# saifahmadgit/go2-sim2real-locomotion-rl

Measured on AMD Instinct MI355X. Metric: env-steps/sec (all envs) Go2 walk 4096 envs; 1/2/4/8-GPU scaling, higher is better.
Workload: dtype f32

## Files before the change

### go2_sim2real_locomotion_rl_amd/csrc/go2sim.hip

```cpp

#include <hip/hip_runtime.h>

#include <algorithm>
#include <cstddef>
#include <cstdint>
#include <cstdio>
#include <cstdlib>
#include <cstring>
#include <new>
#include <vector>

#include "../../include/go2sim.h"
#include "../../include/go2sim_detmath.h"

#define DEV __device__ __forceinline__
#define DEVN __device__ __noinline__

namespace {

constexpr int NL = GO2SIM_NL, ND = GO2SIM_ND, NQ = GO2SIM_NQ, NG = GO2SIM_NG, NJ = GO2SIM_NJ;
constexpr int NPAIR = GO2SIM_NPAIR_MAX, MAXC = GO2SIM_MAX_CONTACTS, MAXB = GO2SIM_MAX_BROAD, MAXR = GO2SIM_MAX_ROWS;
constexpr int JOINT_FIXED = 0, JOINT_REVOLUTE = 1, JOINT_FREE = 4;
constexpr int GEOM_PLANE = 0, GEOM_SPHERE = 1, GEOM_CYLINDER = 3, GEOM_BOX = 5, GEOM_TERRAIN = 7;
constexpr int TERRAIN_CB = 4;
// ... 573 lines not shown
  FA(geom_friction) FA3(l_pos) FA4(l_quat) FA3(root_com) FA(dof_pos) FA3(cd_vel) FA3(cd_ang) FA3(contact_force)
  FA(actions) FA(last_actions) FA(applied_actions) FA2(action_history, NA) FA(target_dof_pos) FA(e_dof_pos) FA(e_dof_vel) FA(last_dof_vel)
  FA(torque) FA(base_pos) FA(base_quat) FA(base_lin_vel) FA(base_ang_vel) FA(projected_gravity) FA(base_euler) FA(commands) FA(time_out)
  FA(kp_factors) FA(kd_factors) FA(motor_strength) FA(gravity_offset) FA(current_push_force) FA(push_stored_force) FA(feet_air_time) FA(base_vel_world) FA(last_base_pos_x)
  FA(episode_sums) FA(rew_terms) FA(rew) FA(obs) FA(priv) FA(base_kp) FA(base_kd)
  IA(n_contacts) IA(n_con) IA(err) IA(is_warmstart) IA(first_time) IA(n_broad) IA(solver_iters) IA(ctrl_mode)
  IA(gjk_fallback) IA(delay_steps) IA(episode_length) IA(reset_buf) IA(push_remaining) IA(foot_contact) IA(last_foot_contact) IA(terrain_row) IA(terrain_key)
  AA(acc) AA(qacc_ws) AA(force) AA(qf_smooth) AA(acc_smooth) AA(qfrc_constraint) AA3(cdof_ang) AA3(cdof_vel) AA3(cdofd_ang)
  AA3(cdofd_vel) AA9(cinr_inertial) AA3(cinr_pos) AA(cinr_mass) AA3(i_pos) AA4(i_quat) AA3(g_pos) AA4(g_quat) AA(sort_value) AA3(c_pos) AA3(c_normal)
  AA(c_pen) AA(c_friction) AA2(c_sol, 7) AA3(c_force) AA(efc_force) AA3(normal_cache)
  AIA(sort_ig) AIA(broad) AIA(c_geom) AIA(c_link) AIA(ncache_valid)
#undef FA
#undef FA3
#undef FA4
#undef FA2
#undef IA
#undef AA
#undef AA3
#undef AA4
#undef AA9
#undef AA2
#undef AIA
};
DEV void team_sync() {
  __builtin_amdgcn_fence(__ATOMIC_RELEASE, "workgroup");
  __builtin_amdgcn_wave_barrier();
  __builtin_amdgcn_fence(__ATOMIC_ACQUIRE, "workgroup");
}
DEV void team_sync_lds() {
  __builtin_amdgcn_fence(__ATOMIC_RELEASE, "workgroup", "local");
  __builtin_amdgcn_wave_barrier();
  __builtin_amdgcn_fence(__ATOMIC_ACQUIRE, "workgroup", "local");
}
DEV float gload(const E& e, int off, int k) { return e.f[(size_t)(off + k) * e.B]; }
DEV void gstore(const E& e, int off, int k, float v) { e.f[(size_t)(off + k) * e.B] = v; }
DEV float aload(const E& e, int off, int k) { return e.fa[off + k]; }
DEV void astore(const E& e, int off, int k, float v) { e.fa[off + k] = v; }


template <int N, int T, class F>
DEV void team_for(int tl, F f) {
#pragma unroll
  for (int k0 = 0; k0 < N; k0 += T) { int k = k0 + tl; if (k < N) f(k); }
}
template <int N, int STRIDE, int R, class FL, class FS>
DEV void team_stage_r(int k0, FL& ld, FS& st) {
  if constexpr (R * STRIDE < N) {
    int k = R * STRIDE + k0;
    k = k < N ? k : N - 1;
    const float v = ld(k);
    team_stage_r<N, STRIDE, R + 1>(k0, ld, st);
    st(k, v);
  }
}
template <int N, int T, class FL, class FS>
DEV void team_stage(int tl, FL ld, FS st) { team_stage_r<N, T, 0>(tl, ld, st); }
template <int EPW, int COUNT, class F>
DEV void wg_load(const Pool& P, int b0, int off, F put) {
  const int ev = threadIdx.x % EPW, k0 = threadIdx.x / EPW;
  const int b = (b0 + ev < P.B) ? b0 + ev : P.B - 1;
  auto ld = [&](int k) { return P.f[(size_t)(off + k) * P.B + b]; };
  auto st = [&](int k, float v) { put(ev, k, v); };
  team_stage_r<COUNT, 64 / EPW, 0>(k0, ld, st);
}

#ifdef GO2SIM_PHASE_PROFILE
// ... 8 lines not shown
#else
#define PH_BEGIN
#define PH(i)
#define PHD_BEGIN
#define PHD(i)
#define PHC(i, n)
#define PHB(i)
#endif

#ifdef GO2SIM_STAMP
constexpr int ST_KINDS = 8, ST_MAX_WG = 4096, ST_DEPTH = 4;
__device__ unsigned long long g_stamp[ST_KINDS * ST_MAX_WG * ST_DEPTH * 2];
__device__ unsigned g_stamp_cnt[ST_KINDS * ST_MAX_WG];
struct StampScope {
  int kind; unsigned long long t0;
  DEV StampScope(int k) : kind(k) { t0 = __builtin_amdgcn_s_memrealtime(); }
  DEV ~StampScope() {
    __builtin_amdgcn_s_waitcnt(0);
    const unsigned long long t1 = __builtin_amdgcn_s_memrealtime();
    if (threadIdx.x == 0 && blockIdx.x < ST_MAX_WG) {
      const int w = kind * ST_MAX_WG + (int)blockIdx.x;
      const unsigned c = g_stamp_cnt[w];
      g_stamp[(w * ST_DEPTH + (int)(c % ST_DEPTH)) * 2] = t0; g_stamp[(w * ST_DEPTH + (int)(c % ST_DEPTH)) * 2 + 1] = t1;
      g_stamp_cnt[w] = c + 1;
    }
  }
};
#define STAMP(kind) StampScope stamp_scope_(kind);
#else
#define STAMP(kind)
#endif
enum { STK_PRE_DYN = 0, STK_COLLIDE, STK_SOLVE, STK_INT_FK_DYN, STK_INT_FK, STK_POST_A, STK_POST_B, STK_OTHER };

enum { SV_COST = 0, SV_PREV_COST, SV_GAUSS, SV_QG0, SV_QG1, SV_QG2, SV_GTOL };
enum { SI_LS_IT = 0, SI_LS_RESULT, SI_IMPROVED };

DEV V3 ld3(const float* p, int i) { return v3(p[3 * i], p[3 * i + 1], p[3 * i + 2]); }
DEV void st3(float* p, int i, V3 v) { p[3 * i] = v.x; p[3 * i + 1] = v.y; p[3 * i + 2] = v.z; }
DEV Q4 ld4(const float* p, int i) { return q4(p[4 * i], p[4 * i + 1], p[4 * i + 2], p[4 * i + 3]); }
DEV void st4(float* p, int i, Q4 q) { p[4 * i] = q.w; p[4 * i + 1] = q.x; p[4 * i + 2] = q.y; p[4 * i + 3] = q.z; }
DEV M3 ld9(const float* p, int i) { M3 r;
#pragma unroll
  for (int k = 0; k < 9; ++k) r.m[k / 3][k % 3] = p[9 * i + k];
  return r; }
DEV void st9(float* p, int i, const M3& r) {
#pragma unroll
  for (int k = 0; k < 9; ++k) p[9 * i + k] = r.m[k / 3][k % 3]; }

DEV int xcd_block() {
  const int n = (int)gridDim.x, q = n >> 3, r = n & 7, x = (int)blockIdx.x & 7, i = (int)blockIdx.x >> 3;
  return (x < r ? x * (q + 1) : r * (q + 1) + (x - r) * q) + i;
}

constexpr int LPT_CLS = 32;
DEV int lpt_solver_xcd(int b, int B, int epw_s) {
  const int n = (B + epw_s - 1) / epw_s, q = n >> 3, r = n & 7, L = b / epw_s;
  if (L < r * (q + 1)) return L / (q + 1);
  return r + (L - r * (q + 1)) / (q > 0 ? q : 1);
}
DEV void lpt_file(int* __restrict__ rec, int cap, int L, int B, int epw_s, int nc) {
  const int x = lpt_solver_xcd(L * epw_s, B, epw_s), cls = LPT_CLS - 1 - imn(LPT_CLS - 1, nc);
  const int pos = atomicAdd(&rec[x * LPT_CLS + cls], 1);
  if (pos < cap) rec[8 * LPT_CLS + (x * LPT_CLS + cls) * cap + pos] = L;
}
DEV int lpt_take(const int* __restrict__ rec, int cap, int B, int epw, int slot) {
  const int ident = xcd_block() * epw + slot;
// ... 6 lines not shown
  for (int c = 0; c < LPT_CLS; ++c) {
    const int k = rec[x * LPT_CLS + c];
    if (cls < 0 && local < total + k) { cls = c; off = local - total; }
    total += k;
  }
  if (total != expected) return ident;
  if (cls < 0 || off >= cap) return B;
  return rec[8 * LPT_CLS + (x * LPT_CLS + cls) * cap + off] * epw + slot;
}

struct KinData {
  float qpos[NQ], vel[ND], qpos_next[NQ], vel_next[ND];
  float l_pos[NL * 3], l_quat[NL * 4], i_pos[NL * 3], i_quat[NL * 4];
  float xanchor[NJ * 3], xaxis[NJ * 3];
  float cdof_ang[ND * 3], cdof_vel[ND * 3];
  float cd_vel[NL * 3], cd_ang[NL * 3];
  float mass[NL];
  int valid;
};

#ifndef GO2SIM_FAST_ORDER
#define GO2SIM_FAST_ORDER 1
#endif
template <int CTRL>
DEV float dpp_perm(float x) { return __int_as_float(__builtin_amdgcn_update_dpp(0, __float_as_int(x), CTRL, 0xf, 0xf, true)); }
#if GO2SIM_FAST_ORDER
constexpr bool ARROW_SHAPE = (ND == 18);
DEV float leg_sum4(float x) {
  const auto r = __builtin_amdgcn_permlane16_swap(__float_as_uint(x), __float_as_uint(x), false, false);
  const float p = __uint_as_float(r[0]) + __uint_as_float(r[1]);
  return p + dpp_perm<0x128>(p);
}
DEV float4 lds4(const float* p) { return *(const float4*)p; }
template <int T, int STRIDE>
DEV void arrow_factor(const int mode, const float eps, const float* A, float* F, int tl) {
  static_assert(T == 32 || T == 64, "four groups of eight lanes");
  const int leg = (tl >> 3) & 3, u = tl & 7, ub = u < 6 ? u : 5;
  const int p0 = dm_arrow_dof(mode, leg, 0), p1 = dm_arrow_dof(mode, leg, 1), p2 = dm_arrow_dof(mode, leg, 2);
  const bool w_lane = tl < 32 && u < 6;
  const float a00 = A[p0 * STRIDE + p0], a10 = A[p1 * STRIDE + p0], a11 = A[p1 * STRIDE + p1];
  const float a20 = A[p2 * STRIDE + p0], a21 = A[p2 * STRIDE + p1], a22 = A[p2 * STRIDE + p2];
  const float c0 = A[p0 * STRIDE + ub], c1 = A[p1 * STRIDE + ub], c2 = A[p2 * STRIDE + ub];
  float br[6];
#pragma unroll
  for (int j = 0; j < 6; ++j) br[j] = A[ub * STRIDE + j];
  team_sync();
  const float e0 = fmx(a00, eps), i0 = dm_sqrt(e0) * (1.0f / e0);
  const float l10 = a10 * i0, l20 = a20 * i0;
  const float e1 = fmx(__builtin_fmaf(-l10, l10, a11), eps), i1 = dm_sqrt(e1) * (1.0f / e1);
  const float l21 = __builtin_fmaf(-l20, l10, a21) * i1;
  const float e2 = fmx(__builtin_fmaf(-l21, l21, __builtin_fmaf(-l20, l20, a22)), eps), i2 = dm_sqrt(e2) * (1.0f / e2);
  const float w0 = c0 * i0, w1 = __builtin_fmaf(-w0, l10, c1) * i1, w2 = __builtin_fmaf(-w1, l21, __builtin_fmaf(-w0, l20, c2)) * i2;
  if (w_lane) *(float4*)&F[32 * leg + 8 + 4 * u] = make_float4(w0, w1, w2, 0.0f);
  if (tl < 32 && u == 0) { *(float4*)&F[32 * leg] = make_float4(i0, i1, i2, 0.0f); *(float4*)&F[32 * leg + 4] = make_float4(l10, l20, l21, 0.0f); }
  team_sync();
  float sc[6];
#pragma unroll
  for (int j = 0; j < 6; ++j) {
    const float4 wj = lds4(&F[32 * leg + 8 + 4 * j]);
    sc[j] = __builtin_fmaf(w2, wj.z, __builtin_fmaf(w1, wj.y, w0 * wj.x));
  }
#pragma unroll
  for (int j = 0; j < 6; ++j) sc[j] = leg_sum4(sc[j]);
  const float bp[6] = {br[0] - sc[0], br[1] - sc[1], br[2] - sc[2], br[3] - sc[3], br[4] - sc[4], br[5] - sc[5]};
  if (tl < 6) { *(float4*)&F[128 + 8 * tl] = make_float4(bp[0], bp[1], bp[2], bp[3]); *(float4*)&F[128 + 8 * tl + 4] = make_float4(bp[4], bp[5], 0.0f, 0.0f); }
  team_sync();
  float a[6][6];
#pragma unroll
  for (int k = 0; k < 6; ++k) {
    const float4 lo = lds4(&F[128 + 8 * k]); const float2 hi = *(const float2*)&F[128 + 8 * k + 4];
    a[k][0] = lo.x; a[k][1] = lo.y; a[k][2] = lo.z; a[k][3] = lo.w; a[k][4] = hi.x; a[k][5] = hi.y;
  }
  team_sync();
#pragma unroll
  for (int k = 0; k < 6; ++k) {
    const float e = fmx(a[k][k], eps), ik = dm_sqrt(e) * (1.0f / e);
    a[k][k] = ik;
#pragma unroll
    for (int j = k + 1; j < 6; ++j) a[j][k] = a[j][k] * ik;
#pragma unroll
    for (int j = k + 1; j < 6; ++j)
#pragma unroll
      for (int i = k + 1; i <= j; ++i) a[j][i] = __builtin_fmaf(-a[j][k], a[i][k], a[j][i]);
  }
  if (tl == 0) {
#pragma unroll
    for (int k = 0; k < 6; ++k) {
      *(float4*)&F[128 + 8 * k] = make_float4(a[k][0], k >= 1 ? a[k][1] : 0.0f, k >= 2 ? a[k][2] : 0.0f, k >= 3 ? a[k][3] : 0.0f);
      *(float2*)&F[128 + 8 * k + 4] = make_float2(k >= 4 ? a[k][4] : 0.0f, k >= 5 ? a[k][5] : 0.0f);
    }
  }
  team_sync();
}
template <int T>
DEV void arrow_solve(const float* F, float gl0, float gl1, float gl2, float gb, float* x6, int tl, float (&xb)[6], float& xl0, float& xl1, float& xl2) {
  static_assert(T == 32 || T == 64, "four groups of eight lanes");
  const int leg = (tl >> 3) & 3, u = tl & 7, ub = u < 6 ? u : 5;
  const float4 iv = lds4(&F[32 * leg]), lv = lds4(&F[32 * leg + 4]), wo = lds4(&F[32 * leg + 8 + 4 * ub]);
  float4 W[6];
#pragma unroll
  for (int b = 0; b < 6; ++b) W[b] = lds4(&F[32 * leg + 8 + 4 * b]);
  float L[6][6];
#pragma unroll
  for (int k = 0; k < 6; ++k) {
    const float4 lo = lds4(&F[128 + 8 * k]); const float2 hi = *(const float2*)&F[128 + 8 * k + 4];
    L[k][0] = lo.x; L[k][1] = lo.y; L[k][2] = lo.z; L[k][3] = lo.w; L[k][4] = hi.x; L[k][5] = hi.y;
  }
  const float y0 = gl0 * iv.x, y1 = __builtin_fmaf(-lv.x, y0, gl1) * iv.y, y2 = __builtin_fmaf(-lv.z, y1, __builtin_fmaf(-lv.y, y0, gl2)) * iv.z;
  const float z = leg_sum4(__builtin_fmaf(wo.z, y2, __builtin_fmaf(wo.y, y1, wo.x * y0)));
  if (tl < 6) x6[tl] = gb - z;
  team_sync();
  const float2 r0 = *(const float2*)&x6[0], r1 = *(const float2*)&x6[2], r2 = *(const float2*)&x6[4];
  float x[6] = {r0.x, r0.y, r1.x, r1.y, r2.x, r2.y};
  team_sync();
#pragma unroll
  for (int k = 0; k < 6; ++k) {
    float acc = x[k];
#pragma unroll
    for (int j = 0; j < k; ++j) acc = __builtin_fmaf(-L[k][j], x[j], acc);
    x[k] = acc * L[k][k];
  }
#pragma unroll
  for (int k_ = 0; k_ < 6; ++k_) {
    const int k = 5 - k_;
    float acc = x[k];
#pragma unroll
    for (int j_ = 0; j_ < 5 - k; ++j_) { const int j = 5 - j_; acc = __builtin_fmaf(-L[j][k], x[j], acc); }
    x[k] = acc * L[k][k];
  }
  float v0 = y0, v1 = y1, v2 = y2;
#pragma unroll
  for (int b = 0; b < 6; ++b) { v0 = __builtin_fmaf(-W[b].x, x[b], v0); v1 = __builtin_fmaf(-W[b].y, x[b], v1); v2 = __builtin_fmaf(-W[b].z, x[b], v2); }
  xl2 = v2 * iv.z; xl1 = __builtin_fmaf(-lv.z, xl2, v1) * iv.y; xl0 = __builtin_fmaf(-lv.x, xl1, __builtin_fmaf(-lv.y, xl2, v0)) * iv.x;
#pragma unroll
  for (int k = 0; k < 6; ++k) xb[k] = x[k];
}
#endif
struct DynData {
  float cinr_I[NL * 9], cinr_pos[NL * 3], cinr_mass[NL];
  float crb_I[NL * 9], crb_pos[NL * 3], crb_mass[NL];
  float cdof_ang[ND * 3], cdof_vel[ND * 3], cdofd_ang[ND * 3], cdofd_vel[ND * 3];
  float cd_vel[NL * 3], cd_ang[NL * 3], cdd_vel[NL * 3], cdd_ang[NL * 3], cfrc_vel[NL * 3], cfrc_ang[NL * 3];
  float f_ang[ND * 3], f_vel[ND * 3];
  float vel[ND], qf_applied[ND], qf_passive[ND], force[ND], out[ND], Dinv[ND];
  float M[ND * ND], L[ND * ND];
  int ctrl_mode[ND];
};
// ... 34 lines not shown
      ql = rotvec_to_quat(m.dofs[J.dof_start].motion_ang * dp, m.eps);
    }
    Q4 qloc[LEG_D];
#pragma unroll
    for (int d = 0; d < LEG_D; ++d) {
      const int src = tl < LEG_K ? LEG_D * tl + d : 0;
      qloc[d] = q4(__shfl(ql.w, src, T), __shfl(ql.x, src, T), __shfl(ql.y, src, T), __shfl(ql.z, src, T));
    }
    if (tl < LEG_K) {
      int lk[LEG_D], jk[LEG_D];
      V3 lpos[LEG_D], jpos[LEG_D], axis[LEG_D]; Q4 lquat[LEG_D];
#pragma unroll
      for (int d = 0; d < LEG_D; ++d) {
        lk[d] = m.leg_links[LEG_D * tl + d];
        const auto& L = m.links[lk[d]];
        jk[d] = L.joint_start;
        const Joint& J = m.joints[jk[d]];
        lpos[d] = L.pos; lquat[d] = L.quat; jpos[d] = J.pos; axis[d] = m.dofs[J.dof_start].motion_ang;
      }
      V3 pos = rpos; Q4 quat = rquat;
#pragma unroll
      for (int d = 0; d < LEG_D; ++d) {
        const Q4 pq = quat;
        pos = pos + transform_by_quat(lpos[d], pq);
        quat = transform_quat_by_quat(lquat[d], pq);
        const V3 anchor = transform_by_quat(jpos[d], quat) + pos;
        st3(s->xanchor, jk[d], anchor);
        st3(s->xaxis, jk[d], transform_by_quat(axis[d], quat));
        quat = transform_quat_by_quat(qloc[d], quat);
        pos = anchor - transform_by_quat(jpos[d], quat);
        st3(s->l_pos, lk[d], pos); st4(s->l_quat, lk[d], quat); e.l_pos()[lk[d]] = pos; e.l_quat()[lk[d]] = quat;
      }
    }
    team_sync();
  }
  for (int lev = 0; lev < (legs ? 0 : m.n_levels); ++lev) {
    for (int k = m.level_start[lev] + tl; k < m.level_start[lev + 1]; k += T) {
      int i_l = m.level_links[k];
      const auto& L = m.links[i_l];
      V3 pos = L.pos; Q4 quat = L.quat;
      if (L.parent != -1) {
        Q4 pq = ld4(s->l_quat, L.parent);
        pos = ld3(s->l_pos, L.parent) + transform_by_quat(L.pos, pq);
        quat = transform_quat_by_quat(L.quat, pq);
      }
      for (int i_j = L.joint_start; i_j < L.joint_end; ++i_j) {
        const Joint& J = m.joints[i_j];
        int q_start = J.q_start, dof_start = J.dof_start;
        if (J.type == JOINT_FREE) {
          V3 pos_ = v3(s->qpos[q_start], s->qpos[q_start + 1], s->qpos[q_start + 2]);
          st3(s->xanchor, i_j, pos_);
          st3(s->xaxis, i_j, v3(0, 0, 1));
          Q4 quat_ = q4(s->qpos[q_start + 3], s->qpos[q_start + 4], s->qpos[q_start + 5], s->qpos[q_start + 6]);
          float n = dm_sqrt(norm_sqr(quat_));
          quat_ = q4(quat_.w / n, quat_.x / n, quat_.y / n, quat_.z / n);
          pos = pos_; quat = quat_;
          gstore(e, FO(dof_pos), dof_start + 0, pos.x); gstore(e, FO(dof_pos), dof_start + 1, pos.y); gstore(e, FO(dof_pos), dof_start + 2, pos.z);
          if (dk) { dk->out[dof_start] = pos.x; dk->out[dof_start + 1] = pos.y; dk->out[dof_start + 2] = pos.z; }
        } else if (J.type == JOINT_REVOLUTE) {
          V3 axis = m.dofs[dof_start].motion_ang;
          V3 anchor = transform_by_quat(J.pos, quat) + pos;
          st3(s->xanchor, i_j, anchor);
          st3(s->xaxis, i_j, transform_by_quat(axis, quat));
          float dp = s->qpos[q_start] - m.qpos0[q_start];
          gstore(e, FO(dof_pos), dof_start, dp);
          if (dk) dk->out[dof_start] = dp;
          Q4 qloc = rotvec_to_quat(axis * dp, m.eps);
          quat = transform_quat_by_quat(qloc, quat);
          pos = anchor - transform_by_quat(J.pos, quat);
        }
      }
      if (!(L.parent == -1 && L.is_fixed)) { st3(s->l_pos, i_l, pos); st4(s->l_quat, i_l, quat); e.l_pos()[i_l] = pos; e.l_quat()[i_l] = quat; }
    }
    team_sync();
  }
  PH(18)
  for (int i_l = tl; i_l < NL; i_l += T) {
    const auto& L = m.links[i_l];
    s->mass[i_l] = L.mass + gload(e, FO(mass_shift), i_l);
    V3 ipbw; Q4 iq;
    transform_pos_quat_by_trans_quat(L.inertial_pos + (V3)e.com_shift()[i_l], L.inertial_quat, ld3(s->l_pos, i_l), ld4(s->l_quat, i_l), ipbw, iq);
    st3(s->i_pos, i_l, ipbw); st4(s->i_quat, i_l, iq);
  }
  team_sync();
  V3 rc[2];
#pragma unroll
  for (int i_e = 0; i_e < 2; ++i_e) {
    const Entity& en = m.entities[i_e];
    V3 root_com_bw = v3(0, 0, 0); float mass_sum = 0.0f;
    for (int i_l = en.link_start; i_l < en.link_end; ++i_l) {
      float mass = s->mass[i_l];
      mass_sum = mass_sum + mass;
      root_com_bw = root_com_bw + mass * ld3(s->i_pos, i_l);
    }
    rc[i_e] = root_com_bw / mass_sum;
  }
  team_sync();
  for (int i_l = tl; i_l < NL; i_l += T) {
    const auto& L = m.links[i_l];
    V3 r = (L.entity == 0) ? rc[0] : rc[1];
    e.root_com()[i_l] = r;
    V3 ip = ld3(s->i_pos, i_l) - r;
    Q4 iq = ld4(s->i_quat, i_l);
    if (!dk) e.i_pos()[i_l] = ip;
    e.i_quat()[i_l] = iq;
    float i_mass = s->mass[i_l];
    M3 oI; V3 op;
    transform_inertia_by_trans_quat(L.inertial_i, i_mass, ip, iq, m.eps, oI, op);
    if (!dk) { e.cinr_inertial()[i_l] = oI; e.cinr_pos()[i_l] = op; e.cinr_mass()[i_l] = i_mass; }
    if (dk) { st9(dk->cinr_I, i_l, oI); st9(dk->crb_I, i_l, oI); st3(dk->cinr_pos, i_l, op); st3(dk->crb_pos, i_l, op); dk->cinr_mass[i_l] = i_mass; dk->crb_mass[i_l] = i_mass; }
  }
  for (int i_j = tl; i_j < NJ; i_j += T) {
    const Joint& J = m.joints[i_j];
    const auto& L = m.links[J.link];
    if (L.n_dofs == 0) continue;
    V3 r = (L.entity == 0) ? rc[0] : rc[1];
    V3 offset_pos = r - ld3(s->xanchor, i_j);
    int ds = J.dof_start;
    if (J.type == JOINT_REVOLUTE) {
      V3 ax = ld3(s->xaxis, i_j);
      V3 cv = cross(ax, offset_pos);
      st3(s->cdof_ang, ds, ax); st3(s->cdof_vel, ds, cv);
      e.cdof_ang()[ds] = ax; e.cdof_vel()[ds] = cv;
      if (dk) { st3(dk->cdof_ang, ds, ax); st3(dk->cdof_vel, ds, cv); }
    } else if (J.type == JOINT_FREE) {
      for (int i = 0; i < 3; ++i) {
        V3 cv = v3(0, 0, 0);
        vset(cv, i, 1.0f);
        st3(s->cdof_ang, i + ds, v3(0, 0, 0)); st3(s->cdof_vel, i + ds, cv);
        e.cdof_ang()[i + ds] = v3(0, 0, 0); e.cdof_vel()[i + ds] = cv;
        if (dk) { st3(dk->cdof_ang, i + ds, v3(0, 0, 0)); st3(dk->cdof_vel, i + ds, cv); }
      }
      M3 xmat_T = transpose(quat_to_R(ld4(s->l_quat, J.link), m.eps));
#pragma unroll
      for (int i = 0; i < 3; ++i) {
        V3 row = v3(xmat_T.m[i][0], xmat_T.m[i][1], xmat_T.m[i][2]);
        V3 cv = cross(row, offset_pos);
        st3(s->cdof_ang, i + ds + 3, row); st3(s->cdof_vel, i + ds + 3, cv);
        e.cdof_ang()[i + ds + 3] = row; e.cdof_vel()[i + ds + 3] = cv;
        if (dk) { st3(dk->cdof_ang, i + ds + 3, row); st3(dk->cdof_vel, i + ds + 3, cv); }
      }
    }
  }
  for (int i_g = tl; i_g < NG; i_g += T) {
    const auto& G = m.geoms[i_g];
    bool is_fixed = m.links[G.link].is_fixed;
    if (force_update_fixed || !is_fixed) {
      V3 p; Q4 q;
      transform_pos_quat_by_trans_quat(G.pos, G.quat, ld3(s->l_pos, G.link), ld4(s->l_quat, G.link), p, q);
      e.g_pos()[i_g] = p; e.g_quat()[i_g] = q;
    }
  }
  team_sync();
  PH(19)
  if (legs) {
    const int r = m.leg_root, ds = m.links[r].dof_start;
    float v[6]; V3 ca[6], cv[6];
#pragma unroll
    for (int i = 0; i < 6; ++i) { v[i] = s->vel[ds + i]; ca[i] = ld3(s->cdof_ang, ds + i); cv[i] = ld3(s->cdof_vel, ds + i); }
    V3 cvel_vel = v3(0, 0, 0), cvel_ang = v3(0, 0, 0);
#pragma unroll
    for (int i = 0; i < 3; ++i) { cvel_vel = cvel_vel + cv[i] * v[i]; cvel_ang = cvel_ang + ca[i] * v[i]; }
    if (tl == 0) {
#pragma unroll
      for (int i = 0; i < 3; ++i) {
        if (!dk) { e.cdofd_ang()[ds + i] = v3(0, 0, 0); e.cdofd_vel()[ds + i] = v3(0, 0, 0); }
        if (dk) { st3(dk->cdofd_ang, ds + i, v3(0, 0, 0)); st3(dk->cdofd_vel, ds + i, v3(0, 0, 0)); }
        V3 oa, ov;
        motion_cross_motion(cvel_ang, cvel_vel, ca[i + 3], cv[i + 3], oa, ov);
        if (!dk) { e.cdofd_ang()[ds + i + 3] = oa; e.cdofd_vel()[ds + i + 3] = ov; }
        if (dk) { st3(dk->cdofd_ang, ds + i + 3, oa); st3(dk->cdofd_vel, ds + i + 3, ov); }
      }
    }
#pragma unroll
    for (int i = 0; i < 3; ++i) { cvel_vel = cvel_vel + cv[i + 3] * v[i + 3]; cvel_ang = cvel_ang + ca[i + 3] * v[i + 3]; }
    if (tl == 0) {
      st3(s->cd_vel, r, cvel_vel); st3(s->cd_ang, r, cvel_ang);
      if (!dk) { e.cd_vel()[r] = cvel_vel; e.cd_ang()[r] = cvel_ang; }
      if (dk) { st3(dk->cd_vel, r, cvel_vel); st3(dk->cd_ang, r, cvel_ang); }
    }
    for (int i_l = tl; i_l < NL; i_l += T) {
      if (m.links[i_l].parent != -1 || i_l == r) continue;
      st3(s->cd_vel, i_l, v3(0, 0, 0)); st3(s->cd_ang, i_l, v3(0, 0, 0));
      if (!dk) { e.cd_vel()[i_l] = v3(0, 0, 0); e.cd_ang()[i_l] = v3(0, 0, 0); }
      if (dk) { st3(dk->cd_vel, i_l, v3(0, 0, 0)); st3(dk->cd_ang, i_l, v3(0, 0, 0)); }
    }
    if (tl < LEG_K) {
      int lk[LEG_D], dd[LEG_D]; float lv[LEG_D]; V3 la[LEG_D], lc[LEG_D];
#pragma unroll
      for (int d = 0; d < LEG_D; ++d) {
        lk[d] = m.leg_links[LEG_D * tl + d];
        dd[d] = m.links[lk[d]].dof_start;
        lv[d] = s->vel[dd[d]]; la[d] = ld3(s->cdof_ang, dd[d]); lc[d] = ld3(s->cdof_vel, dd[d]);
      }
#pragma unroll
      for (int d = 0; d < LEG_D; ++d) {
        V3 oa, ov;
        motion_cross_motion(cvel_ang, cvel_vel, la[d], lc[d], oa, ov);
        if (!dk) { e.cdofd_ang()[dd[d]] = oa; e.cdofd_vel()[dd[d]] = ov; }
        if (dk) { st3(dk->cdofd_ang, dd[d], oa); st3(dk->cdofd_vel, dd[d], ov); }
        cvel_vel = cvel_vel + lc[d] * lv[d];
        cvel_ang = cvel_ang + la[d] * lv[d];
        st3(s->cd_vel, lk[d], cvel_vel); st3(s->cd_ang, lk[d], cvel_ang);
        if (!dk) { e.cd_vel()[lk[d]] = cvel_vel; e.cd_ang()[lk[d]] = cvel_ang; }
        if (dk) { st3(dk->cd_vel, lk[d], cvel_vel); st3(dk->cd_ang, lk[d], cvel_ang); }
      }
    }
    team_sync();
  }
  for (int lev = 0; lev < (legs ? 0 : m.n_levels); ++lev) {
    for (int k = m.level_start[lev] + tl; k < m.level_start[lev + 1]; k += T) {
      int i_l = m.level_links[k];
      const auto& L = m.links[i_l];
      V3 cvel_vel = v3(0, 0, 0), cvel_ang = v3(0, 0, 0);
      if (L.parent != -1) { cvel_vel = ld3(s->cd_vel, L.parent); cvel_ang = ld3(s->cd_ang, L.parent); }
      for (int i_j = L.joint_start; i_j < L.joint_end; ++i_j) {
        const Joint& J = m.joints[i_j];
        int ds = J.dof_start;
        if (J.type == JOINT_FREE) {
          for (int i = 0; i < 3; ++i) {
            float v = s->vel[ds + i];
            cvel_vel = cvel_vel + ld3(s->cdof_vel, ds + i) * v;
            cvel_ang = cvel_ang + ld3(s->cdof_ang, ds + i) * v;
          }
          for (int i = 0; i < 3; ++i) {
            if (!dk) { e.cdofd_ang()[ds + i] = v3(0, 0, 0); e.cdofd_vel()[ds + i] = v3(0, 0, 0); }
            if (dk) { st3(dk->cdofd_ang, ds + i, v3(0, 0, 0)); st3(dk->cdofd_vel, ds + i, v3(0, 0, 0)); }
            V3 oa, ov;
            motion_cross_motion(cvel_ang, cvel_vel, ld3(s->cdof_ang, ds + i + 3), ld3(s->cdof_vel, ds + i + 3), oa, ov);
            if (!dk) { e.cdofd_ang()[ds + i + 3] = oa; e.cdofd_vel()[ds + i + 3] = ov; }
            if (dk) { st3(dk->cdofd_ang, ds + i + 3, oa); st3(dk->cdofd_vel, ds + i + 3, ov); }
          }
          for (int i = 0; i < 3; ++i) {
            float v = s->vel[ds + i + 3];
            cvel_vel = cvel_vel + ld3(s->cdof_vel, ds + i + 3) * v;
            cvel_ang = cvel_ang + ld3(s->cdof_ang, ds + i + 3) * v;
          }
        } else {
          for (int i_d = ds; i_d < J.dof_end; ++i_d) {
            V3 oa, ov;
            motion_cross_motion(cvel_ang, cvel_vel, ld3(s->cdof_ang, i_d), ld3(s->cdof_vel, i_d), oa, ov);
            if (!dk) { e.cdofd_ang()[i_d] = oa; e.cdofd_vel()[i_d] = ov; }
            if (dk) { st3(dk->cdofd_ang, i_d, oa); st3(dk->cdofd_vel, i_d, ov); }
          }
          for (int i_d = ds; i_d < J.dof_end; ++i_d) {
            float v = s->vel[i_d];
            cvel_vel = cvel_vel + ld3(s->cdof_vel, i_d) * v;
            cvel_ang = cvel_ang + ld3(s->cdof_ang, i_d) * v;
          }
        }
      }
      st3(s->cd_vel, i_l, cvel_vel); st3(s->cd_ang, i_l, cvel_ang);
      if (!dk) { e.cd_vel()[i_l] = cvel_vel; e.cd_ang()[i_l] = cvel_ang; }
      if (dk) { st3(dk->cd_vel, i_l, cvel_vel); st3(dk->cd_ang, i_l, cvel_ang); }
    }
    team_sync();
  }
  PH(55)
}

template <int T, class MT>
DEV void tk_integrate(const MT& m, const E& e, KinData* s, int tl) {
  for (int i_l = tl; i_l < NL; i_l += T) {
    const auto& L = m.links[i_l];
    if (L.n_dofs == 0) continue;
    int ds = L.dof_start, qs = L.q_start;
    int joint_type = m.joints[L.joint_start].type;
    if (joint_type == JOINT_FREE) {
      V3 pos = v3(s->qpos[qs], s->qpos[qs + 1], s->qpos[qs + 2]);
      V3 v = v3(s->vel_next[ds], s->vel_next[ds + 1], s->vel_next[ds + 2]);
      pos = pos + v * m.substep_dt;
      s->qpos_next[qs] = pos.x; s->qpos_next[qs + 1] = pos.y; s->qpos_next[qs + 2] = pos.z;
      Q4 rot0 = q4(s->qpos[qs + 3], s->qpos[qs + 4], s->qpos[qs + 5], s->qpos[qs + 6]);
      V3 ang = v3(s->vel_next[ds + 3], s->vel_next[ds + 4], s->vel_next[ds + 5]) * m.substep_dt;
      Q4 qrot = rotvec_to_quat(ang, m.eps);
      Q4 rot = transform_quat_by_quat(qrot, rot0);
      s->qpos_next[qs + 3] = rot.w; s->qpos_next[qs + 4] = rot.x; s->qpos_next[qs + 5] = rot.y; s->qpos_next[qs + 6] = rot.z;
    } else {
      for (int j_ = 0; j_ < L.q_end - qs; ++j_) s->qpos_next[qs + j_] = s->qpos[qs + j_] + s->vel_next[ds + j_] * m.substep_dt;
    }
  }
  team_sync();
  bool bad = false;
  for (int d = tl; d < ND; d += T) bad |= isnan_(s->vel_next[d]);
  for (int q = tl; q < NQ; q += T) bad |= isnan_(s->qpos_next[q]);
  if (bad) s->valid = 0;
  team_sync();
  if (s->valid) {
    for (int d = tl; d < ND; d += T) { float v = s->vel_next[d]; s->vel[d] = v; gstore(e, FO(vel), d, v); }
    for (int q = tl; q < NQ; q += T) { float v = s->qpos_next[q]; s->qpos[q] = v; gstore(e, FO(qpos), q, v); }
  } else if (tl == 0) {
    atomicOr(&e.err()[0], GO2SIM_ERR_INVALID_ACC_NAN);
  }
  team_sync();
}

template <int T>
DEV void integrate_fk_body(const Pool& P, const ModelS* __restrict__ mp, int b, KinData* lds, char* ms_raw, bool pre, float pre_vel, float pre_acc) {
  const ModelS& ms = *(const ModelS*)ms_raw;
  wg_dma_to_lds<(int)sizeof(ModelS)>(ms_raw, mp);
  const int tl = threadIdx.x % T, slot = threadIdx.x / T;
  const ModelView m(&ms, mp);
  E e(P, b < P.B ? b : P.B - 1);
  KinData* s = &lds[slot];
  PH_BEGIN
  if (pre) { if (tl < ND) { s->vel[tl] = pre_vel; s->vel_next[tl] = pre_acc; } }
  else {
    team_stage<ND, T>(tl, [&](int d) { return gload(e, FO(vel), d); }, [&](int d, float v) { s->vel[d] = v; });
    team_stage<ND, T>(tl, [&](int d) { return aload(e, AO(acc), d); }, [&](int d, float a) { s->vel_next[d] = a; });
  }
  team_stage<NQ, T>(tl, [&](int q) { return gload(e, FO(qpos), q); }, [&](int q, float v) { s->qpos[q] = v; });
  team_for<ND, T>(tl, [&](int d) { s->vel_next[d] = s->vel[d] + s->vel_next[d] * m.substep_dt; });
  if (tl == 0) s->valid = 1;
  tk_stage_links<T>(e, s, tl);
  team_sync();
  if (b >= P.B) return;
  tk_integrate<T>(m, e, s, tl);
  PH(40)
  tk_kinematics<T>(m, e, s, tl, false);
  PH(41)
}
template <int T>
__global__ __launch_bounds__(64) void k_integrate_fk_team(Pool P, const ModelS* __restrict__ mp) {
  STAMP(STK_INT_FK)
  constexpr int EPW = 64 / T;
  __shared__ KinData lds[EPW];
  __shared__ alignas(16) char ms_raw[MODELS_LDS_BYTES];
  integrate_fk_body<T>(P, mp, xcd_block() * EPW + (int)threadIdx.x / T, lds, ms_raw, false, 0.0f, 0.0f);
}

template <int T>
__global__ __launch_bounds__(64) void k_fk_team(Pool P, const ModelS* __restrict__ mp, int force_update_fixed, const int* __restrict__ cond) {
  constexpr int EPW = 64 / T;
  __shared__ KinData lds[EPW];
  __shared__ alignas(16) char ms_raw[MODELS_LDS_BYTES];
  const ModelS& ms = *(const ModelS*)ms_raw;
  if (cond && *cond <= 0) return;
  wg_dma_to_lds<(int)sizeof(ModelS)>(ms_raw, mp);
  const int tl = threadIdx.x % T, slot = threadIdx.x / T;
  const int b = xcd_block() * EPW + slot;
  const ModelView m(&ms, mp);
  E e(P, b < P.B ? b : P.B - 1);
  KinData* s = &lds[slot];
  team_stage<ND, T>(tl, [&](int d) { return gload(e, FO(vel), d); }, [&](int d, float v) { s->vel[d] = v; });
  team_stage<NQ, T>(tl, [&](int q) { return gload(e, FO(qpos), q); }, [&](int q, float v) { s->qpos[q] = v; });
  tk_stage_links<T>(e, s, tl);
  team_sync();
  if (b >= P.B) return;
  tk_kinematics<T>(m, e, s, tl, force_update_fixed != 0);
}

template <int T, class MT>
DEV void tk_dynamics(const MT& m, const E& e, DynData* s, int tl, bool env_valid) {
  PH_BEGIN
  const bool legs = (T == 32 || T == 64) && m.leg_form;
  if (legs) {
    for (int c = tl; c < 13; c += T) {
      auto at = [&](int i_l) -> float* { return (c < 9) ? &s->crb_I[9 * i_l + c] : ((c < 12) ? &s->crb_pos[3 * i_l + c - 9] : &s->crb_mass[i_l]); };
      const int r = m.leg_root;
      float x[LEG_K][LEG_D];
#pragma unroll
      for (int l = 0; l < LEG_K; ++l)
#pragma unroll
        for (int d = 0; d < LEG_D; ++d) x[l][d] = *at(m.leg_links[LEG_D * l + d]);
      float a = *at(r);
#pragma unroll
      for (int l = 0; l < LEG_K; ++l) {
#pragma unroll
        for (int d = LEG_D - 2; d >= 0; --d) { x[l][d] = x[l][d] + x[l][d + 1]; *at(m.leg_links[LEG_D * l + d]) = x[l][d]; }
      }
#pragma unroll
      for (int l = 0; l < LEG_K; ++l) a = a + x[l][0];
      *at(r) = a;
    }
    team_sync();
  }
  for (int lev = (legs ? -1 : m.n_levels - 2); lev >= 0; --lev) {
    int n_par = m.level_start[lev + 1] - m.level_start[lev];
    for (int w = tl; w < n_par * 13; w += T) {
      int i_p = m.level_links[m.level_start[lev] + w / 13], comp = w % 13;
      float* dst = (comp < 9) ? &s->crb_I[9 * i_p + comp] : ((comp < 12) ? &s->crb_pos[3 * i_p + comp - 9] : &s->crb_mass[i_p]);
      float a = *dst;
      for (int c = m.child_start[i_p]; c < m.child_start[i_p + 1]; ++c) {
        int i_l = m.child_list[c];
        float v = (comp < 9) ? s->crb_I[9 * i_l + comp] : ((comp < 12) ? s->crb_pos[3 * i_l + comp - 9] : s->crb_mass[i_l]);
        a = a + v;
      }
      *dst = a;
    }
    team_sync();
  }
  PH(21)
  for (int i_d = tl; i_d < ND; i_d += T) {
    int i_l = m.dof_link[i_d];
    V3 oa, ov;
    inertial_mul(ld3(s->crb_pos, i_l), ld9(s->crb_I, i_l), s->crb_mass[i_l], ld3(s->cdof_vel, i_d), ld3(s->cdof_ang, i_d), oa, ov);
    st3(s->f_ang, i_d, oa); st3(s->f_vel, i_d, ov);
  }
  team_sync();
  for (int idx = tl; idx < ND * (ND + 1) / 2; idx += T) {
    int i_d, j_d;
    tri_index(m, idx, i_d, j_d);
    float v = (dot(ld3(s->f_ang, i_d), ld3(s->cdof_ang, j_d)) + dot(ld3(s->f_vel, i_d), ld3(s->cdof_vel, j_d))) * mass_mask(m, i_d, j_d);
    if (i_d == j_d) {
      v = v + m.dofs[i_d].armature;
      v = v + m.dofs[i_d].damping * m.substep_dt;
      int cm = s->ctrl_mode[i_d];
      if (cm == CTRL_POSITION || cm == CTRL_VELOCITY) v = v + m.dofs[i_d].kv * m.substep_dt;
    }
    s->M[i_d * ND + j_d] = v; s->M[j_d * ND + i_d] = v;
    s->L[i_d * ND + j_d] = v;
  }
  team_sync();
  PH(22)
#if GO2SIM_FAST_ORDER
  const bool arrow = ARROW_SHAPE && (T == 32 || T == 64) && m.arrow_mode != 0;
  float* const AF = (float*)(((uintptr_t)s->L + 15) & ~(uintptr_t)15);
#else
  const bool arrow = false;
#endif
  if constexpr (T == 32 || T == 64) {
#if GO2SIM_FAST_ORDER
    if (arrow) arrow_factor<T, ND>(m.arrow_mode, m.eps, s->M, AF, tl);
#endif
  }
  if (arrow) {
  } else if constexpr (T >= ND) {
    const int row = tl < ND ? tl : ND - 1;
    float Lr[ND];
#pragma unroll
    for (int k = 0; k < ND; ++k) Lr[k] = s->L[row * ND + k];
    float dinv_own = 0.0f;
#pragma unroll
    for (int i_d_ = 0; i_d_ < ND; ++i_d_) {
      const int i_d = ND - i_d_ - 1;
      if (i_d_ > 0) {
        if (tl == i_d) {
#pragma unroll
          for (int k = 0; k <= i_d; ++k) s->L[i_d * ND + k] = Lr[k];
        }
        team_sync();
      }
      float ri[ND];
#pragma unroll
      for (int k = 0; k <= i_d; ++k) ri[k] = s->L[i_d * ND + k];
      const float lij = s->L[i_d * ND + (row < i_d ? row : 0)];
      const float D_inv = 1.0f / ri[i_d];
      if (row == i_d) dinv_own = D_inv;
      const bool act = row < i_d;
      const float a = lij * D_inv;
#pragma unroll
      for (int k = 0; k < i_d; ++k) { const float nv = Lr[k] - a * ri[k]; Lr[k] = act ? nv : Lr[k]; }
    }
    team_sync();
    if (tl < ND) {
#pragma unroll
      for (int k = 0; k < ND; ++k) if (k < row) s->L[row * ND + k] = Lr[k] * dinv_own;
      s->L[row * ND + row] = 1.0f;
      s->Dinv[row] = dinv_own;
    }
    team_sync();
  } else {
#pragma unroll
    for (int i_d_ = 0; i_d_ < ND; ++i_d_) {
      const int i_d = ND - i_d_ - 1;
      float D_inv = 1.0f / s->L[i_d * ND + i_d];
      for (int idx = tl; idx < i_d * (i_d + 1) / 2; idx += T) {
        int j_d, k_d;
        tri_index(m, idx, j_d, k_d);
        float a = s->L[i_d * ND + j_d] * D_inv;
        s->L[j_d * ND + k_d] -= a * s->L[i_d * ND + k_d];
      }
      team_sync();
      for (int j_d = tl; j_d < i_d; j_d += T) s->L[i_d * ND + j_d] = s->L[i_d * ND + j_d] * D_inv;
      if (tl == 0) { s->Dinv[i_d] = D_inv; s->L[i_d * ND + i_d] = 1.0f; }
      team_sync();
    }
  }
  PH(23)
  for (int i_d = tl; i_d < ND; i_d += T) {
    const Dof& D = m.dofs[i_d];
    const auto& L = m.links[m.dof_link[i_d]];
    int joint_type = m.joints[L.joint_start].type;
    float force = 0.0f;
    int cm = s->ctrl_mode[i_d];
    const float in_ctrl_force = s->qf_applied[i_d], in_ctrl_pos = s->qf_passive[i_d], in_ctrl_vel = s->force[i_d], in_dof_pos = s->out[i_d];
    if (cm == CTRL_FORCE) force = in_ctrl_force;
    else if (cm == CTRL_VELOCITY) force = D.kv * (in_ctrl_vel - s->vel[i_d]);
    else if (cm == CTRL_POSITION && !(joint_type == JOINT_FREE && i_d >= L.dof_start + 3))
      force = D.kp * (in_ctrl_pos - in_dof_pos) + D.kv * (in_ctrl_vel - s->vel[i_d]);
    s->qf_applied[i_d] = clampf(force, D.force_range[0], D.force_range[1]);
    float qp = -D.damping * s->vel[i_d];
    if (joint_type != JOINT_FREE && joint_type != JOINT_FIXED) qp = qp + (-in_dof_pos * D.stiffness);
    s->qf_passive[i_d] = qp;
  }
  if (legs) {
    const int r = m.leg_root;
    if (tl < 6 * LEG_K) {
      const int l = tl / 6, c = tl % 6;
      const float* src = (c < 3) ? s->cdofd_vel : s->cdofd_ang;
      const int cc = (c < 3) ? c : c - 3;
      const V3 g0 = -m.gravity * (1.0f - 0.0f);
      const int ds = m.links[r].dof_start;
      float vr[6], xr[6], vl[LEG_D], xl[LEG_D]; int lk[LEG_D];
#pragma unroll
      for (int i = 0; i < 6; ++i) { vr[i] = s->vel[ds + i]; xr[i] = src[3 * (ds + i) + cc]; }
#pragma unroll
      for (int d = 0; d < LEG_D; ++d) {
        lk[d] = m.leg_links[LEG_D * l + d];
        const int i_d = m.links[lk[d]].dof_start;
        vl[d] = s->vel[i_d]; xl[d] = src[3 * i_d + cc];
      }
      float* dst = (c < 3) ? s->cdd_vel : s->cdd_ang;
      float a = (c < 3) ? ((cc == 0) ? g0.x : ((cc == 1) ? g0.y : g0.z)) : 0.0f;
#pragma unroll
      for (int i = 0; i < 6; ++i) a = a + xr[i] * vr[i];
      if (l == 0) dst[3 * r + cc] = a;
#pragma unroll
      for (int d = 0; d < LEG_D; ++d) { a = a + xl[d] * vl[d]; dst[3 * lk[d] + cc] = a; }
    }
    for (int i_l = tl; i_l < NL; i_l += T) {
      if (m.links[i_l].parent != -1 || i_l == r) continue;
      st3(s->cdd_vel, i_l, -m.gravity * (1.0f - 0.0f)); st3(s->cdd_ang, i_l, v3(0, 0, 0));
    }
    team_sync();
  }
  for (int lev = 0; lev < (legs ? 0 : m.n_levels); ++lev) {
    for (int k = m.level_start[lev] + tl; k < m.level_start[lev + 1]; k += T) {
      int i_l = m.level_links[k];
      const auto& L = m.links[i_l];
      V3 cv, ca;
      if (L.parent == -1) { cv = -m.gravity * (1.0f - 0.0f); ca = v3(0, 0, 0); }
      else { cv = ld3(s->cdd_vel, L.parent); ca = ld3(s->cdd_ang, L.parent); }
      for (int i_d = L.dof_start; i_d < L.dof_end; ++i_d) {
        float v = s->vel[i_d];
        V3 local_cdd_vel = ld3(s->cdofd_vel, i_d) * v;
        V3 local_cdd_ang = ld3(s->cdofd_ang, i_d) * v;
        cv = cv + local_cdd_vel;
        ca = ca + local_cdd_ang;
      }
      st3(s->cdd_vel, i_l, cv); st3(s->cdd_ang, i_l, ca);
    }
    team_sync();
  }
  for (int i_l = tl; i_l < NL; i_l += T) {
    V3 f1_ang, f1_vel, f2_ang, f2_vel, f3_ang, f3_vel;
    M3 I = ld9(s->cinr_I, i_l); V3 cp = ld3(s->cinr_pos, i_l); float cm = s->cinr_mass[i_l];
    V3 cdv = ld3(s->cd_vel, i_l), cda = ld3(s->cd_ang, i_l);
    inertial_mul(cp, I, cm, ld3(s->cdd_vel, i_l), ld3(s->cdd_ang, i_l), f1_ang, f1_vel);
    inertial_mul(cp, I, cm, cdv, cda, f2_ang, f2_vel);
    motion_cross_force(cda, cdv, f2_ang, f2_vel, f3_ang, f3_vel);
    V3 ext_ang = ld3(s->cfrc_ang, i_l), ext_vel = ld3(s->cfrc_vel, i_l);
    st3(s->cfrc_vel, i_l, f1_vel + f3_vel + ext_vel + v3(0, 0, 0));
    st3(s->cfrc_ang, i_l, f1_ang + f3_ang + ext_ang + v3(0, 0, 0));
  }
  team_sync();
  if (legs) {
    for (int c = tl; c < 6; c += T) {
      auto at = [&](int i_l) -> float* { return (c < 3) ? &s->cfrc_vel[3 * i_l + c] : &s->cfrc_ang[3 * i_l + c - 3]; };
      const int r = m.leg_root;
      float x[LEG_K][LEG_D];
#pragma unroll
      for (int l = 0; l < LEG_K; ++l)
#pragma unroll
        for (int d = 0; d < LEG_D; ++d) x[l][d] = *at(m.leg_links[LEG_D * l + d]);
      float a = *at(r);
#pragma unroll
      for (int l = 0; l < LEG_K; ++l) {
#pragma unroll
        for (int d = LEG_D - 2; d >= 0; --d) { x[l][d] = x[l][d] + x[l][d + 1]; *at(m.leg_links[LEG_D * l + d]) = x[l][d]; }
      }
#pragma unroll
      for (int l = 0; l < LEG_K; ++l) a = a + x[l][0];
      *at(r) = a;
    }
    team_sync();
  }
  for (int lev = (legs ? -1 : m.n_levels - 2); lev >= 0; --lev) {
    int n_par = m.level_start[lev + 1] - m.level_start[lev];
    for (int w = tl; w < n_par * 6; w += T) {
      int i_p = m.level_links[m.level_start[lev] + w / 6], comp = w % 6;
      float* dst = (comp < 3) ? &s->cfrc_vel[3 * i_p + comp] : &s->cfrc_ang[3 * i_p + comp - 3];
      float a = *dst;
      for (int c = m.child_start[i_p]; c < m.child_start[i_p + 1]; ++c) {
        int i_l = m.child_list[c];
        a = a + ((comp < 3) ? s->cfrc_vel[3 * i_l + comp] : s->cfrc_ang[3 * i_l + comp - 3]);
      }
      *dst = a;
    }
    team_sync();
  }
  for (int i_d = tl; i_d < ND; i_d += T) {
    int i_l = m.dof_link[i_d];
    float qf_bias = dot(ld3(s->cdof_ang, i_d), ld3(s->cfrc_ang, i_l)) + dot(ld3(s->cdof_vel, i_d), ld3(s->cfrc_vel, i_l));
    float f = s->qf_passive[i_d] - qf_bias + s->qf_applied[i_d];
    s->force[i_d] = f;
    if (env_valid) { astore(e, AO(force), i_d, f); astore(e, AO(qf_smooth), i_d, f); }
  }
  team_sync();
  PH(24)
  bool solved = false;
#if GO2SIM_FAST_ORDER
  if constexpr (T == 32 || T == 64) {
    if (arrow) {
      const int leg = (tl >> 3) & 3, u = tl & 7, ub = u < 6 ? u : 5;
      const int p0 = dm_arrow_dof(m.arrow_mode, leg, 0), p1 = dm_arrow_dof(m.arrow_mode, leg, 1), p2 = dm_arrow_dof(m.arrow_mode, leg, 2);
      float xb[6], x0, x1, x2;
      arrow_solve<T>(AF, s->force[p0], s->force[p1], s->force[p2], s->force[ub], s->Dinv, tl, xb, x0, x1, x2);
      if (tl == 0) {
#pragma unroll
        for (int k = 0; k < 6; ++k) s->out[k] = xb[k];
      }
      if (tl < 32 && u == 0) { s->out[p0] = x0; s->out[p1] = x1; s->out[p2] = x2; }
      solved = true;
    }
  }
#endif
  if (!solved) {
    float y[ND];
#pragma unroll
    for (int i_d_ = 0; i_d_ < ND; ++i_d_) {
      const int i_d = ND - i_d_ - 1;
      float cur = s->force[i_d];
#pragma unroll
      for (int j_d = i_d + 1; j_d < ND; ++j_d) cur = cur - s->L[j_d * ND + i_d] * y[j_d];
      y[i_d] = cur;
    }
#pragma unroll
    for (int i_d = 0; i_d < ND; ++i_d) y[i_d] = y[i_d] * s->Dinv[i_d];
#pragma unroll
    for (int i_d = 0; i_d < ND; ++i_d) {
      float cur = y[i_d];
#pragma unroll
      for (int j_d = 0; j_d < i_d; ++j_d) cur = cur - s->L[i_d * ND + j_d] * y[j_d];
      y[i_d] = cur;
    }
    if (tl == 0) {
#pragma unroll
      for (int i_d = 0; i_d < ND; ++i_d) s->out[i_d] = y[i_d];
    }
  }
  team_sync();
  if (env_valid) for (int i_d = tl; i_d < ND; i_d += T) { float a = s->out[i_d]; astore(e, AO(acc_smooth), i_d, a); astore(e, AO(acc), i_d, a); }
  if (env_valid) for (int idx = tl; idx < NTRI; idx += T) { int i, j; tri_index(m, idx, i, j); astore(e, AO(mass_mat), idx, s->M[i * ND + j]); }
  PH(25)
}

template <int T> DEV unsigned long long team_ballot(bool p) {
  const unsigned long long b = __ballot(p);
  if constexpr (T == 64) return b;
  else return (b >> (threadIdx.x & (64 - T))) & ((1ull << T) - 1ull);
}
template <int T>
struct BroadData {
  alignas(16) float amin[NG * 4], amax[NG * 4];
  alignas(16) unsigned long long skey[2 * NG];
  alignas(8) int rank_mm[NG * 2];
  int cand_key[MAXB], cand_pair[MAXB];
  unsigned pair_sorted[MAXB];
};
static_assert(NPAIR <= (1 << 16) && NG <= (1 << 8), "broad_word: 8 bits per geom, 16 bits of pair index");
DEV unsigned broad_word(int packed, int pidx) { return (unsigned)packed | ((unsigned)pidx << 16); }
constexpr int BROAD_PAD = 12;
template <int T> constexpr bool BROAD_OVERLAY = sizeof(BroadData<T>) + BROAD_PAD <= sizeof(DynData);
template <bool OVERLAY, int T> struct BroadSeparate { BroadData<T> k[64 / T]; DEV BroadData<T>* at(int slot, DynData*) { return &k[slot]; } };
template <int T> struct BroadSeparate<true, T> {
  DEV BroadData<T>* at(int slot, DynData* d) {
    static_assert(sizeof(BroadData<T>) + BROAD_PAD <= sizeof(DynData) && sizeof(DynData) % 4 == 0 && alignof(BroadData<T>) == 16, "BroadData overlay");
    return (BroadData<T>*)((char*)d + (16 - (slot * (int)sizeof(DynData)) % 16) % 16);
  }
};
static_assert((BROAD_OVERLAY<16> && BROAD_OVERLAY<32> && BROAD_OVERLAY<64>) || NG != 28 || ND != 18, "the Go2 shape keeps the dynamics kernels' LDS size");

template <int T>
DEV void tk_broadphase(const Model& m, const E& e, BroadData<T>* s, int tl) {
  const float inf = dm_bits2f(0x7f800000u);
  PH_BEGIN
  const int nc_old = e.n_contacts()[0];
  const bool first = e.first_time()[0] != 0;
  const unsigned ncv_old = (unsigned)e.ncache_valid()[tl < NCV ? tl : NCV - 1];
  constexpr int n2 = 2 * NG, NK = (2 * NG + T - 1) / T, NPI = (NPAIR + T - 1) / T, NGR = (NG + T - 1) / T;
  int sig_[NK];
#pragma unroll
  for (int q = 0; q < NK; ++q) { const int i = tl + q * T; sig_[q] = e.sort_ig()[i < n2 ? i : n2 - 1]; }
  int packed_[NPI];
  {
    const int n_pairs = m.n_pairs;
#pragma unroll
    for (int it = 0; it < NPI; ++it) { int pidx = it * T + tl; int v = m.pair_list[pidx < NPAIR ? pidx : NPAIR - 1]; packed_[it] = (pidx < n_pairs) ? v : -1; }
  }
  V3 lower_[NGR], upper_[NGR];
#pragma unroll
  for (int g = 0; g < NGR; ++g) {
    const int i_g = (g * T + tl < NG) ? g * T + tl : NG - 1;
    V3 lower = v3(inf, inf, inf), upper = v3(-inf, -inf, -inf);
    V3 gp = e.g_pos()[i_g]; Q4 gq = e.g_quat()[i_g];
#pragma unroll
    for (int c = 0; c < 8; ++c) {
      V3 corner = transform_by_trans_quat(m.geoms[i_g].aabb[c], gp, gq);
      lower = vmin(lower, corner); upper = vmax(upper, corner);
    }
    lower_[g] = lower; upper_[g] = upper;
  }
  team_sync();
#pragma unroll
  for (int g = 0; g < NGR; ++g) {
    const int i_g = (g * T + tl < NG) ? g * T + tl : NG - 1;
    *(float4*)&s->amin[4 * i_g] = make_float4(lower_[g].x, lower_[g].y, lower_[g].z, 0.0f);
    *(float4*)&s->amax[4 * i_g] = make_float4(upper_[g].x, upper_[g].y, upper_[g].z, 0.0f);
  }
  team_sync();
  PH(30)
  int r[NK]; float sorted_v[NK]; int sorted_sg[NK];
  unsigned long long key[NK];
#pragma unroll
  for (int q = 0; q < NK; ++q) {
    const int i = (tl + q * T < n2) ? tl + q * T : n2 - 1;
    const int sg = first ? ((i >> 1) | ((i & 1) ? 0x100 : 0)) : sig_[q];
    const int g = sg & 0xff;
    const float v = (sg & 0x100) ? s->amax[4 * g] : s->amin[4 * g];
    unsigned u = (unsigned)__float_as_int(v + 0.0f);
    u = (u & 0x80000000u) ? ~u : (u | 0x80000000u);
    key[q] = ((unsigned long long)u << 8) | (unsigned long long)i;
    s->skey[i] = key[q];
    sorted_v[q] = v; sorted_sg[q] = sg; r[q] = 0;
  }
  team_sync();
#pragma unroll
  for (int j = 0; j < 2 * NG; ++j) {
    const unsigned long long kj = s->skey[j];
#pragma unroll
    for (int q = 0; q < NK; ++q) r[q] += (kj < key[q]) ? 1 : 0;
  }
#pragma unroll
  for (int q = 0; q < NK; ++q)
    if (tl + q * T < n2) s->rank_mm[2 * (sorted_sg[q] & 0xff) + ((sorted_sg[q] & 0x100) ? 1 : 0)] = r[q];
  team_sync();
  PH(31)
  int n_cand = 0;
  unsigned ncv_clear = 0u;
  static_assert(NCV <= T, "one lane per word of the normal-cache mask");
#pragma unroll
  for (int it = 0; it < NPI; ++it) {
    const int packed = packed_[it];
    const int a = (packed < 0) ? 0 : (packed & 0xff), bg = (packed < 0) ? 0 : (packed >> 8);
    const int2 rka = *(const int2*)&s->rank_mm[2 * a], rkb = *(const int2*)&s->rank_mm[2 * bg];
    const float4 amn = *(const float4*)&s->amin[4 * a], amx = *(const float4*)&s->amax[4 * a], bmn = *(const float4*)&s->amin[4 * bg], bmx = *(const float4*)&s->amax[4 * bg];
    const int ra = rka.x, rb = rkb.x;
    const int rs = (ra < rb) ? rb : ra, rf = (ra < rb) ? ra : rb;
    const int rmax_first = (ra < rb) ? rka.y : rkb.y;
    const bool swept = packed >= 0 && rs < rmax_first;
    const bool any1 = (amx.x <= bmn.x) || (amx.y <= bmn.y) || (amx.z <= bmn.z);
    const bool any2 = (amn.x >= bmx.x) || (amn.y >= bmx.y) || (amn.z >= bmx.z);
    const bool cand = swept && !(any1 || any2);
    const unsigned long long cb = team_ballot<T>(cand);
    if (cand) {
      const int pos = n_cand + __popcll(cb & ((1ull << tl) - 1ull));
      if (pos < MAXB) { s->cand_key[pos] = rs * 64 + rf; s->cand_pair[pos] = (int)broad_word(packed, it * T + tl); }
    }
    n_cand += __popcll(cb);
    const unsigned long long sep = team_ballot<T>(swept && (any1 || any2));
    if constexpr (T < 32) { if (tl == ((it * T) >> 5)) ncv_clear |= (unsigned)(sep << ((it * T) & 31)); }
    else if constexpr (T == 32) { if (tl == it) ncv_clear |= (unsigned)sep; }
    else { if (tl == 2 * it) ncv_clear |= (unsigned)sep; if (tl == 2 * it + 1) ncv_clear |= (unsigned)(sep >> 32); }
  }
  const bool overflow = n_cand > m.max_broad_pairs;
  n_cand = imn(n_cand, MAXB);
  team_sync();
  for (int c = tl; c < n_cand; c += T) {
    const int ck = s->cand_key[c]; int cr = 0;
    for (int j = 0; j < n_cand; ++j) cr += s->cand_key[j] < ck;
    s->pair_sorted[cr] = (unsigned)s->cand_pair[c];
  }
  const int n_broad = imn(n_cand, m.max_broad_pairs);
  team_sync();
  for (int c = tl; c < n_broad; c += T) e.broad()[c] = (int)s->pair_sorted[c];
#pragma unroll
  for (int q = 0; q < NK; ++q) if (tl + q * T < n2) { e.sort_value()[r[q]] = sorted_v[q]; e.sort_ig()[r[q]] = sorted_sg[q]; }
  if (tl < NCV && ncv_clear != 0u) e.ncache_valid()[tl] = (int)(ncv_old & ~ncv_clear);
  if (tl == 0) {
    e.n_broad()[0] = n_broad;
    if (first) e.first_time()[0] = 0;
    if (overflow) atomicOr(&e.err()[0], GO2SIM_ERR_OVERFLOW_CANDIDATE_CONTACTS);
  }
  for (int i_c = tl; i_c < nc_old; i_c += T) {
    e.c_link()[i_c] = -1; e.c_link()[MAXC + i_c] = -1; e.c_geom()[i_c] = -1; e.c_geom()[MAXC + i_c] = -1;
    e.c_pen()[i_c] = 0.0f; e.c_pos()[i_c] = v3(0, 0, 0); e.c_normal()[i_c] = v3(0, 0, 0); e.c_force()[i_c] = v3(0, 0, 0);
  }
  PH(32)
}

template <int T>
__global__ __launch_bounds__(64) void k_dynamics_team(Pool P, const ModelS* __restrict__ mp, const Model* __restrict__ gm) {
  constexpr int EPW = 64 / T;
  __shared__ alignas(16) DynData lds[EPW];
  __shared__ alignas(16) char ms_raw[MODELS_LDS_BYTES];
  __shared__ BroadSeparate<BROAD_OVERLAY<T>, T> lds_b;
  const ModelS& ms = *(const ModelS*)ms_raw;
  wg_dma_to_lds<(int)sizeof(ModelS)>(ms_raw, mp);
  {
    const int b0 = xcd_block() * EPW;
    wg_load<EPW, NL * 3>(P, b0, FO(cd_vel), [&](int ev, int k, float v) { lds[ev].cd_vel[k] = v; });
    wg_load<EPW, NL * 3>(P, b0, FO(cd_ang), [&](int ev, int k, float v) { lds[ev].cd_ang[k] = v; });
    wg_load<EPW, ND>(P, b0, FO(vel), [&](int ev, int k, float v) { lds[ev].vel[k] = v; });
  }
  const int tl = threadIdx.x % T, slot = threadIdx.x / T;
  const int b = xcd_block() * EPW + slot;
  const bool env_valid = b < P.B;
  const ModelView m(&ms, mp);
  E e(P, env_valid ? b : P.B - 1);
  DynData* s = &lds[slot];
  PH_BEGIN
  team_stage<NL * 9, T>(tl, [&](int k) { return aload(e, AO(cinr_inertial), k); }, [&](int k, float v) { s->cinr_I[k] = v; s->crb_I[k] = v; });
  team_stage<NL * 3, T>(tl, [&](int k) { return aload(e, AO(cinr_pos), k); }, [&](int k, float v) { s->cinr_pos[k] = v; s->crb_pos[k] = v; });
  team_stage<NL, T>(tl, [&](int k) { return aload(e, AO(cinr_mass), k); }, [&](int k, float v) { s->cinr_mass[k] = v; s->crb_mass[k] = v; });
  team_stage<ND, T>(tl, [&](int d) { return __int_as_float((int)e.ctrl_mode()[d]); }, [&](int d, float v) { s->ctrl_mode[d] = __float_as_int(v); });
  team_stage<ND * 3, T>(tl, [&](int k) { return aload(e, AO(cdof_ang), k); }, [&](int k, float v) { s->cdof_ang[k] = v; });
  team_stage<ND * 3, T>(tl, [&](int k) { return aload(e, AO(cdof_vel), k); }, [&](int k, float v) { s->cdof_vel[k] = v; });
  team_stage<ND * 3, T>(tl, [&](int k) { return aload(e, AO(cdofd_ang), k); }, [&](int k, float v) { s->cdofd_ang[k] = v; });
  team_stage<ND * 3, T>(tl, [&](int k) { return aload(e, AO(cdofd_vel), k); }, [&](int k, float v) { s->cdofd_vel[k] = v; });
  team_stage<ND, T>(tl, [&](int d) { return gload(e, FO(ctrl_force), d); }, [&](int d, float v) { s->qf_applied[d] = v; });
  team_stage<ND, T>(tl, [&](int d) { return gload(e, FO(ctrl_pos), d); }, [&](int d, float v) { s->qf_passive[d] = v; });
  team_stage<ND, T>(tl, [&](int d) { return gload(e, FO(ctrl_vel), d); }, [&](int d, float v) { s->force[d] = v; });
  team_stage<ND, T>(tl, [&](int d) { return gload(e, FO(dof_pos), d); }, [&](int d, float v) { s->out[d] = v; });
  team_stage<NL * 6, T>(tl, [&](int k) { return gload(e, FO(ext), k); },
                        [&](int k, float v) { int i_l = k / 6, c = k % 6; if (c < 3) s->cfrc_ang[3 * i_l + c] = v; else s->cfrc_vel[3 * i_l + c - 3] = v; });
  team_sync();
  PH(20)
  tk_dynamics<T>(m, e, s, tl, env_valid);
  if (env_valid) tk_broadphase<T>(*gm, e, lds_b.at(slot, s), tl);
}


template <bool OVERLAY, int EPW> struct KinSeparate { KinData k[EPW]; DEV KinData* at(int slot, void*) { return &k[slot]; } };
template <int EPW> struct KinSeparate<true, EPW> { DEV KinData* at(int, void* overlay) { return (KinData*)overlay; } };
constexpr bool KIN_OVERLAY = sizeof(KinData) <= 2 * sizeof(float) * ND * ND;
template <int T>
DEV void integrate_fk_dynamics_body(const Pool& P, const ModelS* __restrict__ mp, const Model* __restrict__ gm, int b, DynData* lds_d, char* ms_raw,
                                    KinSeparate<KIN_OVERLAY, 64 / T>& lds_k, BroadSeparate<BROAD_OVERLAY<T>, T>& lds_b, bool pre, float pre_vel, float pre_acc) {
  const ModelS& ms = *(const ModelS*)ms_raw;
  wg_dma_to_lds<(int)sizeof(ModelS)>(ms_raw, mp);
  const int tl = threadIdx.x % T, slot = threadIdx.x / T;
  const ModelView m(&ms, mp);
  asm volatile("" : "+v"(b));
  E e(P, b < P.B ? b : P.B - 1);
  DynData* d = &lds_d[slot];
  static_assert(offsetof(DynData, L) == offsetof(DynData, M) + sizeof(float) * ND * ND, "KinData overlay");
  KinData* s = lds_k.at(slot, d->M);
  PH_BEGIN
  if (pre) { if (tl < ND) { s->vel[tl] = pre_vel; s->vel_next[tl] = pre_acc; } }
  else {
    team_stage<ND, T>(tl, [&](int i) { return gload(e, FO(vel), i); }, [&](int i, float v) { s->vel[i] = v; });
    team_stage<ND, T>(tl, [&](int i) { return aload(e, AO(acc), i); }, [&](int i, float a) { s->vel_next[i] = a; });
  }
  team_stage<NQ, T>(tl, [&](int q) { return gload(e, FO(qpos), q); }, [&](int q, float v) { s->qpos[q] = v; });
  team_stage<ND, T>(tl, [&](int i) { return __int_as_float((int)e.ctrl_mode()[i]); }, [&](int i, float v) { d->ctrl_mode[i] = __float_as_int(v); });
  team_stage<ND, T>(tl, [&](int i) { return gload(e, FO(ctrl_force), i); }, [&](int i, float v) { d->qf_applied[i] = v; });
  team_stage<ND, T>(tl, [&](int i) { return gload(e, FO(ctrl_pos), i); }, [&](int i, float v) { d->qf_passive[i] = v; });
  team_stage<ND, T>(tl, [&](int i) { return gload(e, FO(ctrl_vel), i); }, [&](int i, float v) { d->force[i] = v; });
  team_stage<NL * 6, T>(tl, [&](int k) { return gload(e, FO(ext), k); },
                        [&](int k, float v) { int i_l = k / 6, c = k % 6; if (c < 3) d->cfrc_ang[3 * i_l + c] = v; else d->cfrc_vel[3 * i_l + c - 3] = v; });
  team_for<ND, T>(tl, [&](int i) { s->vel_next[i] = s->vel[i] + s->vel_next[i] * m.substep_dt; });
  if (tl == 0) s->valid = 1;
  tk_stage_links<T>(e, s, tl);
  team_sync();
  if (b >= P.B) return;
  tk_integrate<T>(m, e, s, tl);
  PH(40)
  tk_kinematics<T>(m, e, s, tl, false, d);
  team_for<ND, T>(tl, [&](int i) { d->vel[i] = s->vel[i]; });
  team_sync();
  PH(41)
  tk_dynamics<T>(m, e, d, tl, true);
  tk_broadphase<T>(*gm, e, lds_b.at(slot, d), tl);
}
template <int T>
__global__ __launch_bounds__(64) void k_integrate_fk_dynamics_team(Pool P, const ModelS* __restrict__ mp, const Model* __restrict__ gm) {
  STAMP(STK_INT_FK_DYN)
  constexpr int EPW = 64 / T;
  __shared__ alignas(16) DynData lds_d[EPW];
  __shared__ alignas(16) char ms_raw[MODELS_LDS_BYTES];
  __shared__ KinSeparate<KIN_OVERLAY, EPW> lds_k;
  __shared__ BroadSeparate<BROAD_OVERLAY<T>, T> lds_b;
  integrate_fk_dynamics_body<T>(P, mp, gm, xcd_block() * EPW + (int)threadIdx.x / T, lds_d, ms_raw, lds_k, lds_b, false, 0.0f, 0.0f);
}

DEV int wrap180(float x) {
  if (!(x >= 0.0f)) return 0;
  int i = (x >= 180.0f) ? (int)(x - 180.0f) : (int)x;
  return (i > 179) ? 179 : i;
}
DEV int clampidx(float x) {
  if (!(x >= 0.0f)) return 0;
  return (x >= 179.0f) ? 179 : (int)x;
}
DEV V3 support_cylinder_local(const Model& m, const Geom& G, V3 d_mesh, int* vid_out = nullptr) {
  const float PI = 3.14159265358979323846f;
  float theta = dm_atan2(d_mesh.y, d_mesh.x);
// ... 626 lines not shown
}

template <int T>
__global__ __launch_bounds__(64) void k_collide_team(Pool P, const Model* __restrict__ mp, const GeomK* __restrict__ gkp, GjkStoreFull* __restrict__ gjk_scratch, int* __restrict__ lpt_rec, int lpt_cap, int solver_epw) {
  STAMP(STK_COLLIDE)
  constexpr int EPW = 64 / T;
  __shared__ CollideData<T> lds[EPW];
  __shared__ alignas(16) char gk_raw[GEOMK_LDS_BYTES];
  static_assert(T != 16 || NG != 28 || sizeof(CollideData<T>) * EPW + GEOMK_LDS_BYTES <= 40960, "k_collide_team<16>: four workgroups per CU");
  wg_dma_to_lds<GEOMK_BYTES>(gk_raw, gkp);
  const GeomK* gk = (const GeomK*)gk_raw;
  const int tl = threadIdx.x % T, slot = threadIdx.x / T;
  const int b = xcd_block() * EPW + slot;
  if (slot >= EPW || b >= P.B) return;
  const Model& m = *mp;
  E e(P, b);
  CollideData<T>* s = &lds[slot];
  PH_BEGIN
  constexpr int NPRE = (T == 16) ? 2 : 1;
  static_assert(NPRE * T <= MAXB, "the unconditional pair-word loads stay inside e.broad()");
  const int n_broad_ld = e.n_broad()[0];
  unsigned ncv_ld[(NCV + T - 1) / T]; int pw_ld[NPRE];
#pragma unroll
  for (int q = 0; q < (NCV + T - 1) / T; ++q) { const int i = tl + q * T; ncv_ld[q] = (unsigned)e.ncache_valid()[i < NCV ? i : NCV - 1]; }
#pragma unroll
  for (int q = 0; q < NPRE; ++q) pw_ld[q] = e.broad()[tl + q * T];
  if (tl == 0) s->gjk_slot_mask = 0u;
  const int n_broad = imn(imx(n_broad_ld, 0), MAXB);
#pragma unroll
  for (int q = 0; q < (NCV + T - 1) / T; ++q) if (tl + q * T < NCV) s->ncv[tl + q * T] = ncv_ld[q];
#pragma unroll
  for (int q = 0; q < NPRE; ++q) if (tl + q * T < n_broad) s->pair_w[tl + q * T] = (unsigned)pw_ld[q];
  for (int c = tl + NPRE * T; c < n_broad; c += T) s->pair_w[c] = (unsigned)e.broad()[c];
  team_sync();
  PH(62)
  int nc_run = 0;
  const int n_np_iter = (n_broad + T - 1) / T;
  struct PairConst { float friction, sol[7]; int link_a, link_b; };
  struct Fric { float gf_a, fr_a, gf_b, fr_b; };
  auto load_fric = [&](int i_ga, int i_gb) { Fric f = {e.geom_friction()[i_ga], e.friction_ratio()[i_ga], e.geom_friction()[i_gb], e.friction_ratio()[i_gb]}; return f; };
  auto pair_const = [&](int i_ga, int i_gb, const Fric& f) {
    PairConst pc;
    float friction_a = f.gf_a * f.fr_a;
    float friction_b = f.gf_b * f.fr_b;
    pc.friction = fmx(fmx(friction_a, friction_b), 1e-2f);
#pragma unroll
    for (int q = 0; q < 7; ++q) pc.sol[q] = 0.5f * (gk[i_ga].sol_params[q] + gk[i_gb].sol_params[q]);
    pc.link_a = gk[i_ga].link; pc.link_b = gk[i_gb].link;
    return pc;
  };
  static_assert(MAX_CONTACTS_PER_PAIR < 8, "append_staged: three bits of contact count");
  auto append_staged = [&](const ContactStage& cs, int i_ga, int i_gb, const PairConst& pc) {
    const unsigned long long b0 = team_ballot<T>((cs.n & 1) != 0), b1 = team_ballot<T>((cs.n & 2) != 0), b2 = team_ballot<T>((cs.n & 4) != 0);
    const unsigned long long below = (1ull << tl) - 1ull;
    const int off = __popcll(b0 & below) + 2 * __popcll(b1 & below) + 4 * __popcll(b2 & below);
    const int tot = __popcll(b0) + 2 * __popcll(b1) + 4 * __popcll(b2);
    for (int k = 0; k < cs.n; ++k) {
      int i_c = nc_run + off + k;
      if (i_c < m.max_contact_pairs) {
        const float* p = cs.st + 7 * k;
        e.c_geom()[i_c] = i_ga; e.c_geom()[MAXC + i_c] = i_gb;
        e.c_normal()[i_c] = v3(p[0], p[1], p[2]); e.c_pos()[i_c] = v3(p[3], p[4], p[5]); e.c_pen()[i_c] = p[6];
        e.c_friction()[i_c] = pc.friction;
        auto sol = e.c_sol()[i_c];
#pragma unroll
        for (int q = 0; q < 7; ++q) sol[q] = pc.sol[q];
        e.c_link()[i_c] = pc.link_a; e.c_link()[MAXC + i_c] = pc.link_b;
// ... 261 lines not shown
DEV int update_bracket(LsPoint& p, const float alphas[3], const float costs[3], const float grads[3], const float hess[3], float& p_next_alpha) {
  int flag = 0;
#pragma unroll
  for (int i = 0; i < 3; ++i) {
    if (p.grad < 0 && grads[i] < 0 && p.grad < grads[i]) { p.alpha = alphas[i]; p.cost = costs[i]; p.grad = grads[i]; p.hess = hess[i]; flag = 1; }
    else if (p.grad > 0 && grads[i] > 0 && p.grad > grads[i]) { p.alpha = alphas[i]; p.cost = costs[i]; p.grad = grads[i]; p.hess = hess[i]; flag = 2; }
  }
  p_next_alpha = p.alpha;
  if (flag > 0) p_next_alpha = p.alpha - p.grad / p.hess;
  return flag;
}

struct BrOut { float alpha, cost, grad, hess, next_alpha; int flag; };
DEVN BrOut update_bracket_v(float pa, float pc, float pg, float ph, float a0, float a1, float a2, float c0, float c1, float c2, float g0, float g1, float g2,
                            float h0, float h1, float h2) {
  LsPoint p = {pa, pc, pg, ph};
  const float alphas[3] = {a0, a1, a2}, costs[3] = {c0, c1, c2}, grads[3] = {g0, g1, g2}, hess[3] = {h0, h1, h2};
  int flag = 0;
#pragma unroll
  for (int i = 0; i < 3; ++i) {
    if (p.grad < 0 && grads[i] < 0 && p.grad < grads[i]) { p.alpha = alphas[i]; p.cost = costs[i]; p.grad = grads[i]; p.hess = hess[i]; flag = 1; }
    else if (p.grad > 0 && grads[i] > 0 && p.grad > grads[i]) { p.alpha = alphas[i]; p.cost = costs[i]; p.grad = grads[i]; p.hess = hess[i]; flag = 2; }
  }
  float next_alpha = p.alpha;
  if (flag > 0) next_alpha = p.alpha - p.grad / p.hess;
  BrOut o = {p.alpha, p.cost, p.grad, p.hess, next_alpha, flag};
  return o;
}

constexpr int RL = 32;
constexpr int RL_TERRAIN = 96;
constexpr int DS = 20;

template <int R>
struct alignas(16) SolverData {
  float J[R * DS];
  float H[ND * DS];
  float M[ND * DS];
  float qacc[DS], Ma[DS], grad[DS], Mgrad[DS], search[DS], mv[DS], force[DS], acc_smooth[DS], qfrc[DS], ntv[DS], vel[DS];
  union {
    struct { float cdof_ang[ND * 3], cdof_vel[ND * 3], root_com[NL * 3]; alignas(16) float rot[ND][4]; };
    float Ablk[21 * 9];
  };
  alignas(16) float aref[R];
  alignas(16) float efc_D[R]; alignas(16) float Jaref[R]; alignas(16) float jv[R]; alignas(16) float efc_force[R];
  alignas(16) float qf0[R]; alignas(16) float qf1[R]; alignas(16) float qf2[R]; alignas(16) float DA[R];
  alignas(16) int active[R]; alignas(16) int prev_active[R];
};

template <int T>
DEV float team_bcast(float x, const int k) {
  if constexpr (T == 64) {
    return __int_as_float(__builtin_amdgcn_readlane(__float_as_int(x), k));
  } else if constexpr (T == 32) {
    const int lo = __builtin_amdgcn_readlane(__float_as_int(x), k), hi = __builtin_amdgcn_readlane(__float_as_int(x), 32 + k);
    return __int_as_float((threadIdx.x & 32) ? hi : lo);
  } else {
    return __shfl(x, k, T);
  }
}
template <int T>
DEV float team_bcast_dyn(float x, int k_uniform) {
  static_assert(T == 32 || T == 64, "teams of 32 or 64 lanes");
  const int k = __builtin_amdgcn_readfirstlane(k_uniform);
  if constexpr (T == 64) {
    return __int_as_float(__builtin_amdgcn_readlane(__float_as_int(x), k));
  } else {
    const int lo = __builtin_amdgcn_readlane(__float_as_int(x), k), hi = __builtin_amdgcn_readlane(__float_as_int(x), 32 + k);
// ... 41 lines not shown
#pragma unroll
  for (int q = 0; q < NQ; ++q) {
    const auto r = __builtin_amdgcn_permlane16_swap(__float_as_uint(a[q]), __float_as_uint(a[q]), false, false);
    const float pair = __uint_as_float(r[0]) + __uint_as_float(r[1]);
    if constexpr (T == 32) total[q] = pair;
    else { const auto h = __builtin_amdgcn_permlane32_swap(__float_as_uint(pair), __float_as_uint(pair), false, false); total[q] = __uint_as_float(h[0]) + __uint_as_float(h[1]); }
  }
}
template <int T>
DEV float team_tree_sum1(float x) { const float xs[1] = {x}; float t[1]; team_tree_sum<T, 1>(xs, t); return t[0]; }

template <int T, class S, class MT>
DEV void ts_update_constraint(const MT& m, S* s, int tl, int n_con, float& cost, float& prev_cost, float& gauss) {
  prev_cost = cost;
  float row_cost = 0.0f;
  bool first_row = true;
  for (int c = tl; c < n_con; c += T) {
    s->prev_active[c] = s->active[c];
    float Ja = s->Jaref[c];
    int act = Ja < 0.0f;
    s->active[c] = act;
    float D = s->efc_D[c];
    const float DA = D * (float)act;
    s->DA[c] = DA;
    s->efc_force[c] = 0.0f + (-Ja * D * (float)act);
    const float rc = 0.5f * (Ja * Ja * DA);
#if GO2SIM_FAST_ORDER
    row_cost = first_row ? rc : row_cost + rc;
    first_row = false;
#else
    row_cost = rc;
#endif
  }
  team_sync();
  for (int d = tl; d < ND; d += T) {
    float q = 0.0f;
#pragma unroll 16
    for (int c = 0; c < n_con; ++c) q = q + s->J[c * DS + d] * s->efc_force[c];
    s->qfrc[d] = q;
  }
  bool done = false;
#if GO2SIM_FAST_ORDER
  if constexpr (T >= 32) {
    const int d = tl < ND ? tl : ND - 1;
    const float v = 0.5f * (s->Ma[d] - s->force[d]) * (s->qacc[d] - s->acc_smooth[d]);
    const float xs[2] = {tl < ND ? v : 0.0f, row_cost};
    float tot[2];
    team_tree_sum<T, 2>(xs, tot);
    gauss = tot[0]; cost = tot[1] + tot[0];
    done = true;
  }
#endif
  if constexpr (T >= 32 && !GO2SIM_FAST_ORDER) {
    const int n_wave = __builtin_amdgcn_readfirstlane(imx(__shfl(n_con, 0), __shfl(n_con, T == 64 ? 0 : 32)));
    if (n_wave <= T) {
      const int d = tl < ND ? tl : ND - 1;
      const float v = 0.5f * (s->Ma[d] - s->force[d]) * (s->qacc[d] - s->acc_smooth[d]);
      const float xd[1] = {tl < ND ? v : 0.0f}, zero[1] = {0.0f};
      float g[1], ct[1];
      team_serial_sum<T, 1>(xd, zero, tl, 2, g);
      const float xr[1] = {tl < n_con ? row_cost : 0.0f};
      team_serial_sum<T, 1>(xr, g, tl, (n_wave + 15) / 16, ct);
      gauss = g[0]; cost = (n_wave > 0) ? ct[0] : g[0];
      done = true;
    }
  }
  if (!done) {
    float cost_i = 0.0f, gauss_i = 0.0f;
#pragma unroll
    for (int d = 0; d < ND; ++d) {
      float v = 0.5f * (s->Ma[d] - s->force[d]) * (s->qacc[d] - s->acc_smooth[d]);
      gauss_i = gauss_i + v;
      cost_i = cost_i + v;
    }
#pragma unroll 16
    for (int c = 0; c < n_con; ++c) { float Ja = s->Jaref[c]; cost_i = cost_i + 0.5f * (Ja * Ja * s->DA[c]); }
    gauss = gauss_i; cost = cost_i;
  }
  team_sync();
}

#if GO2SIM_FAST_ORDER
template <int T, class S, class MT>
DEV void ts_hessian_direct(const MT& m, S* s, int tl, int n_con) {
  constexpr int NB = 21, G = (T >= 3 * NB) ? 3 : 1;
  for (int u0 = 0; u0 < NB * G; u0 += T) {
    const int u = u0 + tl;
    const bool on = u < NB * G;
    const int g = on ? u / NB : 0, blk = on ? u - NB * g : 0;
    const int bi = (blk >= 15) ? 5 : (blk >= 10) ? 4 : (blk >= 6) ? 3 : (blk >= 3) ? 2 : (blk >= 1) ? 1 : 0;
    const int bj = blk - bi * (bi + 1) / 2;
    float h[3][3];
#pragma unroll
    for (int a = 0; a < 3; ++a)
#pragma unroll
      for (int q = 0; q < 3; ++q) h[a][q] = 0.0f;
    const float* Ji = &s->J[3 * bi];
    const float* Jj = &s->J[3 * bj];
    const int n_c = on ? n_con : 0;
#pragma unroll 4
    for (int c = g; c < n_c; c += G) {
      const float D = s->DA[c];
      float jd[3], jj[3];
#pragma unroll
      for (int a = 0; a < 3; ++a) { const float j1 = Ji[c * DS + a]; jd[a] = (dm_abs(j1) > m.eps) ? j1 * D : 0.0f; jj[a] = Jj[c * DS + a]; }
#pragma unroll
      for (int a = 0; a < 3; ++a)
#pragma unroll
        for (int q = 0; q < 3; ++q) h[a][q] = __builtin_fmaf(jj[q], jd[a], h[a][q]);
    }
    if constexpr (G == 3) {
#pragma unroll
      for (int a = 0; a < 3; ++a)
#pragma unroll
        for (int q = 0; q < 3; ++q) { const float p1 = __shfl(h[a][q], tl + NB, T), p2 = __shfl(h[a][q], tl + 2 * NB, T); h[a][q] = (h[a][q] + p1) + p2; }
    }
    if (on && g == 0) {
#pragma unroll
      for (int a = 0; a < 3; ++a)
#pragma unroll
        for (int q = 0; q < 3; ++q) {
          const int i = 3 * bi + a, j = 3 * bj + q;
          const float v = h[a][q] + s->M[i * DS + j];
          if constexpr (T >= NB) s->Ablk[blk * 9 + 3 * a + q] = v;
          if (j <= i) s->H[i * DS + j] = v;
        }
    }
  }
  team_sync();
}
template <int T, class S, class MT>
DEV void ts_hessian_update(const MT& m, S* s, int tl, int n_con) {
  constexpr int NB = 21;
  static_assert(T >= NB, "one lane per block");
  const bool on = tl < NB;
  const int blk = on ? tl : 0;
  const int bi = (blk >= 15) ? 5 : (blk >= 10) ? 4 : (blk >= 6) ? 3 : (blk >= 3) ? 2 : (blk >= 1) ? 1 : 0;
  const int bj = blk - bi * (bi + 1) / 2;
  float h[3][3];
#pragma unroll
  for (int a = 0; a < 3; ++a)
#pragma unroll
    for (int q = 0; q < 3; ++q) h[a][q] = s->Ablk[blk * 9 + 3 * a + q];
  const float* Ji = &s->J[3 * bi];
  const float* Jj = &s->J[3 * bj];
  for (int base = 0; base < n_con; base += T) {
    const int c_me = base + tl;
    unsigned long long mask = team_ballot<T>(c_me < n_con && ((s->active[c_me] != 0) != (s->prev_active[c_me] != 0)));
    while (mask != 0ull) {
      const int c = base + __ffsll((long long)mask) - 1;
      mask &= mask - 1ull;
      const float D = s->efc_D[c], sg = (s->active[c] != 0) ? 1.0f : -1.0f;
      float jd[3], jj[3];
#pragma unroll
      for (int a = 0; a < 3; ++a) { const float j1 = Ji[c * DS + a]; jd[a] = (dm_abs(j1) > m.eps) ? sg * (j1 * D) : 0.0f; jj[a] = Jj[c * DS + a]; }
#pragma unroll
      for (int a = 0; a < 3; ++a)
#pragma unroll
        for (int q = 0; q < 3; ++q) h[a][q] = __builtin_fmaf(jj[q], jd[a], h[a][q]);
    }
  }
  if (on) {
#pragma unroll
    for (int a = 0; a < 3; ++a)
#pragma unroll
      for (int q = 0; q < 3; ++q) {
        const int i = 3 * bi + a, j = 3 * bj + q;
        s->Ablk[blk * 9 + 3 * a + q] = h[a][q];
        if (j <= i) s->H[i * DS + j] = h[a][q];
      }
  }
  team_sync();
}
#else
template <int T, class S, class MT>
DEV void ts_hessian_direct(const MT& m, S* s, int tl, int n_con) {
  for (int idx = tl; idx < ND * (ND + 1) / 2; idx += T) {
    int i, j;
    tri_index(m, idx, i, j);
    float h = 0.0f;
#pragma unroll 16
    for (int c = 0; c < n_con; ++c) {
      float j1 = s->J[c * DS + i];
      float t = s->J[c * DS + j] * j1 * s->DA[c];
      h = (dm_abs(j1) > m.eps) ? (h + t) : h;
    }
    h = h + s->M[i * DS + j];
    s->H[i * DS + j] = h;
  }
  team_sync();
}
#endif

template <int T, class S, class MT>
DEV void ts_cholesky_factor_columns(const MT& m, S* s, int tl) {
#pragma unroll
  for (int i_d = 0; i_d < ND; ++i_d) {
    float pr[ND];
#pragma unroll
    for (int k = 0; k < i_d; ++k) pr[k] = s->H[i_d * DS + k];
    float tmp = s->H[i_d * DS + i_d];
#pragma unroll
    for (int k = 0; k < i_d; ++k) tmp = tmp - pr[k] * pr[k];
    float dgn = dm_sqrt(fmx(tmp, m.eps));
    float inv = 1.0f / dgn;
    if (tl == 0) s->H[i_d * DS + i_d] = dgn;
    for (int j_d = i_d + 1 + tl; j_d < ND; j_d += T) {
      float dotv = 0.0f;
#pragma unroll
      for (int k = 0; k < i_d; ++k) dotv = dotv + s->H[j_d * DS + k] * pr[k];
      float v = (s->H[j_d * DS + i_d] - dotv) * inv;
      s->H[j_d * DS + i_d] = v; s->H[i_d * DS + j_d] = v;
    }
    team_sync();
  }
}
template <int T, class S, class MT>
DEV void ts_cholesky_factor_rows(const MT& m, S* s, int tl) {
  static_assert(T >= ND, "one lane per row");
  const int row = tl < ND ? tl : ND - 1;
  const bool own = tl < ND;
  float r[ND];
#pragma unroll
  for (int k = 0; k < ND; ++k) r[k] = s->H[row * DS + k];
#pragma unroll
  for (int k = 0; k < ND; ++k) {
    const float akk = team_bcast<T>(r[k], k);
    const float d = dm_sqrt(fmx(akk, m.eps));
    const float inv = 1.0f / d;
    const float l = r[k] * inv;
    if (own && row >= k) s->H[row * DS + k] = (row == k) ? d : l;
    if (k < ND - 1) {
      if (own && row > k) s->H[k * DS + row] = l;
      team_sync();
      float col[ND];
#pragma unroll
      for (int i = k + 1; i < ND; ++i) col[i] = s->H[k * DS + i];
#pragma unroll
      for (int i = k + 1; i < ND; ++i) r[i] = __builtin_fmaf(-l, col[i], r[i]);
    }
  }
  team_sync();
}
#if GO2SIM_FAST_ORDER
template <int T, class S, class MT>
DEV void ts_cholesky_factor_arrow(const MT& m, S* s, int tl) { arrow_factor<T, DS>(m.arrow_mode, m.eps, s->H, s->H, tl); }
template <int T, class S, class MT>
DEV float ts_update_gradient_arrow(const MT& m, S* s, int tl) {
  const int leg = (tl >> 3) & 3, u = tl & 7, ub = u < 6 ? u : 5;
  const int p0 = dm_arrow_dof(m.arrow_mode, leg, 0), p1 = dm_arrow_dof(m.arrow_mode, leg, 1), p2 = dm_arrow_dof(m.arrow_mode, leg, 2);
  const int row = tl < ND ? tl : ND - 1;
  const float g_own = s->Ma[row] - s->force[row] - s->qfrc[row];
  const float gl0 = s->Ma[p0] - s->force[p0] - s->qfrc[p0], gl1 = s->Ma[p1] - s->force[p1] - s->qfrc[p1], gl2 = s->Ma[p2] - s->force[p2] - s->qfrc[p2];
  const float gb = s->Ma[ub] - s->force[ub] - s->qfrc[ub];
  if (tl < ND) s->grad[row] = g_own;
  const float grad_sq = team_tree_sum1<T>(tl < ND ? g_own * g_own : 0.0f);
  float xb[6], x0, x1, x2;
  arrow_solve<T>(s->H, gl0, gl1, gl2, gb, s->Mgrad, tl, xb, x0, x1, x2);
  if (tl == 0) { *(float4*)&s->Mgrad[0] = make_float4(xb[0], xb[1], xb[2], xb[3]); *(float2*)&s->Mgrad[4] = make_float2(xb[4], xb[5]); }
  if (tl < 32 && u == 0) { s->Mgrad[p0] = x0; s->Mgrad[p1] = x1; s->Mgrad[p2] = x2; }
  team_sync();
  return grad_sq;
}
#endif
template <int T, class S, class MT>
DEV void ts_cholesky_factor(const MT& m, S* s, int tl) {
#if GO2SIM_FAST_ORDER
  if constexpr (T >= ND) { ts_cholesky_factor_rows<T>(m, s, tl); return; }
#endif
  ts_cholesky_factor_columns<T>(m, s, tl);
}

template <int T, class S, class MT>
DEV bool ts_cholesky_incremental_reg(const MT& m, S* s, int tl, int n_con) {
  static_assert(T >= ND, "one lane per row of the factor");
  bool degenerated = false, touched = false;
  const int row = tl < ND ? tl : ND - 1;
  float Lr[ND];
#pragma unroll
  for (int k = 0; k < ND; ++k) Lr[k] = s->H[row * DS + k];
  for (int base = 0; base < n_con && !degenerated; base += T) {
    const int c_me = base + tl;
    const bool flip = c_me < n_con && ((s->active[c_me] != 0) != (s->prev_active[c_me] != 0));
    const unsigned long long bal = __ballot(flip);
    unsigned long long mask = (T == 64) ? bal : ((bal >> ((threadIdx.x / T) * T)) & ((1ull << (T & 63)) - 1ull));
    PHC(50, 1)
    while (mask != 0ull && !degenerated) {
      PHC(51, 1)
      const int c = base + __ffsll((long long)mask) - 1;
      mask &= mask - 1ull;
      touched = true;
      const float sign = (s->active[c] != 0) ? 1.0f : -1.0f;
      const float efc_D_sqrt = dm_sqrt(s->efc_D[c]);
      float v = s->J[c * DS + row] * efc_D_sqrt;
#pragma unroll
      for (int k = 0; k < ND; ++k) {
        const float vk = team_bcast<T>(v, k), Lkk = team_bcast<T>(Lr[k], k);
        if (dm_abs(vk) > m.eps) {
          const float tmp = Lkk * Lkk + sign * (vk * vk);
          if (tmp < m.eps) { degenerated = true; break; }
          const float r = dm_sqrt(tmp);
          const float cc = r / Lkk;
          const float cinv = 1.0f / cc;
          const float sk = vk / Lkk;
          if (row == k) Lr[k] = r;
          else if (row > k) {
            const float hik = (Lr[k] + sk * v * sign) * cinv;
            Lr[k] = hik;
            v = v * cc - sk * hik;
          }
        }
      }
    }
  }
  if (touched && !degenerated && tl < ND) {
#pragma unroll
    for (int k = 0; k < ND; ++k)
      if (k <= row) { s->H[row * DS + k] = Lr[k]; if (k < row) s->H[k * DS + row] = Lr[k]; }
  }
  team_sync();
  return degenerated;
}
template <int T, int FMAX, class S, class MT>
DEV bool ts_cholesky_incremental_pipelined(const MT& m, S* s, int tl, int n_con) {
  static_assert(T >= ND && (T == 32 || T == 64), "one lane per row of the factor");
  bool degenerated = false;
  const int row = tl < ND ? tl : ND - 1;
  const bool own = tl < ND;
  const unsigned urow = own ? (unsigned)row : 0u;
  float Ld = s->H[row * DS + row];
  for (int base = 0; base < n_con && !degenerated; base += T) {
    const int c_me = base + tl;
    const bool flip = c_me < n_con && ((s->active[c_me] != 0) != (s->prev_active[c_me] != 0));
    const unsigned long long bal = __ballot(flip);
    unsigned long long mask = (T == 64) ? bal : ((bal >> ((threadIdx.x / T) * T)) & ((1ull << (T & 63)) - 1ull));
    while (mask != 0ull && !degenerated) {
      float W[FMAX], sg[FMAX]; int nb = 0;
#pragma unroll
      for (int f = 0; f < FMAX; ++f) {
        W[f] = 0.0f; sg[f] = 0.0f;
        if (mask != 0ull) {
          const int c = base + __ffsll((long long)mask) - 1;
          mask &= mask - 1ull;
          W[f] = s->J[c * DS + row] * dm_sqrt(s->efc_D[c]);
          sg[f] = (s->active[c] != 0) ? 1.0f : -1.0f;
          nb = f + 1;
        }
      }
      const int nb_wave = __builtin_amdgcn_readfirstlane(imx(__shfl(nb, 0), __shfl(nb, T == 64 ? 0 : 32)));
      PHC(52, 1) PHC(53, nb_wave) PHC(54, ND - 1 + nb_wave)
      for (int t = 0; t < ND - 1 + nb_wave && !degenerated; ++t) {
        float hcur[FMAX];
#pragma unroll
        for (int f = 0; f < FMAX; ++f) hcur[f] = s->H[row * DS + imn(imx(t - f, 0), ND - 2)];
        const int f_me = t - row;
        float dv = 0.0f, sg_me = 0.0f;
#pragma unroll
        for (int f = 0; f < FMAX; ++f) { dv = (f_me == f) ? W[f] : dv; sg_me = (f_me == f) ? sg[f] : sg_me; }
        const bool rot = own && sg_me != 0.0f && dm_abs(dv) > m.eps;
        const float tmp = Ld * Ld + sg_me * (dv * dv);
        const bool deg = rot && tmp < m.eps;
        const float r = dm_sqrt(tmp);
        const float cc = r / Ld;
        float cinv = 1.0f / cc;
        const float sk = dv / Ld;
        cinv = rot ? cinv : 0.0f;
        {
          const unsigned long long dbal = __ballot(deg);
          const unsigned long long mine = (T == 64) ? dbal : ((dbal >> ((threadIdx.x / T) * T)) & ((1ull << (T & 63)) - 1ull));
          if (mine != 0ull) { degenerated = true; break; }
        }
        if (rot) { Ld = r; s->H[row * DS + row] = r; }
        if (own) *(float4*)&s->rot[row][0] = make_float4(cc, cinv, sk, 0.0f);
        team_sync();
        float4 rp[FMAX];
#pragma unroll
        for (int f = 0; f < FMAX; ++f) rp[f] = *(const float4*)&s->rot[imn(imx(t - f, 0), ND - 2)][0];
#pragma unroll
        for (int f = 0; f < FMAX; ++f) {
          const int k = t - f;
          const bool on = (unsigned)k < urow && sg[f] != 0.0f && rp[f].y != 0.0f;
          const float hik = (hcur[f] + rp[f].z * W[f] * sg[f]) * rp[f].y;
          const float wn = W[f] * rp[f].x - rp[f].z * hik;
          float* dst = on ? &s->H[row * DS + k] : &s->rot[row][3];
          *dst = hik;
          W[f] = on ? wn : W[f];
        }
      }
    }
  }
  team_sync();
  if (!degenerated) {
    for (int idx = tl; idx < NTRI; idx += T) {
      int i, j;
      tri_index(m, idx, i, j);
      if (i != j) s->H[j * DS + i] = s->H[i * DS + j];
    }
    team_sync();
  }
  return degenerated;
}
template <int T, class S, class MT>
DEV bool ts_cholesky_incremental(const MT& m, S* s, int tl, int n_con) {
  if constexpr (T >= ND && (T == 32 || T == 64)) {
#if GO2SIM_FAST_ORDER
    int n_exact = 0;
    for (int base = 0; base < n_con; base += T) {
      const int c = base + tl;
      n_exact += __popcll(team_ballot<T>(c < n_con && ((s->active[c] != 0) != (s->prev_active[c] != 0))));
    }
    if (n_exact >= 1) return true;
    return false;
#else
    int n_flip = 0;
    for (int c = tl; c < n_con; c += T) n_flip += ((s->active[c] != 0) != (s->prev_active[c] != 0)) ? 1 : 0;
    unsigned long long any2, n_mine;
    {
      const unsigned long long fb = __ballot(n_flip > 0);
      const unsigned long long mine = (T == 64) ? fb : ((fb >> ((threadIdx.x / T) * T)) & ((1ull << (T & 63)) - 1ull));
      any2 = __ballot(__popcll(mine) >= 2);
      n_mine = mine;
    }
    if (any2 != 0ull) {
      const int n_team = __popcll(n_mine);
      const int n_wave = __builtin_amdgcn_readfirstlane(imx(__shfl(n_team, 0), __shfl(n_team, T == 64 ? 0 : 32)));
      if (n_wave <= 2) return ts_cholesky_incremental_pipelined<T, 2>(m, s, tl, n_con);
      if (n_wave <= 3) return ts_cholesky_incremental_pipelined<T, 3>(m, s, tl, n_con);
      if (n_wave <= 4) return ts_cholesky_incremental_pipelined<T, 4>(m, s, tl, n_con);
      if (n_wave <= 6) return ts_cholesky_incremental_pipelined<T, 6>(m, s, tl, n_con);
      return ts_cholesky_incremental_pipelined<T, 8>(m, s, tl, n_con);
    }
    return ts_cholesky_incremental_reg<T>(m, s, tl, n_con);
#endif
  }
  bool degenerated = false;
  for (int c = 0; c < n_con && !degenerated; ++c) {
    bool is_active = s->active[c] != 0, was_active = s->prev_active[c] != 0;
    if (is_active ^ was_active) {
      float sign = is_active ? 1.0f : -1.0f;
      float efc_D_sqrt = dm_sqrt(s->efc_D[c]);
      team_sync();
      for (int d = tl; d < ND; d += T) s->ntv[d] = s->J[c * DS + d] * efc_D_sqrt;
      team_sync();
      for (int k = 0; k < ND; ++k) {
        float vk = s->ntv[k];
        if (dm_abs(vk) > m.eps) {
          float Lkk = s->H[k * DS + k];
          float tmp = Lkk * Lkk + sign * (vk * vk);
          if (tmp < m.eps) { degenerated = true; break; }
          float r = dm_sqrt(tmp);
          float cc = r / Lkk;
          float cinv = 1.0f / cc;
          float sk = vk / Lkk;
          team_sync();
          if (tl == 0) s->H[k * DS + k] = r;
          for (int i = k + 1 + tl; i < ND; i += T) {
            float nv = s->ntv[i];
            float hik = (s->H[i * DS + k] + sk * nv * sign) * cinv;
            s->H[i * DS + k] = hik; s->H[k * DS + i] = hik;
            s->ntv[i] = nv * cc - sk * hik;
          }
          team_sync();
        }
      }
    }
  }
  return degenerated;
}

template <int T, class S>
DEV void ts_update_gradient(S* s, int tl) {
#if GO2SIM_FAST_ORDER
  if constexpr (T >= 32) {
    const int row = tl < ND ? tl : ND - 1;
    float Hr[ND];
#pragma unroll
    for (int k = 0; k < ND; ++k) Hr[k] = s->H[row * DS + k];
    const float g = s->Ma[row] - s->force[row] - s->qfrc[row];
    if (tl < ND) s->grad[row] = g;
    const float linv = 1.0f / s->H[row * DS + row];
    float cur = g;
#pragma unroll
    for (int j = 0; j < ND; ++j) {
      const float yj = team_bcast<T>(cur * linv, j);
      cur = (row == j) ? yj : ((row > j) ? cur - Hr[j] * yj : cur);
    }
#pragma unroll
    for (int j_ = 0; j_ < ND; ++j_) {
      const int j = ND - 1 - j_;
      const float xj = team_bcast<T>(cur * linv, j);
      cur = (row == j) ? xj : ((row < j) ? cur - Hr[j] * xj : cur);
    }
    if (tl < ND) s->Mgrad[row] = cur;
    team_sync();
    return;
  }
#endif
  for (int d = tl; d < ND; d += T) s->grad[d] = s->Ma[d] - s->force[d] - s->qfrc[d];
  team_sync();
  float y[ND];
#pragma unroll
  for (int i_d = 0; i_d < ND; ++i_d) {
    float cur = s->grad[i_d];
#pragma unroll
    for (int j_d = 0; j_d < i_d; ++j_d) cur = cur - s->H[i_d * DS + j_d] * y[j_d];
    y[i_d] = cur / s->H[i_d * DS + i_d];
  }
#pragma unroll
  for (int i_d_ = 0; i_d_ < ND; ++i_d_) {
    const int i_d = ND - 1 - i_d_;
    float cur = y[i_d];
#pragma unroll
    for (int j_d = i_d + 1; j_d < ND; ++j_d) cur = cur - s->H[i_d * DS + j_d] * y[j_d];
    y[i_d] = cur / s->H[i_d * DS + i_d];
  }
  if (tl == 0) {
#pragma unroll
    for (int d = 0; d < ND; ++d) s->Mgrad[d] = y[d];
  }
  team_sync();
}

struct LsRow { float Ja, jv, q0, q1, q2; };
#if GO2SIM_FAST_ORDER
template <int T, class S>
DEV void ts_ls_partials(S* s, int tl, int n_con, const LsRow& rw, float alpha, float (&p)[3]) {
  if (n_con <= T) {
    const float act = (float)((rw.Ja + alpha * rw.jv) < 0.0f);
    p[0] = rw.q0 * act; p[1] = rw.q1 * act; p[2] = rw.q2 * act;
    return;
  }
  p[0] = p[1] = p[2] = 0.0f;
  bool first = true;
  for (int c = tl; c < n_con; c += T) {
    const float act = (float)((s->Jaref[c] + alpha * s->jv[c]) < 0.0f);
    const float a0 = s->qf0[c] * act, a1 = s->qf1[c] * act, a2 = s->qf2[c] * act;
    p[0] = first ? a0 : p[0] + a0; p[1] = first ? a1 : p[1] + a1; p[2] = first ? a2 : p[2] + a2;
    first = false;
  }
}
#endif
template <int T, class S, class MT>
DEV LsPoint ts_ls_point(const MT& m, S* s, int tl, int n_con, int nseg, const LsRow& rw, float alpha, float qg0, float qg1, float qg2) {
  float t0 = qg0 + 0.0f, t1 = qg1 + 0.0f, t2 = qg2 + 0.0f;
  bool done = false;
#if GO2SIM_FAST_ORDER
  if constexpr (T >= 32) {
    float pp[3], tot[3];
    ts_ls_partials<T>(s, tl, n_con, rw, alpha, pp);
    team_tree_sum<T, 3>(pp, tot);
    t0 = tot[0] + t0; t1 = tot[1] + t1; t2 = tot[2] + t2;
    done = true;
  }
// ... 152 lines not shown
#pragma unroll
  for (int d = 0; d < ND; ++d) sr[d] = s->search[d];
#if GO2SIM_FAST_ORDER
  if constexpr (T >= 32) {
    const int d = tl < ND ? tl : ND - 1;
    float mv_own = 0.0f;
    for (int d1 = tl; d1 < ND; d1 += T) {
      float mv = 0.0f;
#pragma unroll
      for (int d2 = 0; d2 < ND; ++d2) mv = mv + s->M[d1 * DS + d2] * sr[d2];
      s->mv[d1] = mv; mv_own = mv;
    }
    LsRow rw = {0.0f, 0.0f, 0.0f, 0.0f, 0.0f};
    float pp[3] = {0.0f, 0.0f, 0.0f};
    bool first = true;
    for (int c = tl; c < n_con; c += T) {
      float jv = 0.0f;
#pragma unroll
      for (int dd = 0; dd < ND; ++dd) jv = jv + s->J[c * DS + dd] * sr[dd];
      s->jv[c] = jv;
      float Ja = s->Jaref[c], D = s->efc_D[c];
      const float q0 = D * (0.5f * Ja * Ja), q1 = D * (jv * Ja), q2 = D * (0.5f * jv * jv);
      s->qf0[c] = q0; s->qf1[c] = q1; s->qf2[c] = q2;
      rw.Ja = Ja; rw.jv = jv; rw.q0 = q0; rw.q1 = q1; rw.q2 = q2;
      const float active = (float)(Ja < 0.0f);
      const float a0 = q0 * active, a1 = q1 * active, a2 = q2 * active;
      pp[0] = first ? a0 : pp[0] + a0; pp[1] = first ? a1 : pp[1] + a1; pp[2] = first ? a2 : pp[2] + a2;
      first = false;
    }
    const float sd = s->search[d];
    const float xs[6] = {tl < ND ? sd * sd : 0.0f, tl < ND ? (sd * s->Ma[d] - sd * s->force[d]) : 0.0f, tl < ND ? 0.5f * sd * mv_own : 0.0f, pp[0], pp[1], pp[2]};
    float tot[6];
    team_tree_sum<T, 6>(xs, tot);
    team_sync();
    const float snorm = dm_sqrt(tot[0]);
    const float scale = m.meaninertia * (float)imx(1, ND);
    const float gtol = m.tolerance * m.ls_tolerance * snorm * scale;
    if (snorm < m.eps) return 0.0f;
    const int nseg = 0;
    const float qg0 = gauss, qg1 = tot[1], qg2 = tot[2];
    LsPoint p0;
    p0.alpha = 0.0f; p0.cost = tot[3] + qg0; p0.grad = tot[4] + qg1; p0.hess = 2.0f * (tot[5] + qg2);
    if (p0.hess <= 0.0f) p0.hess = m.eps;
    LS_MARK(50)
    return ts_linesearch_tail<T>(m, s, tl, n_con, nseg, rw, gtol, qg0, qg1, qg2, p0);
  }
#endif
  float snorm = 0.0f;
  if constexpr (T >= 32) {
    const float my = s->search[tl < ND ? tl : ND - 1];
#if GO2SIM_FAST_ORDER
    snorm = team_tree_sum1<T>(tl < ND ? my * my : 0.0f);
#else
    const float xq[1] = {tl < ND ? my * my : 0.0f}, zero[1] = {0.0f};
    float tot[1];
    team_serial_sum<T, 1>(xq, zero, tl, 2, tot);
    snorm = tot[0];
#endif
  } else {
#pragma unroll
    for (int jd = 0; jd < ND; ++jd) snorm = snorm + sr[jd] * sr[jd];
  }
  snorm = dm_sqrt(snorm);
  float scale = m.meaninertia * (float)imx(1, ND);
  float gtol = m.tolerance * m.ls_tolerance * snorm * scale;
  if (snorm < m.eps) return 0.0f;
  int nseg = 0;
  if constexpr (T >= 32) {
    const int n_wave = __builtin_amdgcn_readfirstlane(imx(__shfl(n_con, 0), __shfl(n_con, T == 64 ? 0 : 32)));
    nseg = (n_wave <= T) ? (n_wave + 15) / 16 : 0;
  }
  for (int d1 = tl; d1 < ND; d1 += T) {
    float mv = 0.0f;
#pragma unroll
    for (int d2 = 0; d2 < ND; ++d2) mv = mv + s->M[d1 * DS + d2] * sr[d2];
    s->mv[d1] = mv;
  }
  LsRow rw = {0.0f, 0.0f, 0.0f, 0.0f, 0.0f};
  for (int c = tl; c < n_con; c += T) {
    float jv = 0.0f;
#pragma unroll
    for (int d = 0; d < ND; ++d) jv = jv + s->J[c * DS + d] * sr[d];
    s->jv[c] = jv;
    float Ja = s->Jaref[c], D = s->efc_D[c];
    const float q0 = D * (0.5f * Ja * Ja), q1 = D * (jv * Ja), q2 = D * (0.5f * jv * jv);
    s->qf0[c] = q0; s->qf1[c] = q1; s->qf2[c] = q2;
    rw.Ja = Ja; rw.jv = jv; rw.q0 = q0; rw.q1 = q1; rw.q2 = q2;
  }
  team_sync();
  float qg1 = 0.0f, qg2 = 0.0f;
  if constexpr (T >= 32) {
    const int d = tl < ND ? tl : ND - 1;
    const float sd = s->search[d];
    const float xq[2] = {tl < ND ? (sd * s->Ma[d] - sd * s->force[d]) : 0.0f, tl < ND ? 0.5f * sd * s->mv[d] : 0.0f}, zero[2] = {0.0f, 0.0f};
    float tot[2];
#if GO2SIM_FAST_ORDER
    team_tree_sum<T, 2>(xq, tot);
#else
    team_serial_sum<T, 2>(xq, zero, tl, 2, tot);
#endif
    qg1 = tot[0]; qg2 = tot[1];
  } else {
#pragma unroll
    for (int d = 0; d < ND; ++d) {
      float sd = sr[d];
      qg1 = qg1 + (sd * s->Ma[d] - sd * s->force[d]);
      qg2 = qg2 + 0.5f * sd * s->mv[d];
    }
  }
  const float qg0 = gauss;
  LsPoint p0;
  {
    float t0 = qg0, t1 = qg1, t2 = qg2;
    bool done = false;
#if GO2SIM_FAST_ORDER
    if constexpr (T >= 32) {
      float pp[3], tot[3];
      if (n_con <= T) {
        const float active = (float)(rw.Ja < 0.0f);
        pp[0] = rw.q0 * active; pp[1] = rw.q1 * active; pp[2] = rw.q2 * active;
      } else {
        pp[0] = pp[1] = pp[2] = 0.0f;
// ... 17 lines not shown
        float tot[3];
        team_serial_sum<T, 3>(xs, bs, tl, nseg, tot);
        t0 = tot[0]; t1 = tot[1]; t2 = tot[2];
        done = true;
      }
    }
    if (!done) {
#pragma unroll 16
      for (int c = 0; c < n_con; ++c) {
        float active = (float)(s->Jaref[c] < 0.0f);
        t0 = t0 + s->qf0[c] * active; t1 = t1 + s->qf1[c] * active; t2 = t2 + s->qf2[c] * active;
      }
    }
    p0.alpha = 0.0f; p0.cost = t0; p0.grad = t1; p0.hess = 2.0f * t2;
    if (p0.hess <= 0.0f) p0.hess = m.eps;
  }
  LS_MARK(50)
  return ts_linesearch_tail<T>(m, s, tl, n_con, nseg, rw, gtol, qg0, qg1, qg2, p0);
}

#undef LS_MARK
template <int T, class S, class MT>
DEV int ts_solve(const MT& m, const E& e, S* s, int tl, int nc, int n_con, unsigned lim_mask, int ws_flag) {
  PH_BEGIN
  const bool ws = (n_con > 0) && ws_flag;
  team_stage<NTRI, T>(tl, [&](int k) { return aload(e, AO(mass_mat), k); }, [&](int k, float v) { int i, j; tri_index(m, k, i, j); s->M[i * DS + j] = v; s->M[j * DS + i] = v; });
  team_stage<ND * 3, T>(tl, [&](int k) { return aload(e, AO(cdof_ang), k); }, [&](int k, float v) { s->cdof_ang[k] = v; });
  team_stage<ND * 3, T>(tl, [&](int k) { return aload(e, AO(cdof_vel), k); }, [&](int k, float v) { s->cdof_vel[k] = v; });
  team_stage<NL * 3, T>(tl, [&](int k) { return gload(e, FO(root_com), k); }, [&](int k, float v) { s->root_com[k] = v; });
  team_stage<ND, T>(tl, [&](int d) { return gload(e, FO(vel), d); }, [&](int d, float v) { s->vel[d] = v; });
  team_stage<ND, T>(tl, [&](int d) { return aload(e, AO(force), d); }, [&](int d, float v) { s->force[d] = v; });
  team_stage<ND, T>(tl, [&](int d) { return aload(e, AO(acc_smooth), d); }, [&](int d, float v) { s->acc_smooth[d] = v; });
  team_stage<ND, T>(tl, [&](int d) { return aload(e, AO(qacc_ws), d); }, [&](int d, float v) { s->qacc[d] = v; });
  team_sync();
  if (!ws) team_for<ND, T>(tl, [&](int d) { s->qacc[d] = s->acc_smooth[d]; });
  team_sync();
  PH(0)
  bool rows_coupled = false;
  for (int r = tl; r < 4 * nc; r += T) {
    int i_col = r >> 2, i = r & 3;
    int link_a = e.c_link()[i_col], link_b = e.c_link()[MAXC + i_col];
    V3 cpos = e.c_pos()[i_col], cnormal = e.c_normal()[i_col];
    float friction = e.c_friction()[i_col], pen = e.c_pen()[i_col];
    float sol[7];
    auto csol = e.c_sol()[i_col];
#pragma unroll
    for (int k = 0; k < 7; ++k) sol[k] = csol[k];
    V3 d1, d2;
    orthogonals(cnormal, d1, d2);
    float invweight = m.links[link_a].invweight[0];
    if (link_b > -1) invweight = invweight + m.links[link_b].invweight[0];
    V3 d = (float)(2 * (i % 2) - 1) * ((i < 2) ? d1 : d2);
    V3 n = d * friction - cnormal;
    float* row = &s->J[r * DS];
#pragma unroll
    for (int i_d = 0; i_d < DS; ++i_d) row[i_d] = 0.0f;
    float jac_qvel = 0.0f;
    unsigned legs = 0u;
    for (int i_ab = 0; i_ab < 2; ++i_ab) {
      float sign = -1.0f; int link = link_a;
      if (i_ab == 1) { sign = 1.0f; link = link_b; }
      while (link > -1) {
        V3 t_pos = cpos - v3(s->root_com[3 * link], s->root_com[3 * link + 1], s->root_com[3 * link + 2]);
        const int nd = m.links[link].n_dofs, de = m.links[link].dof_end;
        if (nd > 0 && de > 6) legs |= 1u << dm_arrow_leg(m.arrow_mode, de - 1);
        for (int i_d_ = 0; i_d_ < nd; ++i_d_) {
          int i_d = de - 1 - i_d_;
          V3 ca = v3(s->cdof_ang[3 * i_d], s->cdof_ang[3 * i_d + 1], s->cdof_ang[3 * i_d + 2]);
          V3 cv = v3(s->cdof_vel[3 * i_d], s->cdof_vel[3 * i_d + 1], s->cdof_vel[3 * i_d + 2]);
// ... 6 lines not shown
        link = m.links[link].parent;
      }
    }
    float imp, aref;
    imp_aref(sol, -pen, jac_qvel, -pen, imp, aref);
    float diag = invweight + friction * friction * invweight;
    diag *= 2.0f * friction * friction * (1.0f - imp) / imp;
    diag = fmx(diag, m.eps);
    s->aref[r] = aref; s->efc_D[r] = 1.0f / diag;
    rows_coupled = rows_coupled || (legs & (legs - 1u)) != 0u;
  }
  for (int i_j = tl; i_j < NJ; i_j += T) {
    if (!((lim_mask >> i_j) & 1u)) continue;
    const Joint& Jt = m.joints[i_j];
    int i_d = Jt.dof_start;
    float q = gload(e, FO(qpos), Jt.q_start);
    float pos_delta_min = q - m.dofs[i_d].limit[0];
    float pos_delta_max = m.dofs[i_d].limit[1] - q;
    float pos_delta = fmn(pos_delta_min, pos_delta_max);
    {
      int r = 4 * nc + __popc(lim_mask & ((1u << i_j) - 1u));
      float j = (float)((pos_delta_min < pos_delta_max) * 2 - 1);
      float jac_qvel = j * s->vel[i_d];
      float imp, aref;
      imp_aref(Jt.sol_params, pos_delta, jac_qvel, pos_delta, imp, aref);
      float diag = fmx(m.dofs[i_d].invweight * (1.0f - imp) / imp, m.eps);
      s->aref[r] = aref; s->efc_D[r] = 1.0f / diag;
      float* row = &s->J[r * DS];
#pragma unroll
      for (int i_d2 = 0; i_d2 < DS; ++i_d2) row[i_d2] = 0.0f;
      row[i_d] = j;
    }
  }
  team_sync();
  PH(1)
  {
    float qa[ND];
#pragma unroll
    for (int d = 0; d < ND; ++d) qa[d] = s->qacc[d];
    for (int d1 = tl; d1 < ND; d1 += T) {
      float Ma_ = 0.0f;
#pragma unroll
      for (int d2 = 0; d2 < ND; ++d2) Ma_ = Ma_ + s->M[d1 * DS + d2] * qa[d2];
      s->Ma[d1] = Ma_;
    }
    for (int c = tl; c < n_con; c += T) {
      float Jv = -s->aref[c];
#pragma unroll
      for (int d = 0; d < ND; ++d) Jv = Jv + s->J[c * DS + d] * qa[d];
      s->Jaref[c] = Jv;
    }
  }
  team_sync();
  float cost = 0.0f, prev_cost = 0.0f, gauss = 0.0f;
  ts_update_constraint<T>(m, s, tl, n_con, cost, prev_cost, gauss);
  PH(2)
  int iters = 0;
  if (n_con > 0) {
    const float tol_scaled = (m.meaninertia * (float)imx(1, ND)) * m.tolerance;
    bool need_full = true;
    [[maybe_unused]] bool arrow = false;
#if GO2SIM_FAST_ORDER
    if constexpr (ARROW_SHAPE && (T == 32 || T == 64)) arrow = m.arrow_mode != 0 && team_ballot<T>(rows_coupled) == 0ull;
#endif
    for (int it = 0;; ++it) {
      if (need_full) {
#if GO2SIM_FAST_ORDER
        if constexpr (T >= 21) { if (it == 0) ts_hessian_direct<T>(m, s, tl, n_con); else ts_hessian_update<T>(m, s, tl, n_con); }
        else ts_hessian_direct<T>(m, s, tl, n_con);
        PH(3)
        if constexpr (ARROW_SHAPE && (T == 32 || T == 64)) { if (arrow) ts_cholesky_factor_arrow<T>(m, s, tl); else ts_cholesky_factor<T>(m, s, tl); }
        else ts_cholesky_factor<T>(m, s, tl);
#else
        ts_hessian_direct<T>(m, s, tl, n_con);
        PH(3)
        ts_cholesky_factor<T>(m, s, tl);
#endif
        PH(4)
      }
#if GO2SIM_FAST_ORDER
      [[maybe_unused]] float grad_sq_arrow = 0.0f;
      if constexpr (ARROW_SHAPE && (T == 32 || T == 64)) { if (arrow) grad_sq_arrow = ts_update_gradient_arrow<T>(m, s, tl); else ts_update_gradient<T>(s, tl); }
      else ts_update_gradient<T>(s, tl);
#else
      ts_update_gradient<T>(s, tl);
#endif
      PH(5)
      if (it > 0) {
        float improvement = prev_cost - cost;
        float grad_norm = 0.0f;
        if constexpr (T >= 32) {
          const float g = s->grad[tl < ND ? tl : ND - 1];
#if GO2SIM_FAST_ORDER
          if (ARROW_SHAPE && (T == 32 || T == 64) && arrow) grad_norm = grad_sq_arrow;
          else grad_norm = team_tree_sum1<T>(tl < ND ? g * g : 0.0f);
#else
          const float xq[1] = {tl < ND ? g * g : 0.0f}, zero[1] = {0.0f};
          float tot[1];
          team_serial_sum<T, 1>(xq, zero, tl, 2, tot);
          grad_norm = tot[0];
#endif
        } else {
#pragma unroll
          for (int d = 0; d < ND; ++d) { float g = s->grad[d]; grad_norm = grad_norm + g * g; }
        }
        grad_norm = dm_sqrt(grad_norm);
        bool improved = (grad_norm > tol_scaled) && (improvement > tol_scaled);
        if (!improved) break;
      }
      if (it == m.iterations) break;
      for (int d = tl; d < ND; d += T) s->search[d] = -s->Mgrad[d];
      team_sync();
      float alpha = ts_linesearch<T>(m, s, tl, n_con, gauss);
      PH(6)
      iters++;
      if (dm_abs(alpha) < m.eps) break;
      team_sync();
      for (int d = tl; d < ND; d += T) {
        s->qacc[d] = s->qacc[d] + s->search[d] * alpha;
        s->Ma[d] = s->Ma[d] + s->mv[d] * alpha;
      }
      for (int c = tl; c < n_con; c += T) s->Jaref[c] = s->Jaref[c] + s->jv[c] * alpha;
      team_sync();
      ts_update_constraint<T>(m, s, tl, n_con, cost, prev_cost, gauss);
      PH(7)
      need_full = ts_cholesky_incremental<T>(m, s, tl, n_con);
      team_sync();
      PH(8)
    }
  }
  return iters;
}

template <int T, class S, class MT>
DEV void ts_commit(const MT& m, const E& e, S* s, int tl, int nc, int n_con, int iters) {
  const int d0 = tl < ND ? tl : ND - 1, c0 = tl < nc ? tl : (nc > 0 ? nc - 1 : 0);
  const float qfs0 = aload(e, AO(qf_smooth), d0);
  V3 cn0 = v3(0, 0, 0); float fr0 = 0.0f; int lk0 = 0;
  if (nc > 0) { cn0 = e.c_normal()[c0]; fr0 = e.c_friction()[c0]; lk0 = e.c_link()[c0] | (e.c_link()[MAXC + c0] << 8); }
  int err = 0;
  for (int d = tl; d < ND; d += T) {
    float q = s->qacc[d];
    astore(e, AO(acc), d, q);
    astore(e, AO(force), d, ((d == d0) ? qfs0 : aload(e, AO(qf_smooth), d)) + s->qfrc[d]);
    astore(e, AO(qacc_ws), d, q);
    astore(e, AO(qfrc_constraint), d, s->qfrc[d]);
    if (isnan_(q)) err |= GO2SIM_ERR_INVALID_FORCE_NAN;
  }
  if (err) atomicOr(&e.err()[0], err);
  for (int c = tl; c < n_con; c += T) astore(e, AO(efc_force), c, s->efc_force[c]);
  if (tl == 0) { e.is_warmstart()[0] = 1; e.n_con()[0] = n_con; e.solver_iters()[0] = iters; }
  team_sync();
  float* cf = s->J;
  for (int i_c = tl; i_c < nc; i_c += T) {
    const bool pre = i_c == c0;
    V3 cnormal = pre ? cn0 : (V3)e.c_normal()[i_c]; float friction = pre ? fr0 : (float)e.c_friction()[i_c];
    V3 f = v3(0, 0, 0), d1, d2;
    orthogonals(cnormal, d1, d2);
#pragma unroll
    for (int i_dir = 0; i_dir < 4; ++i_dir) {
      V3 d = (float)(2 * (i_dir % 2) - 1) * ((i_dir < 2) ? d1 : d2);
      V3 n = d * friction - cnormal;
      f = f + n * s->efc_force[i_c * 4 + i_dir];
    }
    e.c_force()[i_c] = f;
    cf[4 * i_c] = f.x; cf[4 * i_c + 1] = f.y; cf[4 * i_c + 2] = f.z;
    ((int*)cf)[4 * i_c + 3] = pre ? lk0 : (e.c_link()[i_c] | (e.c_link()[MAXC + i_c] << 8));
  }
  team_sync();
  for (int i_l = tl; i_l < NL; i_l += T) {
    V3 acc = v3(0, 0, 0);
#pragma unroll 4
    for (int i_c = 0; i_c < nc; ++i_c) {
      int lk = ((const int*)cf)[4 * i_c + 3];
      int la = lk & 0xff, lb = lk >> 8;
      V3 f = v3(cf[4 * i_c], cf[4 * i_c + 1], cf[4 * i_c + 2]);
      if (la == i_l) acc = acc - f;
      if (lb == i_l) acc = acc + f;
    }
    e.contact_force()[i_l] = acc;
  }
}

template <int T>
DEVN void ts_solve_overflow(float* Pf, int* Pi, int PB, float* Pfa, int* Pia, int b, const LinkS* lnk, const unsigned char* tri_i, const unsigned char* tri_j,
                            const Model* __restrict__ gm, SolverData<MAXR>* s, int tl, int nc, int n_con, unsigned lim_mask, int ws_flag) {
  Pool P; P.f = Pf; P.i = Pi; P.B = PB; P.fa = Pfa; P.ia = Pia;
  const E e(P, b);
  const ModelView m(lnk, tri_i, tri_j, gm);
  int iters = ts_solve<T>(m, e, s, tl, nc, n_con, lim_mask, ws_flag);
  ts_commit<T>(m, e, s, tl, nc, n_con, iters);
}

template <int T, int RLN>
DEV void solve_body(const Pool& P, const Model* __restrict__ gm, const ModelS* __restrict__ mp, SolverData<MAXR>* __restrict__ overflow,
                    const int* __restrict__ lpt_rec, int* __restrict__ lpt_next, int lpt_cap, SolverData<RLN>* lds, char* blk_raw, int& b_out, bool& resident_out) {
  constexpr int EPW = 64 / T;
  const LinkS* lnk = (const LinkS*)blk_raw;
  const unsigned char* tri_i = (const unsigned char*)(blk_raw + sizeof(LinkS) * NL);
  const unsigned char* tri_j = tri_i + (NTRI + 1);
  static_assert(T >= NJ, "one lane per joint in the limit test");
  PH_BEGIN
  wg_dma_to_lds<SOLVER_BLOCK_BYTES>(blk_raw, mp->links);
  const int tl = threadIdx.x % T, slot = threadIdx.x / T;
  const int b = lpt_take(lpt_rec, lpt_cap, P.B, EPW, slot);
  if (lpt_next && blockIdx.x == 0) for (int i = threadIdx.x; i < 8 * LPT_CLS; i += 64) lpt_next[i] = 0;
  const bool env_valid = b < P.B;
  b_out = b; resident_out = false;
  E e(P, env_valid ? b : P.B - 1);
  const int nc = e.n_contacts()[0];
  const int ws_flag = e.is_warmstart()[0];
  const JLim jl = mp->jlim[tl < NJ ? tl : NJ - 1];
  const float q_lim = gload(e, FO(qpos), jl.q_start < 0 ? 0 : jl.q_start);
  const bool lim = tl < NJ && jl.q_start >= 0 && fmn(q_lim - jl.lo, jl.hi - q_lim) < 0;
  const unsigned lim_mask = (unsigned)((__ballot(lim) >> (slot * T)) & ((T == 64) ? ~0ull : ((1ull << T) - 1ull)));
  const int n_lim = __popc(lim_mask);
  __syncthreads();
  PH(9)
  const ModelView m(lnk, tri_i, tri_j, gm);
  if (!env_valid) return;
  const int n_con = 4 * nc + n_lim;
  if (n_con <= RLN) {
    SolverData<RLN>* s = &lds[slot];
    resident_out = true;
    int iters = ts_solve<T>(m, e, s, tl, nc, n_con, lim_mask, ws_flag);
    PH(10)
    ts_commit<T>(m, e, s, tl, nc, n_con, iters);
    PH(11)
  } else {
    ts_solve_overflow<T>(P.f, P.i, P.B, P.fa, P.ia, b, lnk, tri_i, tri_j, gm, &overflow[b], tl, nc, n_con, lim_mask, ws_flag);
  }
}
template <int T, int RLN>
__global__ __launch_bounds__(64) __attribute__((amdgpu_waves_per_eu(2, 2))) void k_constraint_solve_team(Pool P, const Model* __restrict__ gm, const ModelS* __restrict__ mp, SolverData<MAXR>* __restrict__ overflow,
                                                                                                         const int* __restrict__ lpt_rec, int* __restrict__ lpt_next, int lpt_cap) {
  STAMP(STK_SOLVE)
  constexpr int EPW = 64 / T;
  __shared__ SolverData<RLN> lds[EPW];
  __shared__ alignas(16) char blk_raw[lds_dma_bytes(SOLVER_BLOCK_BYTES)];
  int b; bool resident;
  solve_body<T, RLN>(P, gm, mp, overflow, lpt_rec, lpt_next, lpt_cap, lds, blk_raw, b, resident);
}

constexpr size_t cmax(size_t a, size_t b) { return a > b ? a : b; }
template <int T, int RLN, bool WITH_DYN>
__global__ __launch_bounds__(64) __attribute__((amdgpu_waves_per_eu(2, 2))) void k_solve_integrate_team(Pool P, const Model* __restrict__ gm, const ModelS* __restrict__ mp,
                                                                                                        SolverData<MAXR>* __restrict__ overflow, const int* __restrict__ lpt_rec,
                                                                                                        int* __restrict__ lpt_next, int lpt_cap) {
  STAMP(STK_SOLVE)
// ... 383 lines not shown
  auto hist = e.action_history();
  const int delay = e.delay_steps()[0];
  const float a_in = (ia < na) ? actions_in[(size_t)eb * na + ia] : 0.0f;
  const bool base_env = c.i[GO2SIM_IC_ENV_KIND] == 1;
  const int depth = c.i[GO2SIM_IC_MAX_DELAY] + 1;
  const int read_idx = (((write_idx - delay) % depth) + depth) % depth;
  const float h_ = base_env ? e.last_actions()[ia] : hist[read_idx][ia];
  const float kpf = e.kp_factors()[im], kdf = e.kd_factors()[im], mst = e.motor_strength()[im], dp = e.e_dof_pos()[im], dv = e.e_dof_vel()[im];
  const bool manual_pd = c.i[GO2SIM_IC_MANUAL_PD] != 0, pls = c.i[GO2SIM_IC_PLS_ENABLE] != 0;
  const bool base_gains = manual_pd && !pls && c.i[GO2SIM_IC_HAS_KP_RANGE];
  const float bkp = base_gains ? e.base_kp()[0] : c.f[GO2SIM_FC_KP], bkd = base_gains ? e.base_kd()[0] : c.f[GO2SIM_FC_KD];
  const bool push_on = c.i[GO2SIM_IC_HAS_PUSH] && g.push_enable;
  const int pl = c.i[GO2SIM_IC_PUSH_LINK];
  auto psf = e.push_stored_force(); auto prem = e.push_remaining(); auto cpf = e.current_push_force(); auto ext = e.ext();
  float psf_[3] = {psf[0], psf[1], psf[2]}; int rem0 = prem[0];
  const V3 pl_pos = e.l_pos()[pl], pl_com = e.root_com()[pl];
  float ext_[6];
#pragma unroll
  for (int k = 0; k < 6; ++k) ext_[k] = ext[6 * pl + k];
  team_stage<NL * 9, T>(tl, [&](int k) { return aload(e, AO(cinr_inertial), k); }, [&](int k, float v) { s->cinr_I[k] = v; s->crb_I[k] = v; });
  team_stage<NL * 3, T>(tl, [&](int k) { return aload(e, AO(cinr_pos), k); }, [&](int k, float v) { s->cinr_pos[k] = v; s->crb_pos[k] = v; });
  team_stage<NL, T>(tl, [&](int k) { return aload(e, AO(cinr_mass), k); }, [&](int k, float v) { s->cinr_mass[k] = v; s->crb_mass[k] = v; });
  team_stage<ND, T>(tl, [&](int d) { return __int_as_float((int)e.ctrl_mode()[d]); }, [&](int d, float v) { s->ctrl_mode[d] = __float_as_int(v); });
  team_stage<ND * 3, T>(tl, [&](int k) { return aload(e, AO(cdof_ang), k); }, [&](int k, float v) { s->cdof_ang[k] = v; });
  team_stage<ND * 3, T>(tl, [&](int k) { return aload(e, AO(cdof_vel), k); }, [&](int k, float v) { s->cdof_vel[k] = v; });
  team_stage<ND * 3, T>(tl, [&](int k) { return aload(e, AO(cdofd_ang), k); }, [&](int k, float v) { s->cdofd_ang[k] = v; });
  team_stage<ND * 3, T>(tl, [&](int k) { return aload(e, AO(cdofd_vel), k); }, [&](int k, float v) { s->cdofd_vel[k] = v; });
  team_stage<ND, T>(tl, [&](int d) { return gload(e, FO(ctrl_force), d); }, [&](int d, float v) { s->qf_applied[d] = v; });
  team_stage<ND, T>(tl, [&](int d) { return gload(e, FO(ctrl_pos), d); }, [&](int d, float v) { s->qf_passive[d] = v; });
  team_stage<ND, T>(tl, [&](int d) { return gload(e, FO(ctrl_vel), d); }, [&](int d, float v) { s->force[d] = v; });
  team_stage<ND, T>(tl, [&](int d) { return gload(e, FO(dof_pos), d); }, [&](int d, float v) { s->out[d] = v; });
  team_stage<NL * 6, T>(tl, [&](int k) { return gload(e, FO(ext), k); },
                        [&](int k, float v) { int i_l = k / 6, cc = k % 6; if (cc < 3) s->cfrc_ang[3 * i_l + cc] = v; else s->cfrc_vel[3 * i_l + cc - 3] = v; });
  team_sync();
  if (env_valid) {
    const float clip = c.f[GO2SIM_FC_CLIP_ACTIONS];
    float delayed = 0.0f;
    if (tl < NA && tl < na) {
      const float a = fmn(fmx(a_in, -clip), clip);
      e.actions()[tl] = a;
      if (base_env) delayed = (depth > 1) ? h_ : a;
      else { hist[write_idx][tl] = a; delayed = (read_idx == write_idx) ? a : h_; }
      e.applied_actions()[tl] = delayed;
    }
    const float delayed_leg = __shfl(delayed, NM + im / 3, T);
    if (tl < NM) {
      float target = delayed * c.f[GO2SIM_FC_ACTION_SCALE] + c.f[GO2SIM_FC_DEFAULT_DOF_POS0 + tl];
      if (g.action_noise_std_cur > 0.0) {
        dm_u4 r = rng4(seed, RNG_ACTION_NOISE, b, step_count, tl / 4);
        float n0, n1;
        if ((tl & 2) == 0) dm_normal2(r.v[0], r.v[1], &n0, &n1); else dm_normal2(r.v[2], r.v[3], &n0, &n1);
        target = target + ((tl & 1) ? n1 : n0) * (float)g.action_noise_std_cur;
      }
      e.target_dof_pos()[tl] = target;
      const int d = c.i[GO2SIM_IC_MOTOR_DOF0 + tl];
      if (!manual_pd) {
        e.ctrl_mode()[d] = CTRL_POSITION; e.ctrl_pos()[d] = target; e.ctrl_vel()[d] = 0.0f; e.ctrl_force()[d] = 0.0f;
        e.torque()[tl] = 0.0f;
        s->ctrl_mode[d] = CTRL_POSITION; s->qf_passive[d] = target; s->force[d] = 0.0f; s->qf_applied[d] = 0.0f;
      } else {
        float eff_kp, eff_kd;
        if (pls) {
          float kp_leg = c.f[GO2SIM_FC_PLS_KP_DEFAULT] + delayed_leg * c.f[GO2SIM_FC_PLS_KP_ACTION_SCALE];
          kp_leg = fmn(fmx(kp_leg, c.f[GO2SIM_FC_PLS_KP_MIN]), c.f[GO2SIM_FC_PLS_KP_MAX]);
          const float kd_j = 0.2f * dm_sqrt(kp_leg);
          eff_kp = kp_leg * kpf * mst;
          eff_kd = kd_j * kdf;
// ... 3 lines not shown
        const float pos_error = target - dp;
        float torque = eff_kp * pos_error - eff_kd * dv;
        const float lim = c.f[GO2SIM_FC_TORQUE_LIMIT0 + tl];
        torque = fmn(fmx(torque, -lim), lim);
        e.torque()[tl] = torque;
        e.ctrl_mode()[d] = CTRL_FORCE; e.ctrl_force()[d] = torque;
        s->ctrl_mode[d] = CTRL_FORCE; s->qf_applied[d] = torque;
      }
    }
    if (tl == T - 1) {
      if (!push_on) {
        cpf[0] = 0.0f; cpf[1] = 0.0f; cpf[2] = 0.0f;
      } else {
        if (g.push_counter % g.push_interval == 0) {
          dm_u4 r = rng4(seed, RNG_PUSH, b, step_count, 0);
          psf_[0] = rand_float(g.push_force_lo, g.push_force_hi, r.v[0]);
          psf_[1] = rand_float(g.push_force_lo, g.push_force_hi, r.v[1]);
          psf_[2] = 0.0f;
          psf[0] = psf_[0]; psf[1] = psf_[1]; psf[2] = psf_[2];
          rem0 = rand_int(c.i[GO2SIM_IC_PUSH_DUR_LO], c.i[GO2SIM_IC_PUSH_DUR_HI], r.v[2]);
        }
        const float active = (rem0 > 0) ? 1.0f : 0.0f;
        const V3 force = v3(psf_[0] * active, psf_[1] * active, psf_[2] * active);
        cpf[0] = force.x; cpf[1] = force.y; cpf[2] = force.z;
        prem[0] = imx(rem0 - 1, 0);
        const V3 tq = cross(pl_pos - pl_com, force);
        const float x0 = ext_[0] - tq.x, x1 = ext_[1] - tq.y, x2 = ext_[2] - tq.z, x3 = ext_[3] - force.x, x4 = ext_[4] - force.y, x5 = ext_[5] - force.z;
        ext[6 * pl + 0] = x0; ext[6 * pl + 1] = x1; ext[6 * pl + 2] = x2; ext[6 * pl + 3] = x3; ext[6 * pl + 4] = x4; ext[6 * pl + 5] = x5;
        s->cfrc_ang[3 * pl + 0] = x0; s->cfrc_ang[3 * pl + 1] = x1; s->cfrc_ang[3 * pl + 2] = x2;
        s->cfrc_vel[3 * pl + 0] = x3; s->cfrc_vel[3 * pl + 1] = x4; s->cfrc_vel[3 * pl + 2] = x5;
      }
    }
  }
  team_sync();
  PH(20)
  tk_dynamics<T>(m, e, s, tl, env_valid);
  if (env_valid) tk_broadphase<T>(*gm, e, lds_b.at(slot, s), tl);
}

struct RewCtx { float link_vel_xy[8], foot_z[4], foot_xy[8]; float vel_world[3]; int was_reset; };
struct RewState {
  float cmd[3], blv[3], bav[3], pg[3], base_pos[3];
  float dof_pos[NM], dof_vel[NM], last_dof_vel[NM], target[NM], ctrl_force[NM];
  float actions[NA], last_actions[NA];
  float fat[4]; int fc[4];
  float last_x;
  float ctrl_pos[NM], ctrl_vel[NM], s_vel[NM], s_dof_pos[NM]; int ctrl_mode[NM];
};
DEV void load_rew_state(const DCfg& c, const E& e, RewState& rs) {
  auto cmd = e.commands(); auto ldv = e.last_dof_vel(); auto t = e.target_dof_pos(); auto cf = e.ctrl_force(); auto a = e.actions(); auto la = e.last_actions();
  auto fat = e.feet_air_time();
#pragma unroll
  for (int i = 0; i < 3; ++i) rs.cmd[i] = cmd[i];
#pragma unroll
  for (int i = 0; i < NM; ++i) { rs.last_dof_vel[i] = ldv[i]; rs.target[i] = t[i]; rs.ctrl_force[i] = cf[c.i[GO2SIM_IC_MOTOR_DOF0 + i]]; }
#pragma unroll
  for (int i = 0; i < NA; ++i) { rs.actions[i] = a[i]; rs.last_actions[i] = la[i]; }
#pragma unroll
  for (int i = 0; i < 4; ++i) rs.fat[i] = fat[i];
  rs.last_x = e.last_base_pos_x()[0];
  if (c.i[GO2SIM_IC_ENV_KIND] == 1) {
    auto ctrl_mode = e.ctrl_mode(); auto cp = e.ctrl_pos(); auto cv = e.ctrl_vel(); auto vel = e.vel(); auto sdp = e.dof_pos();
#pragma unroll
    for (int i = 0; i < NM; ++i) {
      int d = c.i[GO2SIM_IC_MOTOR_DOF0 + i];
      rs.ctrl_mode[i] = ctrl_mode[d]; rs.ctrl_pos[i] = cp[d]; rs.ctrl_vel[i] = cv[d]; rs.s_vel[i] = vel[d]; rs.s_dof_pos[i] = sdp[d];
    }
// ... 726 lines not shown
  off = (k >= PB_PUSH) ? FO(current_push_force) + k - PB_PUSH : off;
  off = (k >= PB_REW) ? FO(rew) : off;
  off = (k >= PB_TIMEOUT) ? FO(time_out) : off;
  off = (k >= PB_ACTIONS) ? FO(actions) + k - PB_ACTIONS : off;
  return off;
}
template <int T>
__global__ __launch_bounds__(128) void k_env_post_b_team(Pool P, const Model* __restrict__ mp, const ModelS* __restrict__ msp, const DCfg* __restrict__ cp,
                                                        const Glob* __restrict__ gp, uint64_t seed, uint32_t step_count, float* __restrict__ obs_out,
                                                        float* __restrict__ priv_out, float* __restrict__ rew_out, uint8_t* __restrict__ reset_out,
                                                        float* __restrict__ timeout_out) {
  STAMP(STK_POST_B)
  constexpr int EPW = 64 / T;
  __shared__ KinData fk_lds[EPW];
  __shared__ alignas(16) char ms_raw[MODELS_LDS_BYTES];
  const bool fk_needed = gp->n_reset_now > 0;
  const int na = cp->i[GO2SIM_IC_NUM_ACTIONS], nobs = cp->i[GO2SIM_IC_NUM_OBS], npriv = cp->i[GO2SIM_IC_NUM_PRIV_OBS], env_kind = cp->i[GO2SIM_IC_ENV_KIND];
  const int lane = (int)threadIdx.x & 63, wave = (int)threadIdx.x >> 6;
  if (wave == 1) {
    if (!fk_needed) return;
    wg_dma_to_lds<(int)sizeof(ModelS)>(ms_raw, msp, lane);
  }
  const int tl = lane % T, slot = lane / T;
  const int b = xcd_block() * EPW + slot;
  if (wave == 1) {
    __syncthreads();
    __builtin_amdgcn_fence(__ATOMIC_ACQUIRE, "workgroup");
    if (b >= P.B) return;
    E e(P, b);
    KinData* ks = &fk_lds[slot];
    team_stage<ND, T>(tl, [&](int d) { return gload(e, FO(vel), d); }, [&](int d, float v) { ks->vel[d] = v; });
    team_stage<NQ, T>(tl, [&](int q) { return gload(e, FO(qpos), q); }, [&](int q, float v) { ks->qpos[q] = v; });
    tk_stage_links<T>(e, ks, tl);
    team_sync();
    const ModelView mv((const ModelS*)ms_raw, msp);
    tk_kinematics<T>(mv, e, ks, tl, true);
    return;
  }
  const bool valid = b < P.B;
  PH_BEGIN
  const Model& m = *mp; const DCfg& c = *cp; const Glob& g = *gp;
  E e(P, valid ? b : P.B - 1);
  auto fk_refresh = [&]() {};
  const int was_reset = valid ? e.reset_buf()[0] : 0;
  if (valid && g.n_reset_now > 0) {
    {
      const ResetDraws rd = env_reset_draws_team<T>(c, g, e, b, seed, tl, was_reset != 0);
      if (tl == 0 && was_reset) env_reset_one(m, c, g, e, b, seed, &rd);
    }
    const bool per_env = c.i[GO2SIM_IC_PER_ENV_GLOBAL_DR] != 0;
    if (c.i[GO2SIM_IC_HAS_FRICTION_DR] && !per_env) for (int i = tl; i < NG; i += T) e.geom_friction()[i] = g.friction;
    if (tl == 0) {
      int bl = c.i[GO2SIM_IC_BASE_LINK];
      if (c.i[GO2SIM_IC_HAS_MASS_DR] && !per_env) e.mass_shift()[bl] = g.mass_shift;
      if (c.i[GO2SIM_IC_HAS_COM_DR]) e.com_shift()[bl] = v3(g.com_shift[0], g.com_shift[1], g.com_shift[2]);
      if (c.i[GO2SIM_IC_HAS_LEGM_DR]) for (int k = 0; k < 4; ++k) e.mass_shift()[c.i[GO2SIM_IC_HIP_LINK0 + k]] = g.leg_mass_shift[k];
    }
    team_sync();
  }
  if (fk_needed) { __builtin_amdgcn_fence(__ATOMIC_RELEASE, "workgroup"); __syncthreads(); }
  PHB(0)
  if (!valid) return;
  if (env_kind == 1) {
    if (tl == 0) {
      RewCtx rc; rc.was_reset = was_reset;
      auto bvw = e.base_vel_world();
      for (int k = 0; k < 3; ++k) rc.vel_world[k] = was_reset ? 0.0f : bvw[k];
// ... 35 lines not shown
    for (int i = tl; i < NM; i += T) gstore(e, FO(last_dof_vel), i, gload(e, FO(e_dof_vel), i));
    if (tl == 0) {
      if (rew_out) rew_out[b] = e.rew()[0];
      if (reset_out) reset_out[b] = (uint8_t)was_reset;
      if (timeout_out) timeout_out[b] = e.time_out()[0];
    }
    fk_refresh();
    return;
  }
  __shared__ float pb_src[EPW][PB_N + 2];
  float* src = pb_src[slot];
  constexpr int PB_ROUNDS = (PB_N + T - 1) / T;
  float stg[PB_ROUNDS];
#pragma unroll
  for (int r = 0; r < PB_ROUNDS; ++r) {
    int k = r * T + tl; k = k < PB_N ? k : PB_N - 1;
    const float* p = (k < PB_POOL_N) ? e.f + (size_t)post_b_src_off(k) * e.B : (k < PB_GLOB) ? &c.f[GO2SIM_FC_DEFAULT_DOF_POS0 + k - PB_DEF] : (const float*)((const char*)&g + offsetof(Glob, friction)) + (k - PB_GLOB);
    stg[r] = *p;
  }
  const int delay_steps = e.delay_steps()[0];
  const bool noisy = c.i[GO2SIM_IC_HAS_OBS_NOISE] && c.d[GO2SIM_FC_OBS_NOISE_LEVEL_MAX] > 0.0;
  const double lvl = g.obs_noise_level_cur;
  const float s_ang = c.f[GO2SIM_FC_OBS_SCALE_ANG_VEL], s_lin = c.f[GO2SIM_FC_OBS_SCALE_LIN_VEL], s_dp = c.f[GO2SIM_FC_OBS_SCALE_DOF_POS], s_dv = c.f[GO2SIM_FC_OBS_SCALE_DOF_VEL];
  const float nv_ang = (float)(c.d[GO2SIM_FC_OBS_NOISE_ANG_VEL] * c.d[GO2SIM_FC_OBS_SCALE_ANG_VEL] * lvl), nv_grav = (float)(c.d[GO2SIM_FC_OBS_NOISE_GRAVITY] * lvl);
  const float nv_dp = (float)(c.d[GO2SIM_FC_OBS_NOISE_DOF_POS] * c.d[GO2SIM_FC_OBS_SCALE_DOF_POS] * lvl), nv_dv = (float)(c.d[GO2SIM_FC_OBS_NOISE_DOF_VEL] * c.d[GO2SIM_FC_OBS_SCALE_DOF_VEL] * lvl);
  const bool per_env_dr = c.i[GO2SIM_IC_PER_ENV_GLOBAL_DR] != 0;
  float n0[4] = {0.0f, 0.0f, 0.0f, 0.0f};
  if (noisy && tl * 4 < nobs) {
    dm_u4 r = rng4(seed, RNG_OBS_NOISE, b, step_count, tl);
    dm_normal2(r.v[0], r.v[1], &n0[0], &n0[1]); dm_normal2(r.v[2], r.v[3], &n0[2], &n0[3]);
  }
#pragma unroll
  for (int r = 0; r < PB_ROUNDS; ++r) { int k = r * T + tl; k = k < PB_N ? k : PB_N - 1; src[k] = stg[r]; }
  team_sync();
  PHB(1)
  for (int blk = tl; blk * 4 < nobs; blk += T) {
    float n[4] = {n0[0], n0[1], n0[2], n0[3]};
    if (noisy && blk != tl) {
      dm_u4 r = rng4(seed, RNG_OBS_NOISE, b, step_count, blk);
      dm_normal2(r.v[0], r.v[1], &n[0], &n[1]); dm_normal2(r.v[2], r.v[3], &n[2], &n[3]);
    }
#pragma unroll
    for (int k = 0; k < 4; ++k) {
      int i = 4 * blk + k;
      if (i < nobs) {
        float v, nv = 0.0f;
        if (i < 33) {
          const int a = (i < 3) ? PB_BAV + i : (i < 6) ? PB_PG + i - 3 : (i < 9) ? PB_CMD + i - 6 : (i < 21) ? PB_DP + i - 9 : PB_DV + i - 21;
          const float x = src[a];
          const float s = (i < 3) ? s_ang : (i < 8) ? s_lin : (i < 9) ? s_ang : (i < 21) ? s_dp : s_dv;
          nv = (i < 3) ? nv_ang : (i < 6) ? nv_grav : (i < 9) ? 0.0f : (i < 21) ? nv_dp : nv_dv;
          if (i >= 3 && i < 6) v = x + src[PB_GOFF + i - 3];
          else if (i >= 9 && i < 21) v = (x - src[PB_DEF + i - 9]) * s;
          else v = x * s;
        }
        else { v = (i - 33 < na) ? src[PB_ACT + i - 33] : gload(e, FO(obs), i); }
        if (noisy) v = v + n[k] * nv;
        gstore(e, FO(obs), i, v); gstore(e, FO(priv), i, v);
        if (obs_out) obs_out[(size_t)b * nobs + i] = v;
        if (priv_out) priv_out[(size_t)b * npriv + i] = v;
      }
    }
  }
  PHB(2)
  const int max_delay = c.i[GO2SIM_IC_MAX_DELAY], base_link = c.i[GO2SIM_IC_BASE_LINK], use_terrain = c.i[GO2SIM_IC_USE_TERRAIN], scan_n = c.i[GO2SIM_IC_SCAN_N], n_terrain_rows = c.i[GO2SIM_IC_N_TERRAIN_ROWS];
  for (int i = nobs + tl; i < npriv; i += T) {
    int j = i - nobs;
// ... 1029 lines not shown

int go2sim_debug_narrowphase(go2sim_t* h, int which, int i_ga, int i_gb, const float* pa, const float* qa, const float* pb, const float* qb, float* out8) {
  if (!h || !out8 || !pa || !qa || !pb || !qb || i_ga < 0 || i_gb < 0 || i_ga >= NG || i_gb >= NG || which < 0 || which > 6) return GO2SIM_E_BADARG;
  float* dout = nullptr;
  HIPCHK(hipSetDevice(h->device));
  HIPCHK(hipMalloc((void**)&dout, 8 * sizeof(float)));
  V3 pos_a = v3h(pa[0], pa[1], pa[2]), pos_b = v3h(pb[0], pb[1], pb[2]);
  Q4 quat_a = {qa[0], qa[1], qa[2], qa[3]}, quat_b = {qb[0], qb[1], qb[2], qb[3]};
  hipLaunchKernelGGL(k_debug_narrowphase, dim3(1), dim3(64), 0, 0, h->dm, which, i_ga, i_gb, pos_a, quat_a, pos_b, quat_b, h->gjk_scratch, dout);
  hipError_t e1 = hipGetLastError(), e2 = hipMemcpy(out8, dout, 8 * sizeof(float), hipMemcpyDeviceToHost);
  (void)hipFree(dout);
  HIPCHK(e1); HIPCHK(e2);
  return GO2SIM_E_OK;
}

#ifdef GO2SIM_STAMP
int go2sim_debug_stamps(go2sim_t* h, unsigned long long* stamps, unsigned* counts) {
  if (!h || !stamps || !counts) return GO2SIM_E_BADARG;
  HIPCHK(hipDeviceSynchronize());
  HIPCHK(hipMemcpyFromSymbol(stamps, HIP_SYMBOL(g_stamp), sizeof(unsigned long long) * ST_KINDS * ST_MAX_WG * ST_DEPTH * 2));
  HIPCHK(hipMemcpyFromSymbol(counts, HIP_SYMBOL(g_stamp_cnt), sizeof(unsigned) * ST_KINDS * ST_MAX_WG));
  return GO2SIM_E_OK;
}
#endif
#ifdef GO2SIM_PHASE_PROFILE
int go2sim_debug_phases(go2sim_t* h, unsigned long long* out64, int reset) {
  if (!h || !out64) return GO2SIM_E_BADARG;
  HIPCHK(hipDeviceSynchronize());
  HIPCHK(hipMemcpyFromSymbol(out64, HIP_SYMBOL(g_phase_cycles), sizeof(unsigned long long) * 64 * PH_MAX_WG));
  if (reset) { void* p = nullptr; HIPCHK(hipGetSymbolAddress(&p, HIP_SYMBOL(g_phase_cycles))); HIPCHK(hipMemset(p, 0, sizeof(unsigned long long) * 64 * PH_MAX_WG)); }
  return GO2SIM_E_OK;
}
#endif
int go2sim_debug_field(go2sim_t* h, const char* name, void** ptr, int* k, int* is_int) {
  if (!h || !name || !ptr) return GO2SIM_E_BADARG;
#define X(n, c) if (!strcmp(name, #n)) { *ptr = h->P.f + (size_t)FO(n) * h->B; if (k) *k = (c); if (is_int) *is_int = 0; return GO2SIM_E_OK; }
  GO2SIM_FLOAT_FIELDS(X)
#undef X
#define X(n, c) if (!strcmp(name, #n)) { *ptr = h->P.i + (size_t)IO(n) * h->B; if (k) *k = (c); if (is_int) *is_int = 1; return GO2SIM_E_OK; }
  GO2SIM_INT_FIELDS(X)
#undef X
  return GO2SIM_E_BADARG;
}

}
```

Measured before the change: 18.21 million.

## Narrow team barriers to LDS-only fences and explicit DMA waits; add sync profiler

Replaces many full workgroup fences (team_sync) with LDS-scoped fences where the protected data lives only in shared memory. The solver path picks its fence type from the storage policy S. After staging loads it uses an explicit vmcnt wait plus an LDS fence. Narrower fences avoid waiting on outstanding global memory operations at each barrier. This risks ordering bugs wherever global stores or reads actually needed the wider fence. It also adds an opt-in per-site sync-wait profiler under a compile flag.

```diff
diff --git a/go2_sim2real_locomotion_rl_amd/csrc/go2sim.hip b/go2_sim2real_locomotion_rl_amd/csrc/go2sim.hip
--- a/go2_sim2real_locomotion_rl_amd/csrc/go2sim.hip
+++ b/go2_sim2real_locomotion_rl_amd/csrc/go2sim.hip
@@ -629,6 +629,14 @@
   __builtin_amdgcn_wave_barrier();
   __builtin_amdgcn_fence(__ATOMIC_ACQUIRE, "workgroup", "local");
 }
+DEV void lds_dma_wait() {
+  __builtin_amdgcn_s_waitcnt(0x0F70);
+  team_sync_lds();
+}
+template <bool GLOBAL_MEM>
+DEV void mem_sync() { if constexpr (GLOBAL_MEM) team_sync(); else team_sync_lds(); }
+template <class S>
+DEV void store_sync() { mem_sync<S::GLOBAL_MEM>(); }
 DEV float gload(const E& e, int off, int k) { return e.f[(size_t)(off + k) * e.B]; }
 DEV void gstore(const E& e, int off, int k, float v) { e.f[(size_t)(off + k) * e.B] = v; }
 DEV float aload(const E& e, int off, int k) { return e.fa[off + k]; }
@@ -703,6 +711,69 @@
 #endif
 enum { STK_PRE_DYN = 0, STK_COLLIDE, STK_SOLVE, STK_INT_FK_DYN, STK_INT_FK, STK_POST_A, STK_POST_B, STK_OTHER };
 
+#ifdef GO2SIM_SYNC_PROFILE
+constexpr int SP_KINDS = 8, SP_SITES = 160, SP_MAX_WG = 4096;
+__device__ unsigned long long g_sync_site[SP_KINDS * SP_SITES * 2];
+__device__ unsigned long long g_sync_wg[SP_KINDS * SP_MAX_WG];
+__device__ int g_sync_line[SP_SITES];
+struct SpLds { unsigned cyc[2][SP_SITES]; unsigned short cnt[2][SP_SITES]; unsigned short line[SP_SITES]; };
+DEV SpLds* sp_lds() { __shared__ SpLds sp; return &sp; }
+template <int SITE, int LINE>
+struct SpSite {
+  static_assert(SITE >= 0 && SITE < SP_SITES && LINE < (1 << 14), "site table of the ordering points");
+  template <int FORM> static DEV void at() {
+    const unsigned long long t0 = __builtin_readcyclecounter();
+    if constexpr (FORM == 0) team_sync(); else if constexpr (FORM == 1) team_sync_lds(); else lds_dma_wait();
+    const unsigned long long t1 = __builtin_readcyclecounter();
+    SpLds* sp = sp_lds();
+    const int w = ((int)threadIdx.x >> 6) & 1;
+    if ((int)(threadIdx.x & 63) == __ffsll((long long)__ballot(1)) - 1) {
+      atomicAdd(&sp->cyc[w][SITE], (unsigned)(t1 - t0));
+      sp->cnt[w][SITE] = (unsigned short)(sp->cnt[w][SITE] + 1);
+      sp->line[SITE] = (unsigned short)(LINE | (FORM << 14));
+    }
+  }
+  template <bool GLOBAL_MEM> static DEV void mem() { at<GLOBAL_MEM ? 0 : 1>(); }
+  template <class S> static DEV void store() { at<S::GLOBAL_MEM ? 0 : 1>(); }
+};
+struct SpScope {
+  int kind;
+  DEV SpScope(int k) : kind(k) {
+    SpLds* sp = sp_lds();
+    const int w = ((int)threadIdx.x >> 6) & 1;
+    for (int i = (int)(threadIdx.x & 63); i < SP_SITES; i += 64) { sp->cyc[w][i] = 0u; sp->cnt[w][i] = 0; }
+    team_sync_lds();
+  }
+  DEV ~SpScope() {
+    team_sync_lds();
+    SpLds* sp = sp_lds();
+    const int w = ((int)threadIdx.x >> 6) & 1;
+    const unsigned long long act = __ballot(1);
+    const int n = __popcll(act), r = __popcll(act & ((1ull << (threadIdx.x & 63)) - 1ull));
+    unsigned long long tot = 0ull;
+    for (int i = r; i < SP_SITES; i += n) {
+      const unsigned k = sp->cnt[w][i];
+      if (k == 0u) continue;
+      const unsigned c = sp->cyc[w][i];
+      sp->cyc[w][i] = 0u; sp->cnt[w][i] = 0;
+      atomicAdd(&g_sync_site[(kind * SP_SITES + i) * 2], (unsigned long long)c);
+      atomicAdd(&g_sync_site[(kind * SP_SITES + i) * 2 + 1], (unsigned long long)k);
+      g_sync_line[i] = (int)sp->line[i];
+      tot += c;
+    }
+    if (tot != 0ull && blockIdx.x < SP_MAX_WG) atomicAdd(&g_sync_wg[kind * SP_MAX_WG + (int)blockIdx.x], tot);
+  }
+};
+#undef STAMP
+#define STAMP(kind) SpScope sp_scope_(kind);
+enum { SP_BASE = __COUNTER__ + 1 };
+#define team_sync() SpSite<__COUNTER__ - SP_BASE, __LINE__>::at<0>()
+#define team_sync_lds() SpSite<__COUNTER__ - SP_BASE, __LINE__>::at<1>()
+#define lds_dma_wait() SpSite<__COUNTER__ - SP_BASE, __LINE__>::at<2>()
+#define mem_sync SpSite<__COUNTER__ - SP_BASE, __LINE__>::template mem
+#define store_sync SpSite<__COUNTER__ - SP_BASE, __LINE__>::template store
+#endif
+
 enum { SV_COST = 0, SV_PREV_COST, SV_GAUSS, SV_QG0, SV_QG1, SV_QG2, SV_GTOL };
 enum { SI_LS_IT = 0, SI_LS_RESULT, SI_IMPROVED };
 
@@ -775,7 +846,7 @@
   return p + dpp_perm<0x128>(p);
 }
 DEV float4 lds4(const float* p) { return *(const float4*)p; }
-template <int T, int STRIDE>
+template <int T, int STRIDE, bool GLB = false>
 DEV void arrow_factor(const int mode, const float eps, const float* A, float* F, int tl) {
   static_assert(T == 32 || T == 64, "four groups of eight lanes");
   const int leg = (tl >> 3) & 3, u = tl & 7, ub = u < 6 ? u : 5;
@@ -787,7 +858,7 @@
   float br[6];
 #pragma unroll
   for (int j = 0; j < 6; ++j) br[j] = A[ub * STRIDE + j];
-  team_sync();
+  mem_sync<GLB>();
   const float e0 = fmx(a00, eps), i0 = dm_sqrt(e0) * (1.0f / e0);
   const float l10 = a10 * i0, l20 = a20 * i0;
   const float e1 = fmx(__builtin_fmaf(-l10, l10, a11), eps), i1 = dm_sqrt(e1) * (1.0f / e1);
@@ -796,7 +867,7 @@
   const float w0 = c0 * i0, w1 = __builtin_fmaf(-w0, l10, c1) * i1, w2 = __builtin_fmaf(-w1, l21, __builtin_fmaf(-w0, l20, c2)) * i2;
   if (w_lane) *(float4*)&F[32 * leg + 8 + 4 * u] = make_float4(w0, w1, w2, 0.0f);
   if (tl < 32 && u == 0) { *(float4*)&F[32 * leg] = make_float4(i0, i1, i2, 0.0f); *(float4*)&F[32 * leg + 4] = make_float4(l10, l20, l21, 0.0f); }
-  team_sync();
+  mem_sync<GLB>();
   float sc[6];
 #pragma unroll
   for (int j = 0; j < 6; ++j) {
@@ -807,14 +878,14 @@
   for (int j = 0; j < 6; ++j) sc[j] = leg_sum4(sc[j]);
   const float bp[6] = {br[0] - sc[0], br[1] - sc[1], br[2] - sc[2], br[3] - sc[3], br[4] - sc[4], br[5] - sc[5]};
   if (tl < 6) { *(float4*)&F[128 + 8 * tl] = make_float4(bp[0], bp[1], bp[2], bp[3]); *(float4*)&F[128 + 8 * tl + 4] = make_float4(bp[4], bp[5], 0.0f, 0.0f); }
-  team_sync();
+  mem_sync<GLB>();
   float a[6][6];
 #pragma unroll
   for (int k = 0; k < 6; ++k) {
     const float4 lo = lds4(&F[128 + 8 * k]); const float2 hi = *(const float2*)&F[128 + 8 * k + 4];
     a[k][0] = lo.x; a[k][1] = lo.y; a[k][2] = lo.z; a[k][3] = lo.w; a[k][4] = hi.x; a[k][5] = hi.y;
   }
-  team_sync();
+  mem_sync<GLB>();
 #pragma unroll
   for (int k = 0; k < 6; ++k) {
     const float e = fmx(a[k][k], eps), ik = dm_sqrt(e) * (1.0f / e);
@@ -833,9 +904,9 @@
       *(float2*)&F[128 + 8 * k + 4] = make_float2(k >= 4 ? a[k][4] : 0.0f, k >= 5 ? a[k][5] : 0.0f);
     }
   }
-  team_sync();
-}
-template <int T>
+  mem_sync<GLB>();
+}
+template <int T, bool GLB = false>
 DEV void arrow_solve(const float* F, float gl0, float gl1, float gl2, float gb, float* x6, int tl, float (&xb)[6], float& xl0, float& xl1, float& xl2) {
   static_assert(T == 32 || T == 64, "four groups of eight lanes");
   const int leg = (tl >> 3) & 3, u = tl & 7, ub = u < 6 ? u : 5;
@@ -852,10 +923,10 @@
   const float y0 = gl0 * iv.x, y1 = __builtin_fmaf(-lv.x, y0, gl1) * iv.y, y2 = __builtin_fmaf(-lv.z, y1, __builtin_fmaf(-lv.y, y0, gl2)) * iv.z;
   const float z = leg_sum4(__builtin_fmaf(wo.z, y2, __builtin_fmaf(wo.y, y1, wo.x * y0)));
   if (tl < 6) x6[tl] = gb - z;
-  team_sync();
+  mem_sync<GLB>();
   const float2 r0 = *(const float2*)&x6[0], r1 = *(const float2*)&x6[2], r2 = *(const float2*)&x6[4];
   float x[6] = {r0.x, r0.y, r1.x, r1.y, r2.x, r2.y};
-  team_sync();
+  mem_sync<GLB>();
 #pragma unroll
   for (int k = 0; k < 6; ++k) {
     float acc = x[k];
@@ -956,7 +1027,7 @@
         st3(s->l_pos, lk[d], pos); st4(s->l_quat, lk[d], quat); e.l_pos()[lk[d]] = pos; e.l_quat()[lk[d]] = quat;
       }
     }
-    team_sync();
+    team_sync_lds();
   }
   for (int lev = 0; lev < (legs ? 0 : m.n_levels); ++lev) {
     for (int k = m.level_start[lev] + tl; k < m.level_start[lev + 1]; k += T) {
@@ -996,7 +1067,7 @@
       }
       if (!(L.parent == -1 && L.is_fixed)) { st3(s->l_pos, i_l, pos); st4(s->l_quat, i_l, quat); e.l_pos()[i_l] = pos; e.l_quat()[i_l] = quat; }
     }
-    team_sync();
+    team_sync_lds();
   }
   PH(18)
   for (int i_l = tl; i_l < NL; i_l += T) {
@@ -1006,7 +1077,7 @@
     transform_pos_quat_by_trans_quat(L.inertial_pos + (V3)e.com_shift()[i_l], L.inertial_quat, ld3(s->l_pos, i_l), ld4(s->l_quat, i_l), ipbw, iq);
     st3(s->i_pos, i_l, ipbw); st4(s->i_quat, i_l, iq);
   }
-  team_sync();
+  team_sync_lds();
   V3 rc[2];
 #pragma unroll
   for (int i_e = 0; i_e < 2; ++i_e) {
@@ -1019,7 +1090,7 @@
     }
     rc[i_e] = root_com_bw / mass_sum;
   }
-  team_sync();
+  team_sync_lds();
   for (int i_l = tl; i_l < NL; i_l += T) {
     const auto& L = m.links[i_l];
     V3 r = (L.entity == 0) ? rc[0] : rc[1];
@@ -1075,7 +1146,7 @@
       e.g_pos()[i_g] = p; e.g_quat()[i_g] = q;
     }
   }
-  team_sync();
+  team_sync_lds();
   PH(19)
   if (legs) {
     const int r = m.leg_root, ds = m.links[r].dof_start;
@@ -1130,7 +1201,7 @@
         if (dk) { st3(dk->cd_vel, lk[d], cvel_vel); st3(dk->cd_ang, lk[d], cvel_ang); }
       }
     }
-    team_sync();
+    team_sync_lds();
   }
   for (int lev = 0; lev < (legs ? 0 : m.n_levels); ++lev) {
     for (int k = m.level_start[lev] + tl; k < m.level_start[lev + 1]; k += T) {
@@ -1178,7 +1249,7 @@
       if (!dk) { e.cd_vel()[i_l] = cvel_vel; e.cd_ang()[i_l] = cvel_ang; }
       if (dk) { st3(dk->cd_vel, i_l, cvel_vel); st3(dk->cd_ang, i_l, cvel_ang); }
     }
-    team_sync();
+    team_sync_lds();
   }
   PH(55)
 }
@@ -1204,19 +1275,19 @@
       for (int j_ = 0; j_ < L.q_end - qs; ++j_) s->qpos_next[qs + j_] = s->qpos[qs + j_] + s->vel_next[ds + j_] * m.substep_dt;
     }
   }
-  team_sync();
+  team_sync_lds();
   bool bad = false;
   for (int d = tl; d < ND; d += T) bad |= isnan_(s->vel_next[d]);
   for (int q = tl; q < NQ; q += T) bad |= isnan_(s->qpos_next[q]);
   if (bad) s->valid = 0;
-  team_sync();
+  team_sync_lds();
   if (s->valid) {
     for (int d = tl; d < ND; d += T) { float v = s->vel_next[d]; s->vel[d] = v; gstore(e, FO(vel), d, v); }
     for (int q = tl; q < NQ; q += T) { float v = s->qpos_next[q]; s->qpos[q] = v; gstore(e, FO(qpos), q, v); }
   } else if (tl == 0) {
     atomicOr(&e.err()[0], GO2SIM_ERR_INVALID_ACC_NAN);
   }
-  team_sync();
+  team_sync_lds();
 }
 
 template <int T>
@@ -1237,7 +1308,7 @@
   team_for<ND, T>(tl, [&](int d) { s->vel_next[d] = s->vel[d] + s->vel_next[d] * m.substep_dt; });
   if (tl == 0) s->valid = 1;
   tk_stage_links<T>(e, s, tl);
-  team_sync();
+  lds_dma_wait();
   if (b >= P.B) return;
   tk_integrate<T>(m, e, s, tl);
   PH(40)
@@ -1269,7 +1340,7 @@
   team_stage<ND, T>(tl, [&](int d) { return gload(e, FO(vel), d); }, [&](int d, float v) { s->vel[d] = v; });
   team_stage<NQ, T>(tl, [&](int q) { return gload(e, FO(qpos), q); }, [&](int q, float v) { s->qpos[q] = v; });
   tk_stage_links<T>(e, s, tl);
-  team_sync();
+  lds_dma_wait();
   if (b >= P.B) return;
   tk_kinematics<T>(m, e, s, tl, force_update_fixed != 0);
 }
@@ -1297,7 +1368,7 @@
       for (int l = 0; l < LEG_K; ++l) a = a + x[l][0];
       *at(r) = a;
     }
-    team_sync();
+    team_sync_lds();
   }
   for (int lev = (legs ? -1 : m.n_levels - 2); lev >= 0; --lev) {
     int n_par = m.level_start[lev + 1] - m.level_start[lev];
@@ -1312,7 +1383,7 @@
       }
       *dst = a;
     }
-    team_sync();
+    team_sync_lds();
   }
   PH(21)
   for (int i_d = tl; i_d < ND; i_d += T) {
@@ -1321,7 +1392,7 @@
     inertial_mul(ld3(s->crb_pos, i_l), ld9(s->crb_I, i_l), s->crb_mass[i_l], ld3(s->cdof_vel, i_d), ld3(s->cdof_ang, i_d), oa, ov);
     st3(s->f_ang, i_d, oa); st3(s->f_vel, i_d, ov);
   }
-  team_sync();
+  team_sync_lds();
   for (int idx = tl; idx < ND * (ND + 1) / 2; idx += T) {
     int i_d, j_d;
     tri_index(m, idx, i_d, j_d);
@@ -1335,7 +1406,7 @@
     s->M[i_d * ND + j_d] = v; s->M[j_d * ND + i_d] = v;
     s->L[i_d * ND + j_d] = v;
   }
-  team_sync();
+  team_sync_lds();
   PH(22)
 #if GO2SIM_FAST_ORDER
   const bool arrow = ARROW_SHAPE && (T == 32 || T == 64) && m.arrow_mode != 0;
@@ -1363,7 +1434,7 @@
 #pragma unroll
           for (int k = 0; k <= i_d; ++k) s->L[i_d * ND + k] = Lr[k];
         }
-        team_sync();
+        team_sync_lds();
       }
       float ri[ND];
 #pragma unroll
@@ -1376,14 +1447,14 @@
 #pragma unroll
       for (int k = 0; k < i_d; ++k) { const float nv = Lr[k] - a * ri[k]; Lr[k] = act ? nv : Lr[k]; }
     }
-    team_sync();
+    team_sync_lds();
     if (tl < ND) {
 #pragma unroll
       for (int k = 0; k < ND; ++k) if (k < row) s->L[row * ND + k] = Lr[k] * dinv_own;
       s->L[row * ND + row] = 1.0f;
       s->Dinv[row] = dinv_own;
     }
-    team_sync();
+    team_sync_lds();
   } else {
 #pragma unroll
     for (int i_d_ = 0; i_d_ < ND; ++i_d_) {
@@ -1395,10 +1466,10 @@
         float a = s->L[i_d * ND + j_d] * D_inv;
         s->L[j_d * ND + k_d] -= a * s->L[i_d * ND + k_d];
       }
-      team_sync();
+      team_sync_lds();
       for (int j_d = tl; j_d < i_d; j_d += T) s->L[i_d * ND + j_d] = s->L[i_d * ND + j_d] * D_inv;
       if (tl == 0) { s->Dinv[i_d] = D_inv; s->L[i_d * ND + i_d] = 1.0f; }
-      team_sync();
+      team_sync_lds();
     }
   }
   PH(23)
@@ -1447,7 +1518,7 @@
       if (m.links[i_l].parent != -1 || i_l == r) continue;
       st3(s->cdd_vel, i_l, -m.gravity * (1.0f - 0.0f)); st3(s->cdd_ang, i_l, v3(0, 0, 0));
     }
-    team_sync();
+    team_sync_lds();
   }
   for (int lev = 0; lev < (legs ? 0 : m.n_levels); ++lev) {
     for (int k = m.level_start[lev] + tl; k < m.level_start[lev + 1]; k += T) {
@@ -1465,7 +1536,7 @@
       }
       st3(s->cdd_vel, i_l, cv); st3(s->cdd_ang, i_l, ca);
     }
-    team_sync();
+    team_sync_lds();
   }
   for (int i_l = tl; i_l < NL; i_l += T) {
     V3 f1_ang, f1_vel, f2_ang, f2_vel, f3_ang, f3_vel;
@@ -1478,7 +1549,7 @@
     st3(s->cfrc_vel, i_l, f1_vel + f3_vel + ext_vel + v3(0, 0, 0));
     st3(s->cfrc_ang, i_l, f1_ang + f3_ang + ext_ang + v3(0, 0, 0));
   }
-  team_sync();
+  team_sync_lds();
   if (legs) {
     for (int c = tl; c < 6; c += T) {
       auto at = [&](int i_l) -> float* { return (c < 3) ? &s->cfrc_vel[3 * i_l + c] : &s->cfrc_ang[3 * i_l + c - 3]; };
@@ -1498,7 +1569,7 @@
       for (int l = 0; l < LEG_K; ++l) a = a + x[l][0];
       *at(r) = a;
     }
-    team_sync();
+    team_sync_lds();
   }
   for (int lev = (legs ? -1 : m.n_levels - 2); lev >= 0; --lev) {
     int n_par = m.level_start[lev + 1] - m.level_start[lev];
@@ -1512,7 +1583,7 @@
       }
       *dst = a;
     }
-    team_sync();
+    team_sync_lds();
   }
   for (int i_d = tl; i_d < ND; i_d += T) {
     int i_l = m.dof_link[i_d];
@@ -1521,7 +1592,7 @@
     s->force[i_d] = f;
     if (env_valid) { astore(e, AO(force), i_d, f); astore(e, AO(qf_smooth), i_d, f); }
   }
-  team_sync();
+  team_sync_lds();
   PH(24)
   bool solved = false;
 #if GO2SIM_FAST_ORDER
@@ -1564,7 +1635,7 @@
       for (int i_d = 0; i_d < ND; ++i_d) s->out[i_d] = y[i_d];
     }
   }
-  team_sync();
+  team_sync_lds();
   if (env_valid) for (int i_d = tl; i_d < ND; i_d += T) { float a = s->out[i_d]; astore(e, AO(acc_smooth), i_d, a); astore(e, AO(acc), i_d, a); }
   if (env_valid) for (int idx = tl; idx < NTRI; idx += T) { int i, j; tri_index(m, idx, i, j); astore(e, AO(mass_mat), idx, s->M[i * ND + j]); }
   PH(25)
@@ -1626,14 +1697,14 @@
     }
     lower_[g] = lower; upper_[g] = upper;
   }
-  team_sync();
+  team_sync_lds();
 #pragma unroll
   for (int g = 0; g < NGR; ++g) {
     const int i_g = (g * T + tl < NG) ? g * T + tl : NG - 1;
     *(float4*)&s->amin[4 * i_g] = make_float4(lower_[g].x, lower_[g].y, lower_[g].z, 0.0f);
     *(float4*)&s->amax[4 * i_g] = make_float4(upper_[g].x, upper_[g].y, upper_[g].z, 0.0f);
   }
-  team_sync();
+  team_sync_lds();
   PH(30)
   int r[NK]; float sorted_v[NK]; int sorted_sg[NK];
   unsigned long long key[NK];
@@ -1649,7 +1720,7 @@
     s->skey[i] = key[q];
     sorted_v[q] = v; sorted_sg[q] = sg; r[q] = 0;
   }
-  team_sync();
+  team_sync_lds();
 #pragma unroll
   for (int j = 0; j < 2 * NG; ++j) {
     const unsigned long long kj = s->skey[j];
@@ -1659,7 +1730,7 @@
 #pragma unroll
   for (int q = 0; q < NK; ++q)
     if (tl + q * T < n2) s->rank_mm[2 * (sorted_sg[q] & 0xff) + ((sorted_sg[q] & 0x100) ? 1 : 0)] = r[q];
-  team_sync();
+  team_sync_lds();
   PH(31)
   int n_cand = 0;
   unsigned ncv_clear = 0u;
@@ -1690,14 +1761,14 @@
   }
   const bool overflow = n_cand > m.max_broad_pairs;
   n_cand = imn(n_cand, MAXB);
-  team_sync();
+  team_sync_lds();
   for (int c = tl; c < n_cand; c += T) {
     const int ck = s->cand_key[c]; int cr = 0;
     for (int j = 0; j < n_cand; ++j) cr += s->cand_key[j] < ck;
     s->pair_sorted[cr] = (unsigned)s->cand_pair[c];
   }
   const int n_broad = imn(n_cand, m.max_broad_pairs);
-  team_sync();
+  team_sync_lds();
   for (int c = tl; c < n_broad; c += T) e.broad()[c] = (int)s->pair_sorted[c];
 #pragma unroll
   for (int q = 0; q < NK; ++q) if (tl + q * T < n2) { e.sort_value()[r[q]] = sorted_v[q]; e.sort_ig()[r[q]] = sorted_sg[q]; }
@@ -1749,7 +1820,7 @@
   team_stage<ND, T>(tl, [&](int d) { return gload(e, FO(dof_pos), d); }, [&](int d, float v) { s->out[d] = v; });
   team_stage<NL * 6, T>(tl, [&](int k) { return gload(e, FO(ext), k); },
                         [&](int k, float v) { int i_l = k / 6, c = k % 6; if (c < 3) s->cfrc_ang[3 * i_l + c] = v; else s->cfrc_vel[3 * i_l + c - 3] = v; });
-  team_sync();
+  lds_dma_wait();
   PH(20)
   tk_dynamics<T>(m, e, s, tl, env_valid);
   if (env_valid) tk_broadphase<T>(*gm, e, lds_b.at(slot, s), tl);
@@ -1787,7 +1858,7 @@
   team_for<ND, T>(tl, [&](int i) { s->vel_next[i] = s->vel[i] + s->vel_next[i] * m.substep_dt; });
   if (tl == 0) s->valid = 1;
   tk_stage_links<T>(e, s, tl);
-  team_sync();
+  lds_dma_wait();
   if (b >= P.B) return;
   tk_integrate<T>(m, e, s, tl);
   PH(40)
@@ -2480,7 +2551,7 @@
 #pragma unroll
   for (int q = 0; q < NPRE; ++q) if (tl + q * T < n_broad) s->pair_w[tl + q * T] = (unsigned)pw_ld[q];
   for (int c = tl + NPRE * T; c < n_broad; c += T) s->pair_w[c] = (unsigned)e.broad()[c];
-  team_sync();
+  lds_dma_wait();
   PH(62)
   int nc_run = 0;
   const int n_np_iter = (n_broad + T - 1) / T;
@@ -2808,8 +2879,10 @@
 constexpr int RL_TERRAIN = 96;
 constexpr int DS = 20;
 
+static_assert(RL != MAXR && RL_TERRAIN != MAXR, "SolverData<MAXR> is the global overflow record, the smaller stores are LDS blocks");
 template <int R>
 struct alignas(16) SolverData {
+  static constexpr bool GLOBAL_MEM = (R == MAXR);
   float J[R * DS];
   float H[ND * DS];
   float M[ND * DS];
@@ -2917,7 +2990,7 @@
     row_cost = rc;
 #endif
   }
-  team_sync();
+  store_sync<S>();
   for (int d = tl; d < ND; d += T) {
     float q = 0.0f;
 #pragma unroll 16
@@ -2962,7 +3035,7 @@
     for (int c = 0; c < n_con; ++c) { float Ja = s->Jaref[c]; cost_i = cost_i + 0.5f * (Ja * Ja * s->DA[c]); }
     gauss = gauss_i; cost = cost_i;
   }
-  team_sync();
+  store_sync<S>();
 }
 
 #if GO2SIM_FAST_ORDER
@@ -3012,7 +3085,7 @@
         }
     }
   }
-  team_sync();
+  store_sync<S>();
 }
 template <int T, class S, class MT>
 DEV void ts_hessian_update(const MT& m, S* s, int tl, int n_con) {
@@ -3055,7 +3128,7 @@
         if (j <= i) s->H[i * DS + j] = h[a][q];
       }
   }
-  team_sync();
+  store_sync<S>();
 }
 #else
 template <int T, class S, class MT>
@@ -3073,7 +3146,7 @@
     h = h + s->M[i * DS + j];
     s->H[i * DS + j] = h;
   }
-  team_sync();
+  store_sync<S>();
 }
 #endif
 
@@ -3097,7 +3170,7 @@
       float v = (s->H[j_d * DS + i_d] - dotv) * inv;
       s->H[j_d * DS + i_d] = v; s->H[i_d * DS + j_d] = v;
     }
-    team_sync();
+    store_sync<S>();
   }
 }
 template <int T, class S, class MT>
@@ -3117,7 +3190,7 @@
     if (own && row >= k) s->H[row * DS + k] = (row == k) ? d : l;
     if (k < ND - 1) {
       if (own && row > k) s->H[k * DS + row] = l;
-      team_sync();
+      store_sync<S>();
       float col[ND];
 #pragma unroll
       for (int i = k + 1; i < ND; ++i) col[i] = s->H[k * DS + i];
@@ -3125,11 +3198,11 @@
       for (int i = k + 1; i < ND; ++i) r[i] = __builtin_fmaf(-l, col[i], r[i]);
     }
   }
-  team_sync();
+  store_sync<S>();
 }
 #if GO2SIM_FAST_ORDER
 template <int T, class S, class MT>
-DEV void ts_cholesky_factor_arrow(const MT& m, S* s, int tl) { arrow_factor<T, DS>(m.arrow_mode, m.eps, s->H, s->H, tl); }
+DEV void ts_cholesky_factor_arrow(const MT& m, S* s, int tl) { arrow_factor<T, DS, S::GLOBAL_MEM>(m.arrow_mode, m.eps, s->H, s->H, tl); }
 template <int T, class S, class MT>
 DEV float ts_update_gradient_arrow(const MT& m, S* s, int tl) {
   const int leg = (tl >> 3) & 3, u = tl & 7, ub = u < 6 ? u : 5;
@@ -3141,10 +3214,10 @@
   if (tl < ND) s->grad[row] = g_own;
   const float grad_sq = team_tree_sum1<T>(tl < ND ? g_own * g_own : 0.0f);
   float xb[6], x0, x1, x2;
-  arrow_solve<T>(s->H, gl0, gl1, gl2, gb, s->Mgrad, tl, xb, x0, x1, x2);
+  arrow_solve<T, S::GLOBAL_MEM>(s->H, gl0, gl1, gl2, gb, s->Mgrad, tl, xb, x0, x1, x2);
   if (tl == 0) { *(float4*)&s->Mgrad[0] = make_float4(xb[0], xb[1], xb[2], xb[3]); *(float2*)&s->Mgrad[4] = make_float2(xb[4], xb[5]); }
   if (tl < 32 && u == 0) { s->Mgrad[p0] = x0; s->Mgrad[p1] = x1; s->Mgrad[p2] = x2; }
-  team_sync();
+  store_sync<S>();
   return grad_sq;
 }
 #endif
@@ -3203,7 +3276,7 @@
     for (int k = 0; k < ND; ++k)
       if (k <= row) { s->H[row * DS + k] = Lr[k]; if (k < row) s->H[k * DS + row] = Lr[k]; }
   }
-  team_sync();
+  store_sync<S>();
   return degenerated;
 }
 template <int T, int FMAX, class S, class MT>
@@ -3257,7 +3330,7 @@
         }
         if (rot) { Ld = r; s->H[row * DS + row] = r; }
         if (own) *(float4*)&s->rot[row][0] = make_float4(cc, cinv, sk, 0.0f);
-        team_sync();
+        store_sync<S>();
         float4 rp[FMAX];
 #pragma unroll
         for (int f = 0; f < FMAX; ++f) rp[f] = *(const float4*)&s->rot[imn(imx(t - f, 0), ND - 2)][0];
@@ -3274,14 +3347,14 @@
       }
     }
   }
-  team_sync();
+  store_sync<S>();
   if (!degenerated) {
     for (int idx = tl; idx < NTRI; idx += T) {
       int i, j;
       tri_index(m, idx, i, j);
       if (i != j) s->H[j * DS + i] = s->H[i * DS + j];
     }
-    team_sync();
+    store_sync<S>();
   }
   return degenerated;
 }
@@ -3324,9 +3397,9 @@
     if (is_active ^ was_active) {
       float sign = is_active ? 1.0f : -1.0f;
       float efc_D_sqrt = dm_sqrt(s->efc_D[c]);
-      team_sync();
+      store_sync<S>();
       for (int d = tl; d < ND; d += T) s->ntv[d] = s->J[c * DS + d] * efc_D_sqrt;
-      team_sync();
+      store_sync<S>();
       for (int k = 0; k < ND; ++k) {
         float vk = s->ntv[k];
         if (dm_abs(vk) > m.eps) {
@@ -3337,7 +3410,7 @@
           float cc = r / Lkk;
           float cinv = 1.0f / cc;
           float sk = vk / Lkk;
-          team_sync();
+          store_sync<S>();
           if (tl == 0) s->H[k * DS + k] = r;
           for (int i = k + 1 + tl; i < ND; i += T) {
             float nv = s->ntv[i];
@@ -3345,7 +3418,7 @@
             s->H[i * DS + k] = hik; s->H[k * DS + i] = hik;
             s->ntv[i] = nv * cc - sk * hik;
           }
-          team_sync();
+          store_sync<S>();
         }
       }
     }
@@ -3377,12 +3450,12 @@
       cur = (row == j) ? xj : ((row < j) ? cur - Hr[j] * xj : cur);
     }
     if (tl < ND) s->Mgrad[row] = cur;
-    team_sync();
+    store_sync<S>();
     return;
   }
 #endif
   for (int d = tl; d < ND; d += T) s->grad[d] = s->Ma[d] - s->force[d] - s->qfrc[d];
-  team_sync();
+  store_sync<S>();
   float y[ND];
 #pragma unroll
   for (int i_d = 0; i_d < ND; ++i_d) {
@@ -3403,7 +3476,7 @@
 #pragma unroll
     for (int d = 0; d < ND; ++d) s->Mgrad[d] = y[d];
   }
-  team_sync();
+  store_sync<S>();
 }
 
 struct LsRow { float Ja, jv, q0, q1, q2; };
@@ -3622,7 +3695,7 @@
     const float xs[6] = {tl < ND ? sd * sd : 0.0f, tl < ND ? (sd * s->Ma[d] - sd * s->force[d]) : 0.0f, tl < ND ? 0.5f * sd * mv_own : 0.0f, pp[0], pp[1], pp[2]};
     float tot[6];
     team_tree_sum<T, 6>(xs, tot);
-    team_sync();
+    store_sync<S>();
     const float snorm = dm_sqrt(tot[0]);
     const float scale = m.meaninertia * (float)imx(1, ND);
     const float gtol = m.tolerance * m.ls_tolerance * snorm * scale;
@@ -3677,7 +3750,7 @@
     s->qf0[c] = q0; s->qf1[c] = q1; s->qf2[c] = q2;
     rw.Ja = Ja; rw.jv = jv; rw.q0 = q0; rw.q1 = q1; rw.q2 = q2;
   }
-  team_sync();
+  store_sync<S>();
   float qg1 = 0.0f, qg2 = 0.0f;
   if constexpr (T >= 32) {
     const int d = tl < ND ? tl : ND - 1;
@@ -3761,9 +3834,9 @@
   team_stage<ND, T>(tl, [&](int d) { return aload(e, AO(force), d); }, [&](int d, float v) { s->force[d] = v; });
   team_stage<ND, T>(tl, [&](int d) { return aload(e, AO(acc_smooth), d); }, [&](int d, float v) { s->acc_smooth[d] = v; });
   team_stage<ND, T>(tl, [&](int d) { return aload(e, AO(qacc_ws), d); }, [&](int d, float v) { s->qacc[d] = v; });
-  team_sync();
+  store_sync<S>();
   if (!ws) team_for<ND, T>(tl, [&](int d) { s->qacc[d] = s->acc_smooth[d]; });
-  team_sync();
+  store_sync<S>();
   PH(0)
   bool rows_coupled = false;
   for (int r = tl; r < 4 * nc; r += T) {
@@ -3836,7 +3909,7 @@
       row[i_d] = j;
     }
   }
-  team_sync();
+  store_sync<S>();
   PH(1)
   {
     float qa[ND];
@@ -3855,7 +3928,7 @@
       s->Jaref[c] = Jv;
     }
   }
-  team_sync();
+  store_sync<S>();
   float cost = 0.0f, prev_cost = 0.0f, gauss = 0.0f;
   ts_update_constraint<T>(m, s, tl, n_con, cost, prev_cost, gauss);
   PH(2)
@@ -3914,22 +3987,22 @@
       }
       if (it == m.iterations) break;
       for (int d = tl; d < ND; d += T) s->search[d] = -s->Mgrad[d];
-      team_sync();
+      store_sync<S>();
       float alpha = ts_linesearch<T>(m, s, tl, n_con, gauss);
       PH(6)
       iters++;
       if (dm_abs(alpha) < m.eps) break;
-      team_sync();
+      store_sync<S>();
       for (int d = tl; d < ND; d += T) {
         s->qacc[d] = s->qacc[d] + s->search[d] * alpha;
         s->Ma[d] = s->Ma[d] + s->mv[d] * alpha;
       }
       for (int c = tl; c < n_con; c += T) s->Jaref[c] = s->Jaref[c] + s->jv[c] * alpha;
-      team_sync();
+      store_sync<S>();
       ts_update_constraint<T>(m, s, tl, n_con, cost, prev_cost, gauss);
       PH(7)
       need_full = ts_cholesky_incremental<T>(m, s, tl, n_con);
-      team_sync();
+      store_sync<S>();
       PH(8)
     }
   }
@@ -3954,7 +4027,7 @@
   if (err) atomicOr(&e.err()[0], err);
   for (int c = tl; c < n_con; c += T) astore(e, AO(efc_force), c, s->efc_force[c]);
   if (tl == 0) { e.is_warmstart()[0] = 1; e.n_con()[0] = n_con; e.solver_iters()[0] = iters; }
-  team_sync();
+  store_sync<S>();
   float* cf = s->J;
   for (int i_c = tl; i_c < nc; i_c += T) {
     const bool pre = i_c == c0;
@@ -3971,7 +4044,7 @@
     cf[4 * i_c] = f.x; cf[4 * i_c + 1] = f.y; cf[4 * i_c + 2] = f.z;
     ((int*)cf)[4 * i_c + 3] = pre ? lk0 : (e.c_link()[i_c] | (e.c_link()[MAXC + i_c] << 8));
   }
-  team_sync();
+  store_sync<S>();
   for (int i_l = tl; i_l < NL; i_l += T) {
     V3 acc = v3(0, 0, 0);
 #pragma unroll 4
@@ -4019,6 +4092,7 @@
   const bool lim = tl < NJ && jl.q_start >= 0 && fmn(q_lim - jl.lo, jl.hi - q_lim) < 0;
   const unsigned lim_mask = (unsigned)((__ballot(lim) >> (slot * T)) & ((T == 64) ? ~0ull : ((1ull << T) - 1ull)));
   const int n_lim = __popc(lim_mask);
+  lds_dma_wait();
   __syncthreads();
   PH(9)
   const ModelView m(lnk, tri_i, tri_j, gm);
@@ -4468,7 +4542,7 @@
   team_stage<ND, T>(tl, [&](int d) { return gload(e, FO(dof_pos), d); }, [&](int d, float v) { s->out[d] = v; });
   team_stage<NL * 6, T>(tl, [&](int k) { return gload(e, FO(ext), k); },
                         [&](int k, float v) { int i_l = k / 6, cc = k % 6; if (cc < 3) s->cfrc_ang[3 * i_l + cc] = v; else s->cfrc_vel[3 * i_l + cc - 3] = v; });
-  team_sync();
+  lds_dma_wait();
   if (env_valid) {
     const float clip = c.f[GO2SIM_FC_CLIP_ACTIONS];
     float delayed = 0.0f;
@@ -4538,7 +4612,7 @@
       }
     }
   }
-  team_sync();
+  team_sync_lds();
   PH(20)
   tk_dynamics<T>(m, e, s, tl, env_valid);
   if (env_valid) tk_broadphase<T>(*gm, e, lds_b.at(slot, s), tl);
@@ -5331,7 +5405,7 @@
     team_stage<ND, T>(tl, [&](int d) { return gload(e, FO(vel), d); }, [&](int d, float v) { ks->vel[d] = v; });
     team_stage<NQ, T>(tl, [&](int q) { return gload(e, FO(qpos), q); }, [&](int q, float v) { ks->qpos[q] = v; });
     tk_stage_links<T>(e, ks, tl);
-    team_sync();
+    lds_dma_wait();
     const ModelView mv((const ModelS*)ms_raw, msp);
     tk_kinematics<T>(mv, e, ks, tl, true);
     return;
@@ -5433,7 +5507,7 @@
   }
 #pragma unroll
   for (int r = 0; r < PB_ROUNDS; ++r) { int k = r * T + tl; k = k < PB_N ? k : PB_N - 1; src[k] = stg[r]; }
-  team_sync();
+  team_sync_lds();
   PHB(1)
   for (int blk = tl; blk * 4 < nobs; blk += T) {
     float n[4] = {n0[0], n0[1], n0[2], n0[3]};
@@ -6529,6 +6603,21 @@
   return GO2SIM_E_OK;
 }
 #endif
+#ifdef GO2SIM_SYNC_PROFILE
+int go2sim_debug_sync_wait(go2sim_t* h, unsigned long long* site, unsigned long long* wg, int* line, int reset) {
+  if (!h || !site || !wg || !line) return GO2SIM_E_BADARG;
+  HIPCHK(hipDeviceSynchronize());
+  HIPCHK(hipMemcpyFromSymbol(site, HIP_SYMBOL(g_sync_site), sizeof(unsigned long long) * SP_KINDS * SP_SITES * 2));
+  HIPCHK(hipMemcpyFromSymbol(wg, HIP_SYMBOL(g_sync_wg), sizeof(unsigned long long) * SP_KINDS * SP_MAX_WG));
+  HIPCHK(hipMemcpyFromSymbol(line, HIP_SYMBOL(g_sync_line), sizeof(int) * SP_SITES));
+  if (reset) {
+    void* p = nullptr;
+    HIPCHK(hipGetSymbolAddress(&p, HIP_SYMBOL(g_sync_site))); HIPCHK(hipMemset(p, 0, sizeof(unsigned long long) * SP_KINDS * SP_SITES * 2));
+    HIPCHK(hipGetSymbolAddress(&p, HIP_SYMBOL(g_sync_wg))); HIPCHK(hipMemset(p, 0, sizeof(unsigned long long) * SP_KINDS * SP_MAX_WG));
+  }
+  return GO2SIM_E_OK;
+}
+#endif
 int go2sim_debug_field(go2sim_t* h, const char* name, void** ptr, int* k, int* is_int) {
   if (!h || !name || !ptr) return GO2SIM_E_BADARG;
 #define X(n, c) if (!strcmp(name, #n)) { *ptr = h->P.f + (size_t)FO(n) * h->B; if (k) *k = (c); if (is_int) *is_int = 0; return GO2SIM_E_OK; }
```

Result: no change. 18.25 million, median of 3 (+0.2%).
